# a1q123456/image_stitching

Hardware: AMD Instinct MI355X
Metric: 4K frames stitched/sec (higher is better)
Workload: dtype u8

## Files before the change

host/job.cpp:

```cpp
#include "job.hpp"
#include <algorithm>
#include <cstring>
#include <numeric>

namespace mis {

static float median_focal(const std::vector<CameraParams>& cams, const std::vector<int>& idx) {
    std::vector<double> f;
    for (int i : idx) f.push_back(cams[i].focal);
    std::sort(f.begin(), f.end());
    return f.size() % 2 == 1 ? static_cast<float>(f[f.size() / 2]) : static_cast<float>(f[f.size() / 2 - 1] + f[f.size() / 2]) * 0.5f;
}

void StitchJob::check(MisContext* c, int rc, const char* what) const {
    if (rc != MIS_OK) throw std::runtime_error(std::string(what) + " failed: " + mis_last_error(c));
}

StitchJob::StitchJob(int device, int width, int height, const std::vector<CameraParams>& cameras, const StitchConfig& cfg)
    : w_(width), h_(height), n_((int)cameras.size()), cams_(cameras), cfg_(cfg) {
    if (cfg_.features_type != "orb" || cfg_.ba_cost_func != "no" || cfg_.expos_comp_type != "no" || cfg_.seam_find_type != "no")
        throw std::runtime_error("mis::StitchJob runs the hot path (ORB, supplied cameras, no seam-scale step); use mis::Stitcher for the other options");
    if (mis_context_create(device, nullptr, &ctx_) != MIS_OK) throw std::runtime_error("mis_context_create failed: no HIP device (there is no CPU fallback)");
    check(ctx_, mis_stream_create(device, 0, &cstream_), "mis_stream_create");
    if (mis_context_create(device, cstream_, &cctx_) != MIS_OK) throw std::runtime_error("mis_context_create (compose stream) failed");
// ... 24 lines not shown
    check(ctx_, mis_context_synchronize(ctx_), "mis_context_synchronize");
    check(cctx_, mis_context_synchronize(cctx_), "mis_context_synchronize (compose)");
}

StitchJob::Compose StitchJob::prepare(const std::vector<int>& idx) {
    const int m = (int)idx.size();
    const float scale = median_focal(cams_, idx);
    std::vector<float> Ks((size_t)m * 9), Rs((size_t)m * 9);
    for (int k = 0; k < m; k++) {
        std::copy(Ks_.begin() + 9 * idx[k], Ks_.begin() + 9 * idx[k] + 9, Ks.begin() + 9 * k);
        std::copy(Rs_.begin() + 9 * idx[k], Rs_.begin() + 9 * idx[k] + 9, Rs.begin() + 9 * k);
    }
    rois_.assign(m, MisRect{});
    check(cctx_, mis_warp_roi_batch(cctx_, scale, w_, h_, m, Ks.data(), Rs.data(), rois_.data()), "mis_warp_roi_batch");
    std::vector<MisPoint> corners(m);
    std::vector<MisSize> sizes(m);
    for (int k = 0; k < m; k++) { corners[k] = {rois_[k].x, rois_[k].y}; sizes[k] = {rois_[k].width, rois_[k].height}; }
    Compose c;
    check(cctx_, mis_result_roi(corners.data(), sizes.data(), m, &c.pano), "mis_result_roi");
    check(cctx_, mis_blend_config(cfg_.blend_type, cfg_.blend_strength, c.pano.width, c.pano.height, &c.type, &c.bands, &c.sharp), "mis_blend_config");
    if (!blender_ || c.type != key_.type || c.bands != key_.bands || c.sharp != key_.sharp) {
        if (blender_) { mis_blender_destroy(blender_); blender_ = nullptr; }
        check(cctx_, mis_blender_create(cctx_, c.type, c.bands, c.sharp, &blender_), "mis_blender_create");
    }
    key_ = c;
    check(cctx_, mis_blender_prepare(blender_, corners.data(), sizes.data(), m), "mis_blender_prepare");
    return c;
}

void StitchJob::compose(const std::vector<MisImage>& frames, const std::vector<int>& idx) {
    const int m = (int)idx.size();
    const float scale = median_focal(cams_, idx);
    std::vector<MisImage> fr(m);
    std::vector<float> Ks((size_t)m * 9), Rs((size_t)m * 9);
    for (int k = 0; k < m; k++) {
        fr[k] = frames[idx[k]];
        std::copy(Ks_.begin() + 9 * idx[k], Ks_.begin() + 9 * idx[k] + 9, Ks.begin() + 9 * k);
        std::copy(Rs_.begin() + 9 * idx[k], Rs_.begin() + 9 * idx[k] + 9, Rs.begin() + 9 * k);
    }
    check(cctx_, mis_compose_frames(blender_, fr.data(), m, scale, Ks.data(), Rs.data(), rois_.data()), "mis_compose_frames");
}

void StitchJob::finalize() {
    if (pano_.data && (pano_.width != key_.pano.width || pano_.height != key_.pano.height)) { mis_image_free(cctx_, &pano_); mis_image_free(cctx_, &mask_); pano_ = MisImage{}; mask_ = MisImage{}; }
    if (!pano_.data) { pano_ = MisImage{}; mask_ = MisImage{}; pano_.mem = mask_.mem = MIS_MEM_DEVICE; }
    check(cctx_, mis_blender_blend(blender_, &pano_, &mask_), "mis_blender_blend");
}

void StitchJob::hook(void* self_) {
    StitchJob* self = static_cast<StitchJob*>(self_);
    self->hook_ran_ = true;
    try {
        const int rc = mis_match_knn_fence(self->ctx_, self->cstream_, mis_match_sequence(self->ctx_), 0);
        if (rc < 0) self->check(self->ctx_, rc, "mis_match_knn_fence");
        std::vector<int> everyone(self->n_);
        std::iota(everyone.begin(), everyone.end(), 0);
        self->compose(*self->hook_frames_, everyone);
        self->finalize();
    } catch (const std::exception& e) {
        self->hook_error_ = e.what();
    }
}

void StitchJob::prep_hook(void* self_) {
    StitchJob* self = static_cast<StitchJob*>(self_);
    self->prep_ran_ = true;
    try {
        std::vector<int> everyone(self->n_);
        std::iota(everyone.begin(), everyone.end(), 0);
        self->prepare(everyone);
    } catch (const std::exception& e) { self->prep_error_ = e.what(); }
}

JobOutput StitchJob::run(const std::vector<MisImage>& frames) {
    if ((int)frames.size() != n_) throw std::runtime_error("StitchJob::run: one frame per camera");
    JobOutput out;
    std::vector<int> everyone(n_);
    std::iota(everyone.begin(), everyone.end(), 0);
    check(cctx_, mis_context_wait(cctx_, ctx_), "mis_context_wait");
    prep_ran_ = false; prep_error_.clear();
    check(ctx_, mis_orb_on_enqueued(orb_, &StitchJob::prep_hook, this), "mis_orb_on_enqueued");
    std::vector<MisFeatures> feats(n_);
    std::memset(feats.data(), 0, sizeof(MisFeatures) * n_);
    const int rc_f = mis_orb_detect_batch(orb_, frames.data(), n_, feats.data());
    mis_orb_on_enqueued(orb_, nullptr, nullptr);
    check(ctx_, rc_f, "mis_orb_detect_batch");
    if (!prep_ran_) prep_hook(this);
    if (!prep_error_.empty()) throw std::runtime_error(prep_error_);
    for (int i = 0; i < n_; i++) { feats[i].img_idx = i; out.num_features.push_back(feats[i].n); }
    if (!pairwise_.empty()) { mis_matches_free(pairwise_.data(), (int)pairwise_.size()); pairwise_.clear(); }
    pairwise_.assign((size_t)n_ * n_, MisMatchesInfo{});
    MisMatchParams mp;
    mis_match_default_params(&mp);
    mp.match_conf = cfg_.match_conf;
    hook_frames_ = &frames; hook_ran_ = false; hook_error_.clear();
    check(ctx_, mis_match_on_enqueued(ctx_, &StitchJob::hook, this), "mis_match_on_enqueued");
    const int rc = mis_match_all_pairs(ctx_, feats.data(), n_, &mp, pairwise_.data());
    mis_match_on_enqueued(ctx_, nullptr, nullptr);
    for (auto& f : feats) mis_features_free(ctx_, &f);
    check(ctx_, rc, "mis_match_all_pairs");
    if (!hook_ran_) hook(this);
    if (!hook_error_.empty()) throw std::runtime_error(hook_error_);
    out.confidence.resize((size_t)n_ * n_);
    for (int k = 0; k < n_ * n_; k++) out.confidence[k] = pairwise_[k].confidence;
    std::vector<int> idx(n_);
    int kept = 0;
    check(ctx_, mis_leave_biggest_component(pairwise_.data(), n_, cfg_.conf_thresh, idx.data(), &kept), "mis_leave_biggest_component");
    idx.resize(kept);
    if (kept < 2) throw std::runtime_error("Need more images");
    out.indices = idx;
    out.speculation_kept = kept == n_;
    if (!out.speculation_kept) {
        prepare(idx);
        compose(frames, idx);
        finalize();
    }
    check(cctx_, mis_context_synchronize(cctx_), "mis_context_synchronize (compose)");
    out.pano = pano_; out.mask = mask_;
    out.num_bands = key_.bands; out.pano_width = key_.pano.width; out.pano_height = key_.pano.height;
    out.matches = pairwise_;
    return out;
}

}
```

image_stitching_amd/_capi.py:

```python
import ctypes as C
import os
import re

_HERE = os.path.dirname(os.path.abspath(__file__))
LIB_PATH = os.path.join(_HERE, "libmistitch.so")
HEADER_PATH = os.path.join(os.path.dirname(_HERE), "include", "mistitch.h")

MIS_OK = 0
MIS_FENCE_TIMEOUT = 1
MEM_HOST, MEM_DEVICE = 0, 1
U8, S16, F32 = 0, 1, 2
INTER_NEAREST, INTER_LINEAR = 0, 1
BORDER_CONSTANT, BORDER_REFLECT = 0, 2
BLEND_NO, BLEND_FEATHER, BLEND_MULTI_BAND = 0, 1, 2


class MisPoint(C.Structure):
    _fields_ = [("x", C.c_int), ("y", C.c_int)]


class MisSize(C.Structure):
    _fields_ = [("width", C.c_int), ("height", C.c_int)]


class MisRect(C.Structure):
    _fields_ = [("x", C.c_int), ("y", C.c_int), ("width", C.c_int), ("height", C.c_int)]


class MisLevelRect(C.Structure):
    _fields_ = [("level", C.c_int), ("x0", C.c_int), ("y0", C.c_int), ("x1", C.c_int), ("y1", C.c_int), ("offset", C.c_ulonglong)]


class MisImage(C.Structure):
    _fields_ = [("data", C.c_void_p), ("width", C.c_int), ("height", C.c_int), ("channels", C.c_int),
                ("stride", C.c_size_t), ("dtype", C.c_int), ("mem", C.c_int)]


class MisKeyPoint(C.Structure):
    _fields_ = [("x", C.c_float), ("y", C.c_float), ("size", C.c_float), ("angle", C.c_float),
                ("response", C.c_float), ("octave", C.c_int)]


class MisOrbParams(C.Structure):
    _fields_ = [("nfeatures", C.c_int), ("scale_factor", C.c_float), ("nlevels", C.c_int),
                ("edge_threshold", C.c_int), ("first_level", C.c_int), ("wta_k", C.c_int),
                ("score_type", C.c_int), ("patch_size", C.c_int), ("fast_threshold", C.c_int)]


class MisSiftParams(C.Structure):
    _fields_ = [("nfeatures", C.c_int), ("n_octave_layers", C.c_int), ("contrast_threshold", C.c_double),
                ("edge_threshold", C.c_double), ("sigma", C.c_double)]


class MisCameraParams(C.Structure):
    _fields_ = [("focal", C.c_double), ("aspect", C.c_double), ("ppx", C.c_double), ("ppy", C.c_double), ("R", C.c_double * 9),
                ("t", C.c_double * 3)]


class MisFeatures(C.Structure):
    _fields_ = [("img_idx", C.c_int), ("img_w", C.c_int), ("img_h", C.c_int), ("n", C.c_int),
                ("keypoints", C.c_void_p), ("descriptors", C.c_void_p), ("desc_cols", C.c_int),
                ("desc_dtype", C.c_int), ("owner_", C.c_void_p)]


class MisMatchParams(C.Structure):
    _fields_ = [("match_conf", C.c_float), ("num_matches_thresh1", C.c_int), ("num_matches_thresh2", C.c_int),
                ("ransac_thresh", C.c_double), ("max_iters", C.c_int), ("confidence", C.c_double)]


class MisDMatch(C.Structure):
    _fields_ = [("query_idx", C.c_int), ("train_idx", C.c_int), ("img_idx", C.c_int), ("distance", C.c_float)]


class MisMatchesInfo(C.Structure):
    _fields_ = [("src_img_idx", C.c_int), ("dst_img_idx", C.c_int), ("n_matches", C.c_int),
                ("matches", C.POINTER(MisDMatch)), ("inliers_mask", C.POINTER(C.c_uint8)), ("num_inliers", C.c_int),
                ("has_H", C.c_int), ("H", C.c_double * 9), ("confidence", C.c_double)]


_vp, _i, _f, _d = C.c_void_p, C.c_int, C.c_float, C.c_double
_P = C.POINTER

PROTOTYPES = {
    "mis_context_create": (_i, [_i, _vp, _P(_vp)]),
    "mis_stream_create": (_i, [_i, _i, _P(_vp)]),
    "mis_stream_destroy": (_i, [_vp]),
    "mis_context_destroy": (_i, [_vp]),
    "mis_context_synchronize": (_i, [_vp]),
    "mis_context_wait": (_i, [_vp, _vp]),
    "mis_last_error": (C.c_char_p, [_vp]),
    "mis_version": (C.c_char_p, []),
    "mis_image_free": (_i, [_vp, _P(MisImage)]),
    "mis_orb_default_params": (None, [_P(MisOrbParams)]),
    "mis_orb_create": (_i, [_vp, _P(MisOrbParams), _i, _i, _P(_vp)]),
    "mis_orb_destroy": (_i, [_vp]),
    "mis_orb_detect": (_i, [_vp, _P(MisImage), _P(MisFeatures)]),
    "mis_orb_detect_batch": (_i, [_vp, _P(MisImage), _i, _P(MisFeatures)]),
    "mis_orb_on_enqueued": (_i, [_vp, _vp, _vp]),
    "mis_features_download": (_i, [_vp, _P(MisFeatures), _vp, _vp]),
    "mis_features_upload": (_i, [_vp, _i, _i, _i, _vp, _vp, _i, _i, _P(MisFeatures)]),
    "mis_features_free": (_i, [_vp, _P(MisFeatures)]),
    "mis_orb_debug_level": (_i, [_vp, _i, _i, _vp, _P(_i), _P(_i)]),
    "mis_sift_default_params": (None, [_P(MisSiftParams)]),
    "mis_sift_create": (_i, [_vp, _P(MisSiftParams), _i, _i, _P(_vp)]),
    "mis_sift_destroy": (_i, [_vp]),
    "mis_sift_detect": (_i, [_vp, _P(MisImage), _P(MisFeatures)]),
    "mis_sift_detect_batch": (_i, [_vp, _P(MisImage), _i, _P(MisFeatures)]),
    "mis_sift_debug_level": (_i, [_vp, _P(MisImage), _i, _i, _i, _vp, _P(_i), _P(_i)]),
    "mis_match_default_params": (None, [_P(MisMatchParams)]),
    "mis_match_all_pairs": (_i, [_vp, _P(MisFeatures), _i, _P(MisMatchParams), _P(MisMatchesInfo)]),
    "mis_match_pairs_sharded": (_i, [_vp, _P(MisFeatures), _i, _P(MisMatchParams), _i, _i, _P(MisMatchesInfo)]),
    "mis_matches_free": (_i, [_P(MisMatchesInfo), _i]),
    "mis_match_sequence": (C.c_longlong, [_vp]),
    "mis_match_knn_fence": (_i, [_vp, _vp, C.c_longlong, _i]),
    "mis_match_on_enqueued": (_i, [_vp, _vp, _vp]),
    "mis_knn2": (_i, [_vp, _P(MisFeatures), _P(MisFeatures), _vp, _vp]),
    "mis_find_homography": (_i, [_vp, _vp, _vp, _i, _d, _i, _d, _vp, _vp, _P(_i)]),
    "mis_leave_biggest_component": (_i, [_P(MisMatchesInfo), _i, _f, _vp, _P(_i)]),
    "mis_leave_biggest_component_conf": (_i, [_vp, _i, _f, _vp, _P(_i)]),
    "mis_bundle_adjust_reproj": (_i, [_vp, _P(MisFeatures), _P(MisMatchesInfo), _i, _f, C.c_char_p, _P(MisCameraParams)]),
    "mis_wave_correct": (_i, [_vp, _i, _i]),
    "mis_warp_roi": (_i, [_f, _i, _i, _vp, _vp, _P(MisRect)]),
    "mis_warp_spherical": (_i, [_vp, _P(MisImage), _f, _vp, _vp, _i, _i, _P(MisImage), _P(MisPoint)]),
    "mis_warp_roi_batch": (_i, [_vp, _f, _i, _i, _i, _vp, _vp, _P(MisRect)]),
    "mis_warp_spherical_fused_roi": (_i, [_vp, _P(MisImage), _f, _vp, _vp, _P(MisRect), _P(MisImage), _P(MisImage), _P(MisPoint)]),
    "mis_warp_spherical_fused_batch": (_i, [_vp, _P(MisImage), _i, C.c_float, _P(C.c_float), _P(C.c_float), _P(MisRect), _P(MisImage), _P(MisImage), _P(MisPoint)]),
    "mis_warp_spherical_fused_batch_timed": (_i, [_vp, _P(MisImage), _i, C.c_float, _P(C.c_float), _P(C.c_float), _P(MisRect), _P(MisImage), _P(MisImage), _P(MisPoint), _i,
                                               _P(C.c_float)]),
    "mis_warp_spherical_fused": (_i, [_vp, _P(MisImage), _f, _vp, _vp, _P(MisImage), _P(MisImage), _P(MisPoint)]),
    "mis_resize_linear_exact": (_i, [_vp, _P(MisImage), _i, _i, C.c_double, C.c_double, _P(MisImage)]),
    "mis_rotate": (_i, [_vp, _P(MisImage), _i, _P(MisImage)]),
    "mis_seam_mask_apply": (_i, [_vp, _P(MisImage), _P(MisImage)]),
    "mis_compensator_create": (_i, [_vp, _i, _i, _i, _P(_vp)]),
    "mis_compensator_destroy": (_i, [_vp]),
    "mis_compensator_feed": (_i, [_vp, _P(MisPoint), _P(MisImage), _P(MisImage), _i]),
    "mis_compensator_gain_map": (_i, [_vp, _i, _P(C.c_float), _i, _P(_i), _P(_i)]),
    "mis_compensator_apply": (_i, [_vp, _i, _P(MisImage)]),
    "mis_seam_voronoi": (_i, [_vp, _P(MisPoint), _P(MisImage), _i]),
    "mis_seam_dp": (_i, [_vp, _P(MisPoint), _P(MisImage), _P(MisImage), _i, _i]),
    "mis_warp_spherical_fused_timed": (_i, [_vp, _P(MisImage), _f, _vp, _vp, _P(MisImage), _P(MisImage), _P(MisPoint), _i, _P(C.c_float)]),
    "mis_blend_config": (_i, [_i, _f, _i, _i, _P(_i), _P(_i), _P(_f)]),
    "mis_result_roi": (_i, [_P(MisPoint), _P(MisSize), _i, _P(MisRect)]),
    "mis_blender_create": (_i, [_vp, _i, _i, _f, _P(_vp)]),
    "mis_blender_destroy": (_i, [_vp]),
    "mis_blender_prepare": (_i, [_vp, _P(MisPoint), _P(MisSize), _i]),
    "mis_blender_num_bands": (_i, [_vp]),
    "mis_blender_feed": (_i, [_vp, _P(MisImage), _P(MisImage), MisPoint]),
    "mis_blender_feed_batch": (_i, [_vp, _P(MisImage), _P(MisImage), _P(MisPoint), _i]),
    "mis_blender_blend": (_i, [_vp, _P(MisImage), _P(MisImage)]),
    "mis_compose_frames": (_i, [_vp, _P(MisImage), _i, _f, _vp, _vp, _P(MisRect)]),
    "mis_blender_blend_columns": (_i, [_vp, _i, _i, _P(MisImage), _P(MisImage)]),
    "mis_blender_pack_rects": (_i, [_vp, _P(MisLevelRect), _i, _vp, C.c_size_t]),
    "mis_blender_add_rects": (_i, [_vp, _P(MisLevelRect), _i, _vp, C.c_size_t]),
    "mis_blender_zero_rects": (_i, [_vp, _P(MisLevelRect), _i]),
    "mis_features_pack": (_i, [_vp, _P(MisFeatures), _i, _i, _i, _vp, _vp]),
    "mis_copy_2d": (_i, [_vp, _vp, C.c_size_t, _vp, C.c_size_t, C.c_size_t, C.c_size_t]),
    "mis_blender_feed_rect": (_i, [_vp, _i, _i, MisPoint, _P(MisRect)]),
    "mis_blender_level_info": (_i, [_vp, _i, _P(_i), _P(_i), _P(_vp), _P(_vp)]),
}


def header_functions():
    txt = open(HEADER_PATH).read()
    txt = re.sub(r"/\*.*?\*/", "", txt, flags=re.S)
    return sorted(set(re.findall(r"\b(mis_[a-z0-9_]+)\s*\(", txt)))


_lib = None


def load():
    global _lib
    if _lib is not None:
        return _lib
    if not os.path.exists(LIB_PATH):
        raise ImportError("libmistitch.so is not built (%s missing): run `python -c 'import __graft_entry__ as g; g.build()'` "
                          "or `make -C image_stitching_amd/csrc`; there is no CPU fallback" % LIB_PATH)
    lib = C.CDLL(LIB_PATH)
    for name, (res, args) in PROTOTYPES.items():
        fn = getattr(lib, name)
        fn.restype = res
        fn.argtypes = args
    _lib = lib
    return lib
```

image_stitching_amd/csrc/common.h:

```cpp
#pragma once
#include <hip/hip_runtime.h>
#include <stdint.h>
#include <stdio.h>
#include <string.h>
#include <string>
#include <vector>
#include "../../include/mistitch.h"

struct MisWorkspace {
    virtual ~MisWorkspace() {}
};

struct MisContext {
    int device = 0;
    int num_cu = 256;
    MisWorkspace* match_ws = nullptr;
    std::vector<std::pair<size_t, void*>> pool;
    hipStream_t stream = nullptr;
    bool own_stream = false;
    std::string err;
    void* stage = nullptr;
    size_t stage_bytes = 0;
    hipStream_t aux[2] = {nullptr, nullptr};
    void* roi_pinned = nullptr;
    size_t roi_pinned_bytes = 0;
    void* host_stage = nullptr;
    size_t host_stage_bytes = 0;
};

int mis_set_error(MisContext* ctx, int code, const char* fmt, ...);
int mis_host_stage(MisContext* ctx, size_t bytes, void** out);
int mis_pool_alloc(MisContext* ctx, size_t bytes, void** out, size_t* got);
int mis_aux_stream(MisContext* ctx, int k, hipStream_t* out);
void mis_pool_free(MisContext* ctx, void* p, size_t bytes);
int mis_feat_block_alloc(MisContext* ctx, size_t bytes, void** out);

#define MIS_HIP(ctx, call)                                                                             \
    do {                                                                                               \
        hipError_t e_ = (call);                                                                        \
        if (e_ != hipSuccess)                                                                          \
            return mis_set_error((ctx), MIS_E_HIP, "%s failed: %s (%s:%d)", #call, hipGetErrorString(e_), \
                                 __FILE__, __LINE__);                                                  \
    } while (0)

#define MIS_CHECK(ctx, cond, code, ...)                              \
    do {                                                             \
        if (!(cond)) return mis_set_error((ctx), (code), __VA_ARGS__); \
    } while (0)

static inline size_t mis_dtype_size(int dtype) { return dtype == MIS_U8 ? 1 : (dtype == MIS_S16 ? 2 : 4); }
static inline size_t mis_align_up(size_t v, size_t a) { return (v + a - 1) / a * a; }

struct DevImage {
    void* data = nullptr;
    size_t stride = 0;
    bool owned = false;
};
int mis_dev_image_in(MisContext* ctx, const MisImage* img, DevImage* out);
int mis_dev_image_release(MisContext* ctx, DevImage* d);
int mis_dev_image_out(MisContext* ctx, MisImage* img, int width, int height, int channels, int dtype, DevImage* out);
int mis_dev_image_commit(MisContext* ctx, const MisImage* img, DevImage* d);
```

image_stitching_amd/csrc/match.hip:

```cpp
#include "common.h"
#include <thread>
#include <chrono>
#include <atomic>
#include "dev_math.h"
#include "homography.h"
#include <algorithm>
#include <vector>

namespace {

struct FeatDev {
    const uint8_t* desc;
    const MisKeyPoint* kps;
    int n, w, h;
};

struct PairDesc {
    int i, j;
    size_t knn_off12, knn_off21;
    size_t m_off;
    int cap;
};

constexpr int KNN_TILE = 256;
__global__ __launch_bounds__(256) void knn2_hamming_kernel(const FeatDev* feats, const PairDesc* pairs, int* idx2, float* dist2) {
    __shared__ uint4 tr[KNN_TILE * 2];
    const PairDesc pd = pairs[blockIdx.y >> 1];
    const bool fwd = (blockIdx.y & 1) == 0;
    const FeatDev Q = feats[fwd ? pd.i : pd.j], T = feats[fwd ? pd.j : pd.i];
    const size_t off = fwd ? pd.knn_off12 : pd.knn_off21;
    const int q0 = blockIdx.x * 256;
    if (q0 >= Q.n) return;
    const int q = q0 + threadIdx.x;
    const bool active = q < Q.n;
    uint4 a0 = make_uint4(0, 0, 0, 0), a1 = a0;
    if (active) {
        const uint4* p = reinterpret_cast<const uint4*>(Q.desc + (size_t)q * 32);
        a0 = p[0]; a1 = p[1];
    }
    int k0 = 0x7fffffff, k1 = 0x7fffffff;
    for (int t0 = 0; t0 < T.n; t0 += KNN_TILE) {
        const int nt = min(KNN_TILE, T.n - t0);
        __syncthreads();
        const uint4* src = reinterpret_cast<const uint4*>(T.desc + (size_t)t0 * 32);
        for (int k = threadIdx.x; k < nt * 2; k += 256) tr[k] = src[k];
        __syncthreads();
        if (active) {
            auto one = [&](int j) {
                const uint4 b0 = tr[2 * j], b1 = tr[2 * j + 1];
                unsigned d = 0;
                auto acc = [&](unsigned x) { asm("v_bcnt_u32_b32 %0, %1, %0" : "+v"(d) : "v"(x)); };
                acc(a0.x ^ b0.x); acc(a0.y ^ b0.y); acc(a0.z ^ b0.z); acc(a0.w ^ b0.w);
                acc(a1.x ^ b1.x); acc(a1.y ^ b1.y); acc(a1.z ^ b1.z); acc(a1.w ^ b1.w);
                const int key = (int)((d << 22) | (unsigned)(t0 + j));
                asm("v_med3_i32 %0, %1, %2, %3" : "=v"(k1) : "v"(k0), "v"(k1), "v"(key));
                k0 = min(k0, key);
            };
            int j = 0;
            for (; j + 8 <= nt; j += 8) {
#pragma unroll
                for (int u = 0; u < 8; u++) one(j + u);
            }
            for (; j < nt; j++) one(j);
        }
    }
    if (active) {
        const int d0 = k0 == 0x7fffffff ? 1 << 30 : k0 >> 22, d1 = k1 == 0x7fffffff ? 1 << 30 : k1 >> 22;
        idx2[(off + q) * 2] = k0 == 0x7fffffff ? -1 : (k0 & 0x3fffff); idx2[(off + q) * 2 + 1] = k1 == 0x7fffffff ? -1 : (k1 & 0x3fffff);
        dist2[(off + q) * 2] = (float)d0; dist2[(off + q) * 2 + 1] = (float)d1;
    }
}

typedef int v4i __attribute__((ext_vector_type(4)));
typedef int v16i __attribute__((ext_vector_type(16)));
constexpr int HM_ROWPAD = 256;
constexpr int HM_MAX_TRAINS = 8192;
constexpr int HM_NONE = 0x7f000000;

struct HmFrame { size_t train_off, query_off; };

struct HmKeys { int k0[2], k1[2]; };
struct HmJob { int pair, dir, q0, pad; };
constexpr int HM_FBIAS = 0x3F800000;
__device__ __forceinline__ void hm_update(HmKeys& K, int set, int key) {
    asm volatile("v_med3_f32 %0, %1, %2, %3" : "=v"(K.k1[set]) : "v"(K.k0[set]), "v"(K.k1[set]), "v"(key));
    asm volatile("v_min_f32 %0, %1, %2" : "=v"(K.k0[set]) : "v"(K.k0[set]), "v"(key));
}
__device__ __forceinline__ void hm_dma(const int8_t* base, unsigned voff, uint32_t lds_off) {
    asm volatile("s_mov_b32 m0, %2\n\ts_nop 0\n\tglobal_load_lds_dwordx4 %0, %1" ::"v"(voff), "s"(base), "s"(lds_off) : "memory", "m0");
}
__global__ __launch_bounds__(256) void hamming_expand4_kernel(const FeatDev* feats, const HmFrame* fr, int8_t* out) {
    const FeatDev F = feats[blockIdx.y];
    const int npad = (F.n + HM_ROWPAD - 1) / HM_ROWPAD * HM_ROWPAD;
    const int item = blockIdx.x * 256 + threadIdx.x, d = item >> 3, w = item & 7;
    if (d >= npad) return;
    const bool live = d < F.n;
    const unsigned x = live ? reinterpret_cast<const unsigned*>(F.desc)[(size_t)d * 8 + w] : 0u;
    unsigned tq[4], qq[4];
#pragma unroll
    for (int k = 0; k < 4; k++) {
        unsigned t = (x >> (8 * k)) & 255u;
        t = (t | (t << 12)) & 0x000F000Fu;
        t = (t | (t << 6)) & 0x03030303u;
        t = (t | (t << 3)) & 0x11111111u;
        tq[k] = live ? (0xEEEEEEEEu ^ (t << 3)) : 0u;
        qq[k] = live ? (0x66666666u ^ (t << 3)) : 0u;
    }
    *reinterpret_cast<uint4*>(out + fr[blockIdx.y].train_off + (size_t)d * 128 + 16 * w) = make_uint4(tq[0], tq[1], tq[2], tq[3]);
    *reinterpret_cast<uint4*>(out + fr[blockIdx.y].query_off + (size_t)d * 128 + 16 * w) = make_uint4(qq[0], qq[1], qq[2], qq[3]);
}
#define HM4_MFMA_FIRST(D, A, B, C, SA, SB) \
    asm volatile("v_mfma_scale_f32_32x32x64_f8f6f4 %0, %1, %2, %3, %4, %5 op_sel_hi:[0,0,0] cbsz:4 blgp:4" : "=&v"(D) : "v"(A), "v"(B), "v"(C), "v"(SA), "v"(SB))
#define HM4_MFMA_ACC(D, A, B, SA, SB) \
    asm volatile("v_mfma_scale_f32_32x32x64_f8f6f4 %0, %1, %2, %0, %3, %4 op_sel_hi:[0,0,0] cbsz:4 blgp:4" : "+v"(D) : "v"(A), "v"(B), "v"(SA), "v"(SB))
typedef float v16f __attribute__((ext_vector_type(16)));
__device__ __forceinline__ void hm_update_triples(HmKeys& K, int x0, int x1, int x2, int y0, int y1, int y2) {
    int t0, t1, u0, u1;
    asm volatile(
        "v_min3_f32 %4, %8, %9, %10\n\tv_med3_f32 %5, %8, %9, %10\n\tv_min3_f32 %6, %11, %12, %13\n\tv_med3_f32 %7, %11, %12, %13\n\t"
        "v_min_f32 %5, %1, %5\n\tv_min_f32 %7, %3, %7\n\t"
        "v_med3_f32 %1, %0, %4, %5\n\tv_med3_f32 %3, %2, %6, %7\n\t"
        "v_min_f32 %0, %0, %4\n\tv_min_f32 %2, %2, %6"
        : "+v"(K.k0[0]), "+v"(K.k1[0]), "+v"(K.k0[1]), "+v"(K.k1[1]), "=&v"(t0), "=&v"(t1), "=&v"(u0), "=&v"(u1)
        : "v"(x0), "v"(x1), "v"(x2), "v"(y0), "v"(y1), "v"(y2));
}
__device__ __forceinline__ void hm_update_both(HmKeys& K, int a, int b) {
    asm volatile("v_med3_f32 %1, %0, %1, %4\n\tv_min_f32 %0, %0, %4\n\tv_med3_f32 %3, %2, %3, %5\n\tv_min_f32 %2, %2, %5"
                 : "+v"(K.k0[0]), "+v"(K.k1[0]), "+v"(K.k0[1]), "+v"(K.k1[1]) : "v"(a), "v"(b));
}
template <bool UPD>
__device__ __forceinline__ void hm_tile_fp4(v16i& accA, v16i& accB, const v16i& prevA, const v16i& prevB, v16f& cb, v4i* a, const v4i (&bq)[2][4], HmKeys& K,
                                            const int8_t* lds_next, uint32_t lds_store, const int8_t* gnext, unsigned voff, const unsigned (&aoff)[4], int sa, int sb) {
    hm_dma(gnext, voff, lds_store);
#pragma unroll
    for (int s4 = 0; s4 < 4; s4++) {
#pragma unroll
        for (int half = 0; half < 2; half++) {
            const int slot = 2 * s4 + half;
            if (half == 0) { if (s4 == 0) HM4_MFMA_FIRST(accA, a[0], bq[0][0], cb, sa, sb); else HM4_MFMA_ACC(accA, a[s4], bq[0][s4], sa, sb); }
            else {
                if (s4 == 0) HM4_MFMA_FIRST(accB, a[0], bq[1][0], cb, sa, sb); else HM4_MFMA_ACC(accB, a[s4], bq[1][s4], sa, sb);
                a[s4] = *reinterpret_cast<const v4i*>(lds_next + aoff[s4]);
            }
            if (slot >= 2) {
                if (UPD) {
                    const int j = slot - 2;
                    if (j < 5) hm_update_triples(K, prevA[3 * j], prevA[3 * j + 1], prevA[3 * j + 2], prevB[3 * j], prevB[3 * j + 1], prevB[3 * j + 2]);
                    else hm_update_both(K, prevA[15], prevB[15]);
                }
                if (slot >= 4) {
#pragma unroll
                    for (int g = (slot - 4) * 4; g < (slot - 3) * 4; g++) cb[g] += 32.f;
                }
            }
            __builtin_amdgcn_sched_barrier(0);
        }
    }
    asm volatile("s_waitcnt vmcnt(0)" ::: "memory");
    __syncthreads();
}

__global__ __launch_bounds__(256) void knn2_hamming_fp4_kernel(const FeatDev* feats, const PairDesc* pairs, const HmFrame* fr, const int8_t* __restrict__ xp, int* idx2,
                                                               float* dist2, const HmJob* jobs) {
    __shared__ __attribute__((aligned(1024))) int8_t tr[2][32 * 128];
    const HmJob job = jobs[blockIdx.x];
    if (job.pair < 0) return;
    const PairDesc pd = pairs[job.pair];
    const bool fwd = job.dir == 0;
    const int qi = fwd ? pd.i : pd.j, ti = fwd ? pd.j : pd.i;
    const int nq = feats[qi].n, nt = feats[ti].n;
    const size_t off = fwd ? pd.knn_off12 : pd.knn_off21;
    const int q0 = job.q0;
    if (q0 >= nq) return;
    const int lane = threadIdx.x & 63, wave = __builtin_amdgcn_readfirstlane(threadIdx.x >> 6), r = lane & 31, h = lane >> 5;
    const int8_t* qx = xp + fr[qi].query_off;
    const int8_t* tx = xp + fr[ti].train_off;
    HmKeys K;
    K.k0[0] = K.k0[1] = K.k1[0] = K.k1[1] = HM_NONE;
    const int ntiles = (nt + 31) / 32;
    if (ntiles > 0) {
        v4i bq[2][4];
#pragma unroll
        for (int set = 0; set < 2; set++)
#pragma unroll
            for (int s4 = 0; s4 < 4; s4++)
                bq[set][s4] = *reinterpret_cast<const v4i*>(qx + (size_t)(q0 + wave * 64 + set * 32 + r) * 128 + 32 * s4 + 16 * h);
        v16f cb;
#pragma unroll
        for (int g = 0; g < 16; g++) cb[g] = (float)((1 << 20) + (g & 3) + 8 * (g >> 2) + 4 * h);
        const int sa = 127 + 4, sb = 127 + 4;
        const int R = 8 * wave + (lane >> 3);
        const unsigned voff = (unsigned)(R * 128 + 16 * ((lane & 7) ^ ((R >> 1) & 7)));
        unsigned aoff[4];
#pragma unroll
        for (int s4 = 0; s4 < 4; s4++) aoff[s4] = (unsigned)(r * 128 + 16 * ((2 * s4 + h) ^ ((r >> 1) & 7)));
        const uint32_t lds0 = (uint32_t)(uintptr_t)&tr[0][0] + (uint32_t)wave * 1024, lds1 = (uint32_t)(uintptr_t)&tr[1][0] + (uint32_t)wave * 1024;
        auto gtile = [&](int t) { return tx + (size_t)min(t, ntiles - 1) * 32 * 128; };
        hm_dma(gtile(0), voff, lds0);
        hm_dma(gtile(1), voff, lds1);
        asm volatile("s_waitcnt vmcnt(0)" ::: "memory");
        __syncthreads();
        v4i a[4];
#pragma unroll
        for (int s4 = 0; s4 < 4; s4++) a[s4] = *reinterpret_cast<const v4i*>(&tr[0][aoff[s4]]);
        __syncthreads();
        v16i A0, B0, A1, B1;
        hm_tile_fp4<false>(A0, B0, A1, B1, cb, a, bq, K, tr[1], lds0, gtile(2), voff, aoff, sa, sb);
        int t = 1;
        for (; t + 1 < ntiles; t += 2) {
            hm_tile_fp4<true>(A1, B1, A0, B0, cb, a, bq, K, tr[0], lds1, gtile(t + 2), voff, aoff, sa, sb);
            hm_tile_fp4<true>(A0, B0, A1, B1, cb, a, bq, K, tr[1], lds0, gtile(t + 3), voff, aoff, sa, sb);
        }
        const bool odd_last = t < ntiles;
        if (odd_last) hm_tile_fp4<true>(A1, B1, A0, B0, cb, a, bq, K, tr[0], lds1, gtile(t + 2), voff, aoff, sa, sb);
        asm volatile("s_nop 15\n\ts_nop 15\n\ts_nop 15\n\ts_nop 15\n\ts_nop 15" ::: "memory");
#pragma unroll
        for (int g = 0; g < 16; g++) {
            const int ka = odd_last ? A1[g] : A0[g], kb = odd_last ? B1[g] : B0[g];
            hm_update(K, 0, ((int)__int_as_float(ka) & (HM_MAX_TRAINS - 1)) < nt ? ka : HM_NONE);
            hm_update(K, 1, ((int)__int_as_float(kb) & (HM_MAX_TRAINS - 1)) < nt ? kb : HM_NONE);
        }
    }
#pragma unroll
    for (int set = 0; set < 2; set++) {
        const int o0 = __shfl_xor(K.k0[set], 32), o1 = __shfl_xor(K.k1[set], 32);
        const int b0 = min(K.k0[set], o0), b1 = min(max(K.k0[set], o0), min(K.k1[set], o1));
        const int q = q0 + wave * 64 + set * 32 + r;
        if (h == 0 && q < nq) {
            const bool v0 = b0 < HM_NONE, v1 = b1 < HM_NONE;
            const int i0 = v0 ? (int)__int_as_float(b0) : 0, i1 = v1 ? (int)__int_as_float(b1) : 0;
            idx2[(off + q) * 2] = v0 ? (i0 & (HM_MAX_TRAINS - 1)) : -1; idx2[(off + q) * 2 + 1] = v1 ? (i1 & (HM_MAX_TRAINS - 1)) : -1;
            dist2[(off + q) * 2] = (float)(v0 ? i0 >> 13 : 1 << 30); dist2[(off + q) * 2 + 1] = (float)(v1 ? i1 >> 13 : 1 << 30);
        }
    }
}

struct L2Set {
    const _Float16* h;
    const float* nrm;
    int n;
};
__global__ __launch_bounds__(256) void l2_prep_kernel(const float* desc, int n, int dim, _Float16* h, float* nrm, int* bad) {
    const int i = blockIdx.x * 4 + (threadIdx.x >> 6), lane = threadIdx.x & 63;
    if (i >= n) return;
    float s = 0;
    for (int k = lane; k < 128; k += 64) {
        float v = k < dim ? desc[(size_t)i * dim + k] : 0.f;
        if (!(v >= 0.f && v <= 255.f && v == floorf(v))) atomicOr(bad, 1);
        h[(size_t)i * 128 + k] = (_Float16)v;
        s += v * v;
    }
    for (int o = 32; o > 0; o >>= 1) s += __shfl_xor(s, o);
    if (lane == 0) nrm[i] = s;
// ... 114 lines not shown
            }
            float16v acc0 = {0, 0, 0, 0, 0, 0, 0, 0, 0, 0, 0, 0, 0, 0, 0, 0}, acc1 = acc0;
            const uint8_t* brow = sb[buf][sub] + r * L2_PITCH + 16 * hh;
#pragma unroll
            for (int s8 = 0; s8 < 8; s8++) {
                const half8 b = *reinterpret_cast<const half8*>(brow + 32 * s8);
                acc0 = __builtin_amdgcn_mfma_f32_32x32x16_f16(b, a0[s8], acc0, 0, 0, 0);
                acc1 = __builtin_amdgcn_mfma_f32_32x32x16_f16(b, a1[s8], acc1, 0, 0, 0);
            }
            l2_tile_update(acc0, tn, tbase, ta);
            l2_tile_update(acc1, tn, tbase, tb);
        }
        if (tile + L2_SUB < tile_hi) stash(buf ^ 1);
        __syncthreads();
    }
    auto finish = [&](Top2 t, int q) {
        const float od0 = __shfl_xor(t.e0, 32), od1 = __shfl_xor(t.e1, 32);
        const int oi0 = __shfl_xor(t.i0, 32), oi1 = __shfl_xor(t.i1, 32);
        top2_insert(od0, oi0, t.e0, t.i0, t.e1, t.i1);
        top2_insert(od1, oi1, t.e0, t.i0, t.e1, t.i1);
        if (hh == 0 && q < Q.n) {
            const size_t o = ((size_t)slice * Q.n + q) * 2;
            part_idx[o] = t.i0; part_idx[o + 1] = t.i1;
            part_e[o] = t.e0; part_e[o + 1] = t.e1;
        }
    };
    finish(ta, q0 + r);
    finish(tb, q0 + 32 + r);
}

__global__ __launch_bounds__(256) void l2_merge_kernel(L2Set Q, int slices, const int* __restrict__ part_idx, const float* __restrict__ part_e, int* __restrict__ idx2,
                                                      float* __restrict__ dist2) {
    const int q = blockIdx.x * 256 + threadIdx.x;
    if (q >= Q.n) return;
    float d0 = 3.0e38f, d1 = 3.0e38f;
    int i0 = 0x7fffffff, i1 = 0x7fffffff;
    for (int s = 0; s < slices; s++) {
        const size_t o = ((size_t)s * Q.n + q) * 2;
        top2_insert(part_e[o], part_idx[o], d0, i0, d1, i1);
        top2_insert(part_e[o + 1], part_idx[o + 1], d0, i0, d1, i1);
    }
    const float qn = Q.nrm[q];
    idx2[2 * (size_t)q] = i0 == 0x7fffffff ? -1 : i0; idx2[2 * (size_t)q + 1] = i1 == 0x7fffffff ? -1 : i1;
    dist2[2 * (size_t)q] = i0 == 0x7fffffff ? sqrtf(3.0e38f) : sqrtf(qn + d0);
    dist2[2 * (size_t)q + 1] = i1 == 0x7fffffff ? sqrtf(3.0e38f) : sqrtf(qn + d1);
}

static void l2_knn2_launch(hipStream_t st, int num_cu, const L2Set& Q, const L2Set& T, void* part, int* idx2, float* dist2) {
    const int qblocks = (Q.n + 128 * L2_QW - 1) / (128 * L2_QW), ntiles = (T.n + L2_TB - 1) / L2_TB;
    int slices = 1;
    while (slices < L2_MAX_SLICES && qblocks * slices < K8_WG_PER_CU * num_cu && ntiles / (2 * slices) >= 16) slices *= 2;
    const int tiles_per_slice = ((ntiles + slices - 1) / slices + L2_SUB - 1) / L2_SUB * L2_SUB;
    const int nwg = slices >= 8 ? qblocks * slices : (qblocks + 8 / slices - 1) / (8 / slices) * 8;
    int* pi = (int*)part;
    float* pe = (float*)(pi + (size_t)2 * L2_MAX_SLICES * Q.n);
    hipLaunchKernelGGL(l2_knn2_mfma_kernel, dim3(nwg), dim3(256), 0, st, Q, T, tiles_per_slice, slices, qblocks, pi, pe);
    hipLaunchKernelGGL(l2_merge_kernel, dim3((Q.n + 255) / 256), dim3(256), 0, st, Q, slices, (const int*)pi, (const float*)pe, idx2, dist2);
}

__device__ __forceinline__ int block_scan_flag(int flag, int* total) {
    __shared__ int wsum[16];
    __shared__ int wtot;
    const int lane = threadIdx.x & 63, wave = threadIdx.x >> 6;
    unsigned long long b = __ballot(flag);
    int within = __popcll(b & ((1ull << lane) - 1ull));
    if (lane == 0) wsum[wave] = __popcll(b);
    __syncthreads();
    if (threadIdx.x == 0) {
        int s = 0;
        for (int k = 0; k < (int)(blockDim.x >> 6); k++) { int v = wsum[k]; wsum[k] = s; s += v; }
        wtot = s;
    }
    __syncthreads();
    int off = wsum[wave] + within;
    *total = wtot;
    __syncthreads();
    return off;
}

__global__ __launch_bounds__(1024) void ratio_union_kernel(const FeatDev* feats, const PairDesc* pairs, const int* idx2, const float* dist2, float ratio,
                                                           MisDMatch* matches, float* src_xy, float* dst_xy, int* n_matches) {
    const PairDesc pd = pairs[blockIdx.x];
    const FeatDev F1 = feats[pd.i], F2 = feats[pd.j];
    MisDMatch* m = matches + pd.m_off;
    float* sp = src_xy + 2 * pd.m_off;
    float* dp = dst_xy + 2 * pd.m_off;
    const int* i12 = idx2 + pd.knn_off12 * 2;
    const float* d12 = dist2 + pd.knn_off12 * 2;
    const int* i21 = idx2 + pd.knn_off21 * 2;
    const float* d21 = dist2 + pd.knn_off21 * 2;
    const float hw1 = (float)F1.w * 0.5f, hh1 = (float)F1.h * 0.5f, hw2 = (float)F2.w * 0.5f, hh2 = (float)F2.h * 0.5f;
    int base = 0;
    if (F2.n >= 2)
        for (int q0 = 0; q0 < F1.n; q0 += 1024) {
            int q = q0 + threadIdx.x, ok = 0;
            if (q < F1.n) ok = d12[2 * q] < ratio * d12[2 * q + 1];
            int tot, off = block_scan_flag(ok, &tot);
            if (ok) {
                int t = i12[2 * q];
                MisDMatch mm = {q, t, 0, d12[2 * q]};
                m[base + off] = mm;
                sp[2 * (base + off)] = F1.kps[q].x - hw1; sp[2 * (base + off) + 1] = F1.kps[q].y - hh1;
                dp[2 * (base + off)] = F2.kps[t].x - hw2; dp[2 * (base + off) + 1] = F2.kps[t].y - hh2;
            }
            base += tot;
        }
    if (F1.n >= 2)
        for (int q0 = 0; q0 < F2.n; q0 += 1024) {
            int q = q0 + threadIdx.x, ok = 0, t1 = 0;
            if (q < F2.n) {
                ok = d21[2 * q] < ratio * d21[2 * q + 1];
                if (ok) {
                    t1 = i21[2 * q];
                    bool acc12 = F2.n >= 2 && d12[2 * t1] < ratio * d12[2 * t1 + 1];
                    if (acc12 && i12[2 * t1] == q) ok = 0;
                }
            }
            int tot, off = block_scan_flag(ok, &tot);
            if (ok) {
                MisDMatch mm = {t1, q, -1, d21[2 * q]};
                m[base + off] = mm;
                sp[2 * (base + off)] = F1.kps[t1].x - hw1; sp[2 * (base + off) + 1] = F1.kps[t1].y - hh1;
                dp[2 * (base + off)] = F2.kps[q].x - hw2; dp[2 * (base + off) + 1] = F2.kps[q].y - hh2;
            }
            base += tot;
        }
    if (threadIdx.x == 0) n_matches[blockIdx.x] = base;
}

struct PairOut {
    int ran_ransac;
    int passed;
    int second;
    int pad;
};

__host__ __device__ __forceinline__ double det3(const double* H) {
    return H[0] * (H[4] * H[8] - H[5] * H[7]) - H[1] * (H[3] * H[8] - H[5] * H[6]) + H[2] * (H[3] * H[7] - H[4] * H[6]);
}

__global__ void first_calls_kernel(const PairDesc* pairs, int np, const int* n_matches, const float* src_xy, const float* dst_xy, uint8_t* masks,
                                   int thresh1, HomoCall* calls, PairOut* outs) {
    int k = blockIdx.x * blockDim.x + threadIdx.x;
    if (k >= np) return;
    const PairDesc pd = pairs[k];
    const int nm = n_matches[k];
    HomoCall c;
    c.src = src_xy + 2 * pd.m_off; c.dst = dst_xy + 2 * pd.m_off; c.mask = masks + pd.m_off; c.pt_off = (long long)pd.m_off;
    c.n = nm; c.active = nm >= thresh1;
    calls[k] = c;
    outs[k].ran_ransac = c.active; outs[k].passed = 0; outs[k].second = 0;
}


__global__ __launch_bounds__(256) void pack_lists_kernel(const PairDesc* pairs, int np, const int* nm, const MisDMatch* matches, MisDMatch* host_m, int* host_nm) {
    __shared__ int red[256];
    const int k = blockIdx.x, t = threadIdx.x;
    int part = 0;
    for (int q = t; q < k; q += 256) part += nm[q];
    red[t] = part;
    __syncthreads();
    for (int o = 128; o > 0; o >>= 1) { if (t < o) red[t] += red[t + o]; __syncthreads(); }
    const int off = red[0], cnt = nm[k];
    if (t == 0) host_nm[k] = cnt;
    const uint4* s = reinterpret_cast<const uint4*>(matches + pairs[k].m_off);
    uint4* d = reinterpret_cast<uint4*>(host_m + off);
    static_assert(sizeof(MisDMatch) == 16, "one 16-byte store per match");
    for (int i = t; i < cnt; i += 256) d[i] = s[i];
}

struct CopySegs { const uint8_t* src[8]; uint8_t* dst[8]; unsigned bytes[8]; int n; };
__global__ __launch_bounds__(256) void copy_segments_kernel(CopySegs c) {
    for (int k = 0; k < c.n; k++) {
        const uint8_t* s = c.src[k];
        uint8_t* d = c.dst[k];
        const unsigned nb = c.bytes[k];
        if ((((uintptr_t)s | (uintptr_t)d) & 3) == 0) {
            const unsigned nw = nb >> 2;
            for (unsigned i = blockIdx.x * 256 + threadIdx.x; i < nw; i += gridDim.x * 256) reinterpret_cast<unsigned*>(d)[i] = reinterpret_cast<const unsigned*>(s)[i];
            for (unsigned i = (nw << 2) + blockIdx.x * 256 + threadIdx.x; i < nb; i += gridDim.x * 256) d[i] = s[i];
        } else {
            for (unsigned i = blockIdx.x * 256 + threadIdx.x; i < nb; i += gridDim.x * 256) d[i] = s[i];
        }
    }
}

__global__ void second_calls_kernel(int np, const HomoCall* calls1, const HomoResult* res1, const float* scr1, const int* fin1, int want, int thresh2,
                                    HomoCall* calls2, PairOut* outs) {
    int k = blockIdx.x * blockDim.x + threadIdx.x;
    if (k >= np) return;
    const HomoCall c1 = calls1[k];
    HomoCall c;
    c.src = nullptr; c.dst = nullptr; c.mask = nullptr; c.pt_off = c1.pt_off; c.n = 0; c.active = 0;
    if (fin1[k] == want && c1.active && res1[k].ok) {
        outs[k].passed = 1;
        const int ninl = res1[k].ninl;
        if (ninl >= thresh2) {
            c.src = scr1 + 4 * c1.pt_off; c.dst = c.src + 2 * (size_t)c1.n; c.n = ninl; c.active = 1;
            outs[k].second = 1;
        }
    }
    calls2[k] = c;
}

void invert3(const double* H, double* I) {
    double d = H[0] * (H[4] * H[8] - H[5] * H[7]) - H[1] * (H[3] * H[8] - H[5] * H[6]) + H[2] * (H[3] * H[7] - H[4] * H[6]);
    if (d != 0.) d = 1. / d;
    I[0] = (H[4] * H[8] - H[5] * H[7]) * d; I[1] = (H[2] * H[7] - H[1] * H[8]) * d; I[2] = (H[1] * H[5] - H[2] * H[4]) * d;
    I[3] = (H[5] * H[6] - H[3] * H[8]) * d; I[4] = (H[0] * H[8] - H[2] * H[6]) * d; I[5] = (H[2] * H[3] - H[0] * H[5]) * d;
    I[6] = (H[3] * H[7] - H[4] * H[6]) * d; I[7] = (H[1] * H[6] - H[0] * H[7]) * d; I[8] = (H[0] * H[4] - H[1] * H[3]) * d;
}

struct Arena {
    void* p = nullptr;
    size_t bytes = 0;
    bool host = false;
    hipError_t reserve(size_t need) {
        if (need <= bytes) return hipSuccess;
        if (p) { hipError_t e = host ? hipHostFree(p) : hipFree(p); p = nullptr; bytes = 0; if (e != hipSuccess) return e; }
        need = need + need / 4 + 4096;
        hipError_t e = host ? hipHostMalloc(&p, need, hipHostMallocDefault) : hipMalloc(&p, need);
        if (e == hipSuccess) bytes = need;
        return e;
    }
    void release() { if (p) { if (host) hipHostFree(p); else hipFree(p); } p = nullptr; bytes = 0; }
};

struct MatchWorkspace : MisWorkspace {
    Arena dev, pinned, l2;
    HomoBatch b1, b2, b3;
    hipStream_t side = nullptr, third = nullptr;
    hipEvent_t ev_phase0 = nullptr, ev_side_done = nullptr, ev_phase1 = nullptr, ev_third_done = nullptr, ev_matches = nullptr;
    hipEvent_t ev_knn = nullptr;
    hipEvent_t ev_draw1 = nullptr;
    hipEvent_t tev[8] = {nullptr};
    hipEvent_t ev_gate = nullptr;
    std::atomic<long long> seq{0}, knn_seq{0};
    hipEvent_t ev_lists = nullptr;
    void (*enqueued_cb)(void*) = nullptr;
    void* enqueued_user = nullptr;
    MatchWorkspace() { pinned.host = true; }
    ~MatchWorkspace() override {
        dev.release(); pinned.release(); l2.release();
        homo_batch_release(&b1); homo_batch_release(&b2); homo_batch_release(&b3);
        if (ev_phase1) hipEventDestroy(ev_phase1);
        if (ev_third_done) hipEventDestroy(ev_third_done);
        if (ev_matches) hipEventDestroy(ev_matches);
        if (ev_lists) hipEventDestroy(ev_lists);
        if (ev_phase0) hipEventDestroy(ev_phase0);
        if (ev_side_done) hipEventDestroy(ev_side_done);
        if (ev_knn) hipEventDestroy(ev_knn);
        if (ev_draw1) hipEventDestroy(ev_draw1);
    }
};

MatchWorkspace* workspace(MisContext* ctx) {
    if (!ctx->match_ws) ctx->match_ws = new MatchWorkspace();
    return static_cast<MatchWorkspace*>(ctx->match_ws);
}

struct Carver {
    size_t off = 0;
    size_t take(size_t bytes) { size_t o = off; off += mis_align_up(bytes ? bytes : 1, 256); return o; }
};

void init_info(MisMatchesInfo* m) {
    memset(m, 0, sizeof(*m));
    m->src_img_idx = -1; m->dst_img_idx = -1;
}

int match_impl(MisContext* ctx, const MisFeatures* feats, int n, const MisMatchParams* p, int rank, int world, MisMatchesInfo* out) {
    MIS_CHECK(ctx, feats && p && out && n >= 1, MIS_E_INVALID, "null argument");
    MIS_CHECK(ctx, world >= 1 && rank >= 0 && rank < world, MIS_E_INVALID, "bad rank / world size");
    MIS_HIP(ctx, hipSetDevice(ctx->device));
    const auto t_begin = std::chrono::steady_clock::now();
    struct SeqGuard {
        MatchWorkspace* ws; long long seq;
        ~SeqGuard() { if (ws->knn_seq.load() < seq) ws->knn_seq.store(seq); }
    } seq_guard{workspace(ctx), 0};
    seq_guard.seq = ++seq_guard.ws->seq;
    for (int i = 0; i < n * n; i++) init_info(&out[i]);
    std::vector<PairDesc> pairs;
    std::vector<FeatDev> fd(n);
    size_t knn_total = 0, m_total = 0;
    bool use_l2 = false, use_bin = false;
    for (int i = 0; i < n; i++) {
        const bool bin_i = feats[i].desc_dtype == MIS_U8 && feats[i].desc_cols == 32;
        const bool l2_i = feats[i].desc_dtype == MIS_F32 && feats[i].desc_cols >= 1 && feats[i].desc_cols <= 128;
        MIS_CHECK(ctx, feats[i].n == 0 || bin_i || l2_i, MIS_E_UNSUPPORTED,
                  "all-pairs matching supports 32-byte binary descriptors (Hamming) or f32 descriptors of <= 128 columns (L2)");
        MIS_CHECK(ctx, feats[i].n < (1 << 22), MIS_E_UNSUPPORTED, "more than 4 M keypoints in one image");
        if (feats[i].n > 0) { if (l2_i) use_l2 = true; else use_bin = true; }
        fd[i] = FeatDev{(const uint8_t*)feats[i].descriptors, feats[i].keypoints, feats[i].n, feats[i].img_w, feats[i].img_h};
    }
    int pair_index = 0;
    for (int i = 0; i < n; i++)
        for (int j = i + 1; j < n; j++) {
            if (feats[i].n <= 0 || feats[j].n <= 0) continue;
            if ((pair_index++ % world) != rank) continue;
            PairDesc pd;
            pd.i = i; pd.j = j;
            pd.knn_off12 = knn_total; knn_total += feats[i].n;
            pd.knn_off21 = knn_total; knn_total += feats[j].n;
            pd.m_off = m_total; pd.cap = feats[i].n + feats[j].n; m_total += pd.cap;
            pairs.push_back(pd);
        }
    MIS_CHECK(ctx, !(use_l2 && use_bin), MIS_E_INVALID, "binary and float descriptors cannot be mixed in one matcher call");
    for (int i = 0, cols = 0; use_l2 && i < n; i++)
        if (feats[i].n > 0) {
            MIS_CHECK(ctx, cols == 0 || feats[i].desc_cols == cols, MIS_E_INVALID, "float descriptors of different widths in one matcher call");
            cols = feats[i].desc_cols;
        }
    const int np = (int)pairs.size();
    if (np == 0) return MIS_OK;
    int maxq = 0;
    for (int i = 0; i < n; i++) maxq = std::max(maxq, feats[i].n);
    std::vector<HmJob> hm_jobs;
    if (!use_l2 && maxq <= HM_MAX_TRAINS) {
        std::vector<HmJob> lists[8];
        for (int t = 0; t < n; t++)
            for (int k = 0; k < np; k++) {
                const int dir = pairs[k].j == t ? 0 : (pairs[k].i == t ? 1 : -1);
                if (dir < 0) continue;
                const int nqf = feats[dir == 0 ? pairs[k].i : pairs[k].j].n;
                for (int q0 = 0; q0 < nqf; q0 += 256) lists[t & 7].push_back(HmJob{k, dir, q0, 0});
            }
        size_t longest = 0;
        for (auto& l : lists) longest = std::max(longest, l.size());
        hm_jobs.assign(longest * 8, HmJob{-1, 0, 0, 0});
        for (int c = 0; c < 8; c++)
            for (size_t sl = 0; sl < lists[c].size(); sl++) hm_jobs[sl * 8 + c] = lists[c][sl];
    }
    MatchWorkspace* ws = workspace(ctx);
    hipStream_t st = ctx->stream;
    MIS_HIP(ctx, hipStreamSynchronize(st));
    Carver dc;
    const size_t o_feats = dc.take(sizeof(FeatDev) * n), o_pairs = dc.take(sizeof(PairDesc) * np), o_idx = dc.take(sizeof(int) * 2 * knn_total),
                 o_dist = dc.take(sizeof(int) * 2 * knn_total), o_matches = dc.take(sizeof(MisDMatch) * m_total), o_src = dc.take(sizeof(float) * 2 * m_total),
                 o_dst = dc.take(sizeof(float) * 2 * m_total), o_nm = dc.take(sizeof(int) * np), o_mask = dc.take(m_total), o_out = dc.take(sizeof(PairOut) * np);
    MIS_HIP(ctx, ws->dev.reserve(dc.off));
    uint8_t* D = (uint8_t*)ws->dev.p;
    FeatDev* d_feats = (FeatDev*)(D + o_feats); PairDesc* d_pairs = (PairDesc*)(D + o_pairs);
    int* d_idx = (int*)(D + o_idx); float* d_dist = (float*)(D + o_dist);
    MisDMatch* d_matches = (MisDMatch*)(D + o_matches); float* d_src = (float*)(D + o_src); float* d_dst = (float*)(D + o_dst);
    int* d_nm = (int*)(D + o_nm); uint8_t* d_mask = D + o_mask; PairOut* d_out = (PairOut*)(D + o_out);
    int rc;
    if ((rc = homo_batch_reserve(ctx, &ws->b1, np, (long long)m_total, p->max_iters)) != MIS_OK) return rc;
    if ((rc = homo_batch_reserve(ctx, &ws->b2, np, (long long)m_total, p->max_iters)) != MIS_OK) return rc;
    if ((rc = homo_batch_reserve(ctx, &ws->b3, np, (long long)m_total, p->max_iters)) != MIS_OK) return rc;
    Carver hc;
    const size_t h_in = hc.take(sizeof(FeatDev) * n + sizeof(PairDesc) * np + sizeof(HmFrame) * n + 1024), h_nm = hc.take(sizeof(int) * np), h_out = hc.take(sizeof(PairOut) * np),
                 h_r1 = hc.take(sizeof(HomoResult) * np), h_r2 = hc.take(sizeof(HomoResult) * np), h_r3 = hc.take(sizeof(HomoResult) * np), h_fin = hc.take(sizeof(int) * np), h_m = hc.take(sizeof(MisDMatch) * m_total), h_mask = hc.take(m_total), h_bad = hc.take(256), h_jobs = hc.take(sizeof(HmJob) * std::max<size_t>(hm_jobs.size(), 1));
    MIS_HIP(ctx, ws->pinned.reserve(hc.off));
    uint8_t* Hh = (uint8_t*)ws->pinned.p;
    memcpy(Hh + h_in, fd.data(), sizeof(FeatDev) * n);
    PairDesc* h_pairs = (PairDesc*)(Hh + h_in + mis_align_up(sizeof(FeatDev) * n, 256));
    memcpy(h_pairs, pairs.data(), sizeof(PairDesc) * np);
    MIS_HIP(ctx, hipMemcpyAsync(d_feats, Hh + h_in, sizeof(FeatDev) * n, hipMemcpyHostToDevice, st));
    MIS_HIP(ctx, hipMemcpyAsync(d_pairs, h_pairs, sizeof(PairDesc) * np, hipMemcpyHostToDevice, st));
    volatile int& l2_bad = *reinterpret_cast<volatile int*>(Hh + h_bad);
    l2_bad = 0;
    if (!use_l2 && maxq > HM_MAX_TRAINS) {
        hipLaunchKernelGGL(knn2_hamming_kernel, dim3((maxq + 255) / 256, 2 * np), dim3(256), 0, st, (const FeatDev*)d_feats, (const PairDesc*)d_pairs, d_idx, d_dist);
    } else if (!use_l2 && !hm_jobs.empty()) {
        std::vector<HmFrame> hf(n);
        Carver lc;
        const size_t o_fr = lc.take(sizeof(HmFrame) * n), o_jobs = lc.take(sizeof(HmJob) * hm_jobs.size());
        for (int i = 0; i < n; i++) {
            const size_t rows = (size_t)(std::max(feats[i].n, 1) + HM_ROWPAD - 1) / HM_ROWPAD * HM_ROWPAD;
            hf[i].train_off = lc.take(rows * 128); hf[i].query_off = lc.take(rows * 128);
        }
        MIS_HIP(ctx, ws->l2.reserve(lc.off));
        uint8_t* L = (uint8_t*)ws->l2.p;
        HmFrame* h_fr = (HmFrame*)(Hh + h_in + mis_align_up(sizeof(FeatDev) * n, 256) + mis_align_up(sizeof(PairDesc) * np, 256));
        memcpy(h_fr, hf.data(), sizeof(HmFrame) * n);
        MIS_HIP(ctx, hipMemcpyAsync(L + o_fr, h_fr, sizeof(HmFrame) * n, hipMemcpyHostToDevice, st));
        const int maxpad = (maxq + HM_ROWPAD - 1) / HM_ROWPAD * HM_ROWPAD;
        hipLaunchKernelGGL(hamming_expand4_kernel, dim3(maxpad * 8 / 256, n), dim3(256), 0, st, (const FeatDev*)d_feats, (const HmFrame*)(L + o_fr), (int8_t*)L);
        memcpy(Hh + h_jobs, hm_jobs.data(), sizeof(HmJob) * hm_jobs.size());
        MIS_HIP(ctx, hipMemcpyAsync(L + o_jobs, Hh + h_jobs, sizeof(HmJob) * hm_jobs.size(), hipMemcpyHostToDevice, st));
        hipLaunchKernelGGL(knn2_hamming_fp4_kernel, dim3((unsigned)hm_jobs.size()), dim3(256), 0, st, (const FeatDev*)d_feats, (const PairDesc*)d_pairs,
                           (const HmFrame*)(L + o_fr), (const int8_t*)L, d_idx, d_dist, (const HmJob*)(L + o_jobs));
    } else if (!use_l2) {
    } else {
        std::vector<size_t> hoff(n), noff(n);
        Carver lc;
        for (int i = 0; i < n; i++) { hoff[i] = lc.take((size_t)std::max(feats[i].n, 1) * 256); noff[i] = lc.take((size_t)std::max(feats[i].n, 1) * 4); }
        const size_t o_bad = lc.take(4);
        const size_t o_part = lc.take((size_t)16 * L2_MAX_SLICES * std::max(maxq, 1));
        MIS_HIP(ctx, ws->l2.reserve(lc.off));
        uint8_t* L = (uint8_t*)ws->l2.p;
        MIS_HIP(ctx, hipMemsetAsync(L + o_bad, 0, 4, st));
        for (int i = 0; i < n; i++)
            if (feats[i].n > 0)
                hipLaunchKernelGGL(l2_prep_kernel, dim3((feats[i].n + 3) / 4), dim3(256), 0, st, (const float*)feats[i].descriptors, feats[i].n,
                                   feats[i].desc_cols, (_Float16*)(L + hoff[i]), (float*)(L + noff[i]), (int*)(L + o_bad));
        for (const PairDesc& pd : pairs) {
            L2Set A{(const _Float16*)(L + hoff[pd.i]), (const float*)(L + noff[pd.i]), feats[pd.i].n}, B{(const _Float16*)(L + hoff[pd.j]), (const float*)(L + noff[pd.j]), feats[pd.j].n};
            l2_knn2_launch(st, ctx->num_cu, A, B, L + o_part, d_idx + 2 * pd.knn_off12, d_dist + 2 * pd.knn_off12);
            l2_knn2_launch(st, ctx->num_cu, B, A, L + o_part, d_idx + 2 * pd.knn_off21, d_dist + 2 * pd.knn_off21);
        }
        MIS_HIP(ctx, hipMemcpyAsync(Hh + h_bad, L + o_bad, 4, hipMemcpyDeviceToHost, st));
    }
    if (!ws->ev_knn) MIS_HIP(ctx, hipEventCreateWithFlags(&ws->ev_knn, hipEventDisableTiming));
    MIS_HIP(ctx, hipEventRecord(ws->ev_knn, st));
    ws->ev_gate = ws->ev_knn;
    hipLaunchKernelGGL(ratio_union_kernel, dim3(np), dim3(1024), 0, st, (const FeatDev*)d_feats, (const PairDesc*)d_pairs, (const int*)d_idx,
                       (const float*)d_dist, 1.f - p->match_conf, d_matches, d_src, d_dst, d_nm);
    hipLaunchKernelGGL(first_calls_kernel, dim3((np + 127) / 128), dim3(128), 0, st, (const PairDesc*)d_pairs, np, (const int*)d_nm, (const float*)d_src,
                       (const float*)d_dst, d_mask, p->num_matches_thresh1, ws->b1.calls, d_out);
    if (!ws->side) {
        if ((rc = mis_aux_stream(ctx, 0, &ws->side)) != MIS_OK) return rc;
        MIS_HIP(ctx, hipEventCreateWithFlags(&ws->ev_phase0, hipEventDisableTiming));
        MIS_HIP(ctx, hipEventCreateWithFlags(&ws->ev_side_done, hipEventDisableTiming));
    }
    const double rt = p->ransac_thresh, cf = p->confidence;
    static const bool trace_ev = getenv("MIS_MATCH_TRACE") != nullptr;
    auto mark = [&](int i, hipStream_t s_) {
        if (!trace_ev) return;
        if (!ws->tev[i]) hipEventCreate(&ws->tev[i]);
        hipEventRecord(ws->tev[i], s_);
    };
    mark(0, st);
    auto enqueue_chains = [&]() -> int {
        if (!ws->third) {
            if ((rc = mis_aux_stream(ctx, 1, &ws->third)) != MIS_OK) return rc;
            MIS_HIP(ctx, hipEventCreateWithFlags(&ws->ev_phase1, hipEventDisableTiming));
            MIS_HIP(ctx, hipEventCreateWithFlags(&ws->ev_third_done, hipEventDisableTiming));
            MIS_HIP(ctx, hipEventCreateWithFlags(&ws->ev_matches, hipEventDisableTiming));
            MIS_HIP(ctx, hipEventCreateWithFlags(&ws->ev_lists, hipEventDisableTiming));
        }
        MIS_HIP(ctx, hipEventRecord(ws->ev_matches, st));
        MIS_HIP(ctx, hipStreamWaitEvent(ws->third, ws->ev_matches, 0));
        hipLaunchKernelGGL(pack_lists_kernel, dim3(np), dim3(256), 0, ws->third, (const PairDesc*)d_pairs, np, (const int*)d_nm, (const MisDMatch*)d_matches,
                           (MisDMatch*)(Hh + h_m), (int*)(Hh + h_nm));
        MIS_HIP(ctx, hipEventRecord(ws->ev_lists, ws->third));
        if ((rc = homo_batch_run(ctx, &ws->b1, rt, p->max_iters, cf, HOMO_PHASE0_REPLAY, st)) != MIS_OK) return rc;
        if ((rc = homo_batch_run(ctx, &ws->b1, rt, p->max_iters, cf, HOMO_TAIL0_MASK, st)) != MIS_OK) return rc;
        MIS_HIP(ctx, hipEventRecord(ws->ev_phase0, st));
        mark(1, st);
        MIS_HIP(ctx, hipStreamWaitEvent(ws->side, ws->ev_phase0, 0));
        hipLaunchKernelGGL(second_calls_kernel, dim3((np + 127) / 128), dim3(128), 0, ws->side, np, (const HomoCall*)ws->b1.calls, (const HomoResult*)ws->b1.results,
                           (const float*)ws->b1.scr, (const int*)ws->b1.fin, 0, p->num_matches_thresh2, ws->b2.calls, d_out);
        if (!ws->ev_draw1) MIS_HIP(ctx, hipEventCreateWithFlags(&ws->ev_draw1, hipEventDisableTiming));
        {
            HomoSync sy;
            sy.rec = ws->ev_draw1; sy.rec_pos = 2; ws->ev_gate = ws->ev_draw1;
            if ((rc = homo_batch_run(ctx, &ws->b2, rt, p->max_iters, cf, HOMO_BOTH_PHASES, ws->side, &sy)) != MIS_OK) return rc;
        }
        MIS_HIP(ctx, hipEventRecord(ws->ev_side_done, ws->side));
        mark(4, ws->side);
        MIS_HIP(ctx, hipStreamWaitEvent(ws->third, ws->ev_phase0, 0));
        if ((rc = homo_batch_run(ctx, &ws->b1, rt, p->max_iters, cf, HOMO_TAIL0_REFINE, ws->third)) != MIS_OK) return rc;
        mark(6, ws->third);
        {
            HomoSync sy;
            if (trace_ev) {
                if (!ws->tev[7]) hipEventCreate(&ws->tev[7]);
                sy.rec = ws->tev[7]; sy.rec_pos = 0;
            }
            if ((rc = homo_batch_run(ctx, &ws->b1, rt, p->max_iters, cf, HOMO_PHASE1_REPLAY, st, &sy)) != MIS_OK) return rc;
        }
        if ((rc = homo_batch_run(ctx, &ws->b1, rt, p->max_iters, cf, HOMO_TAIL1_MASK, st)) != MIS_OK) return rc;
        MIS_HIP(ctx, hipEventRecord(ws->ev_phase1, st));
        mark(2, st);
        if ((rc = homo_batch_run(ctx, &ws->b1, rt, p->max_iters, cf, HOMO_TAIL1_REFINE, st)) != MIS_OK) return rc;
        mark(3, st);
        MIS_HIP(ctx, hipStreamWaitEvent(ws->third, ws->ev_phase1, 0));
        hipLaunchKernelGGL(second_calls_kernel, dim3((np + 127) / 128), dim3(128), 0, ws->third, np, (const HomoCall*)ws->b1.calls, (const HomoResult*)ws->b1.results,
                           (const float*)ws->b1.scr, (const int*)ws->b1.fin, 1, p->num_matches_thresh2, ws->b3.calls, d_out);
        if ((rc = homo_batch_run(ctx, &ws->b3, rt, p->max_iters, cf, HOMO_BOTH_PHASES, ws->third)) != MIS_OK) return rc;
        MIS_HIP(ctx, hipEventRecord(ws->ev_third_done, ws->third));
        mark(5, ws->third);
        MIS_HIP(ctx, hipStreamWaitEvent(st, ws->ev_third_done, 0));
        MIS_HIP(ctx, hipStreamWaitEvent(st, ws->ev_side_done, 0));
        return MIS_OK;
    };
    if ((rc = enqueue_chains()) != MIS_OK) {
        if (ws->side) hipStreamSynchronize(ws->side);
        if (ws->third) hipStreamSynchronize(ws->third);
        hipStreamSynchronize(st);
        return rc;
    }
    MIS_HIP(ctx, hipGetLastError());
    int* nm = (int*)(Hh + h_nm);
    PairOut* po = (PairOut*)(Hh + h_out);
    HomoResult* r1 = (HomoResult*)(Hh + h_r1);
    HomoResult* r2 = (HomoResult*)(Hh + h_r2);
    HomoResult* r3 = (HomoResult*)(Hh + h_r3);
    int* fin = (int*)(Hh + h_fin);
    MisDMatch* hm = (MisDMatch*)(Hh + h_m);
    uint8_t* hmask = Hh + h_mask;
    {
        CopySegs cs;
        const void* srcs[6] = {d_out, ws->b1.results, ws->b2.results, ws->b3.results, ws->b1.fin, d_mask};
        void* dsts[6] = {po, r1, r2, r3, fin, hmask};
        const size_t sizes[6] = {sizeof(PairOut) * np, sizeof(HomoResult) * np, sizeof(HomoResult) * np, sizeof(HomoResult) * np, sizeof(int) * np, m_total};
        cs.n = 6;
        for (int k = 0; k < 6; k++) { cs.src[k] = (const uint8_t*)srcs[k]; cs.dst[k] = (uint8_t*)dsts[k]; cs.bytes[k] = (unsigned)sizes[k]; }
        for (int k = 6; k < 8; k++) { cs.src[k] = nullptr; cs.dst[k] = nullptr; cs.bytes[k] = 0; }
        hipLaunchKernelGGL(copy_segments_kernel, dim3(64), dim3(256), 0, st, cs);
    }
    ws->knn_seq.store(seq_guard.seq);
    if (ws->enqueued_cb) {
        void (*cb)(void*) = ws->enqueued_cb;
        void* user = ws->enqueued_user;
        ws->enqueued_cb = nullptr; ws->enqueued_user = nullptr;
        cb(user);
        MIS_HIP(ctx, hipSetDevice(ctx->device));
    }
    const bool trace = getenv("MIS_MATCH_TRACE") != nullptr;
    const auto tq = std::chrono::steady_clock::now();
    auto drop_lists = [&]() {
        for (int k = 0; k < np; k++) {
            const PairDesc& pd = pairs[k];
            MisMatchesInfo* e[2] = {&out[pd.i * n + pd.j], &out[pd.j * n + pd.i]};
            for (MisMatchesInfo* m : e) { free(m->matches); free(m->inliers_mask); init_info(m); }
        }
    };
    MIS_HIP(ctx, hipEventSynchronize(ws->ev_lists));
    {
        size_t packed_off = 0;
        for (int k = 0; k < np; k++) {
            const PairDesc& pd = pairs[k];
            MisMatchesInfo* a = &out[pd.i * n + pd.j];
            MisMatchesInfo* b = &out[pd.j * n + pd.i];
            a->src_img_idx = pd.i; a->dst_img_idx = pd.j;
            a->n_matches = nm[k];
            a->matches = (MisDMatch*)malloc(sizeof(MisDMatch) * (size_t)(nm[k] + 1));
            memcpy(a->matches, hm + packed_off, sizeof(MisDMatch) * (size_t)nm[k]);
            packed_off += (size_t)nm[k];
            b->matches = (MisDMatch*)malloc(sizeof(MisDMatch) * (size_t)(nm[k] + 1));
            for (int q = 0; q < nm[k]; q++) {
                b->matches[q] = a->matches[q];
                b->matches[q].query_idx = a->matches[q].train_idx;
                b->matches[q].train_idx = a->matches[q].query_idx;
            }
        }
    }
    {
        const hipError_t e = hipStreamSynchronize(st);
        if (e != hipSuccess) {
            drop_lists();
            return mis_set_error(ctx, MIS_E_HIP, "hipStreamSynchronize failed: %s (%s:%d)", hipGetErrorString(e), __FILE__, __LINE__);
        }
    }
    const auto ts = std::chrono::steady_clock::now();
    if (l2_bad) {
        drop_lists();
        return mis_set_error(ctx, MIS_E_UNSUPPORTED, "L2 matching needs integer-valued descriptors in 0..255 (SIFT style)");
    }
    for (int k = 0; k < np; k++) {
        const PairDesc& pd = pairs[k];
        MisMatchesInfo* a = &out[pd.i * n + pd.j];
        MisMatchesInfo* b = &out[pd.j * n + pd.i];
        MisDMatch* bm = b->matches;
        if (po[k].ran_ransac) {
            a->inliers_mask = (uint8_t*)malloc((size_t)nm[k] + 1);
            memcpy(a->inliers_mask, hmask + pd.m_off, (size_t)nm[k]);
        }
        const bool det_ok = !(fabs(det3(r1[k].H)) < DBL_EPSILON);
        const bool passed = po[k].passed && det_ok, second = po[k].second && det_ok;
        const HomoResult& hr = second ? (fin[k] == 0 ? r2[k] : r3[k]) : r1[k];
        a->has_H = po[k].ran_ransac ? hr.ok : 0;
        if (a->has_H) memcpy(a->H, hr.H, sizeof(a->H));
        a->num_inliers = passed ? r1[k].ninl : 0;
        if (passed) {
            double c = a->num_inliers / (8 + 0.3 * nm[k]);
            a->confidence = c > 3. ? 0. : c;
        }
        *b = *a;
        b->src_img_idx = pd.j; b->dst_img_idx = pd.i;
        b->matches = bm;
        if (a->inliers_mask) {
            b->inliers_mask = (uint8_t*)malloc((size_t)nm[k] + 1);
            memcpy(b->inliers_mask, a->inliers_mask, (size_t)nm[k]);
        }
        if (a->has_H) invert3(a->H, b->H);
    }
    if (trace) {
        const auto te = std::chrono::steady_clock::now();
        auto us = [](auto a, auto b) { return (double)std::chrono::duration_cast<std::chrono::microseconds>(b - a).count(); };
        fprintf(stderr, "match: enqueue %.0f us, device wait %.0f us, host assembly %.0f us\n", us(t_begin, tq), us(tq, ts), us(ts, te));
        if (ws->tev[0] && ws->tev[1] && ws->tev[3] && ws->tev[4] && ws->tev[5] && ws->tev[6]) {
            float e1 = 0, e3 = 0, e4 = 0, e5 = 0, e6 = 0;
            hipEventElapsedTime(&e1, ws->tev[0], ws->tev[1]); hipEventElapsedTime(&e3, ws->tev[0], ws->tev[3]); hipEventElapsedTime(&e4, ws->tev[0], ws->tev[4]);
            hipEventElapsedTime(&e5, ws->tev[0], ws->tev[5]); hipEventElapsedTime(&e6, ws->tev[0], ws->tev[6]);
            float e2 = 0, e7 = 0;
            if (ws->tev[2]) hipEventElapsedTime(&e2, ws->tev[0], ws->tev[2]);
            if (ws->tev[7]) { hipEventElapsedTime(&e7, ws->tev[0], ws->tev[7]); fprintf(stderr, "match chains: main chain's second draw done %.2f\n", e7); }
            fprintf(stderr, "match chains, ms after the 2-NN pass was enqueued-behind (device events): first phase done %.2f | tails of its finishers done %.2f | main chain: second RANSAC phase done %.2f, done %.2f | side chain done %.2f | third chain done %.2f\n", e1, e6, e2, e3, e4, e5);
        }
    }
    return MIS_OK;
}

}

extern "C" int mis_match_on_enqueued(MisContext* ctx, void (*fn)(void*), void* user) {
    if (!ctx) return MIS_E_INVALID;
    MatchWorkspace* ws = workspace(ctx);
    ws->enqueued_cb = fn; ws->enqueued_user = user;
    return MIS_OK;
}

extern "C" long long mis_match_sequence(MisContext* ctx) {
    if (!ctx) return -1;
    return workspace(ctx)->seq.load();
}

extern "C" int mis_match_knn_fence(MisContext* ctx, void* stream, long long target_seq, int timeout_ms) {
    if (!ctx) return MIS_E_INVALID;
    MatchWorkspace* ws = (MatchWorkspace*)ctx->match_ws;
    MIS_CHECK(ctx, ws, MIS_E_STATE, "mis_match_sequence must have been called on this context first");
    const auto t0 = std::chrono::steady_clock::now();
    while (ws->knn_seq.load() < target_seq) {
        if (std::chrono::duration_cast<std::chrono::milliseconds>(std::chrono::steady_clock::now() - t0).count() >= timeout_ms) return MIS_FENCE_TIMEOUT;
        std::this_thread::yield();
    }
    if (stream && ws->ev_gate && hipStreamWaitEvent((hipStream_t)stream, ws->ev_gate, 0) != hipSuccess) return mis_set_error(ctx, MIS_E_HIP, "hipStreamWaitEvent failed");
    return MIS_OK;
}

extern "C" int mis_debug_ransac_states(MisContext* ctx, int which, int* out, int cap) {
    if (!ctx || !ctx->match_ws || !out) return -1;
    MatchWorkspace* ws = (MatchWorkspace*)ctx->match_ws;
    return homo_batch_debug_states(ctx, which ? &ws->b2 : &ws->b1, out, cap);
}

extern "C" void mis_match_default_params(MisMatchParams* p) {
    if (p) *p = MisMatchParams{0.32f, 6, 6, 3.0, 2000, 0.995};
}

extern "C" int mis_match_all_pairs(MisContext* ctx, const MisFeatures* feats, int n, const MisMatchParams* p, MisMatchesInfo* out) {
    if (!ctx) return MIS_E_INVALID;
    return match_impl(ctx, feats, n, p, 0, 1, out);
}

extern "C" int mis_match_pairs_sharded(MisContext* ctx, const MisFeatures* feats, int n, const MisMatchParams* p, int rank, int world,
                                       MisMatchesInfo* out) {
    if (!ctx) return MIS_E_INVALID;
    return match_impl(ctx, feats, n, p, rank, world, out);
}

extern "C" int mis_matches_free(MisMatchesInfo* m, int count) {
    if (!m) return MIS_E_INVALID;
    for (int i = 0; i < count; i++) {
        free(m[i].matches); free(m[i].inliers_mask);
        m[i].matches = nullptr; m[i].inliers_mask = nullptr;
    }
    return MIS_OK;
}

extern "C" int mis_knn2(MisContext* ctx, const MisFeatures* q, const MisFeatures* t, int* idx2, float* dist2) {
    if (!ctx) return MIS_E_INVALID;
    MIS_CHECK(ctx, q && t && idx2 && dist2, MIS_E_INVALID, "null argument");
    const bool binary = q->desc_dtype == MIS_U8 && q->desc_cols == 32 && t->desc_dtype == MIS_U8 && t->desc_cols == 32;
    const bool l2 = q->desc_dtype == MIS_F32 && t->desc_dtype == MIS_F32 && q->desc_cols == t->desc_cols && q->desc_cols >= 1 && q->desc_cols <= 128;
    MIS_CHECK(ctx, binary || l2, MIS_E_UNSUPPORTED, "mis_knn2 supports 32-byte binary descriptors (Hamming) and f32 descriptors of <= 128 columns (L2)");
    if (q->n <= 0) return MIS_OK;
    MIS_HIP(ctx, hipSetDevice(ctx->device));
    MatchWorkspace* ws = workspace(ctx);
    hipStream_t st = ctx->stream;
    MIS_HIP(ctx, hipStreamSynchronize(st));
    const size_t nq = (size_t)q->n, nt = (size_t)std::max(t->n, 0);
    Carver dc;
    const size_t o_feats = dc.take(2 * sizeof(FeatDev)), o_pairs = dc.take(sizeof(PairDesc)), o_idx = dc.take(sizeof(int) * 2 * nq), o_dist = dc.take(sizeof(float) * 2 * nq);
    const size_t o_qh = dc.take(nq * 256), o_th = dc.take(nt * 256), o_qn = dc.take(nq * 4), o_tn = dc.take(nt * 4), o_bad = dc.take(4);
    const size_t o_part = dc.take((size_t)16 * L2_MAX_SLICES * nq);
    MIS_HIP(ctx, ws->dev.reserve(dc.off));
    uint8_t* D = (uint8_t*)ws->dev.p;
    int bad = 0;
    if (binary) {
        FeatDev fd[2] = {{(const uint8_t*)q->descriptors, q->keypoints, q->n, q->img_w, q->img_h},
                         {(const uint8_t*)t->descriptors, t->keypoints, t->n, t->img_w, t->img_h}};
        PairDesc pd;
        pd.i = 0; pd.j = 1; pd.knn_off12 = 0; pd.knn_off21 = q->n; pd.m_off = 0; pd.cap = q->n + t->n;
        MIS_HIP(ctx, hipMemcpyAsync(D + o_feats, fd, sizeof(fd), hipMemcpyHostToDevice, st));
        MIS_HIP(ctx, hipMemcpyAsync(D + o_pairs, &pd, sizeof(pd), hipMemcpyHostToDevice, st));
        MIS_HIP(ctx, hipStreamSynchronize(st));
        hipLaunchKernelGGL(knn2_hamming_kernel, dim3((q->n + 255) / 256, 1), dim3(256), 0, st, (const FeatDev*)(D + o_feats), (const PairDesc*)(D + o_pairs),
                           (int*)(D + o_idx), (float*)(D + o_dist));
    } else {
        MIS_HIP(ctx, hipMemsetAsync(D + o_bad, 0, 4, st));
        hipLaunchKernelGGL(l2_prep_kernel, dim3((q->n + 3) / 4), dim3(256), 0, st, (const float*)q->descriptors, q->n, q->desc_cols, (_Float16*)(D + o_qh),
                           (float*)(D + o_qn), (int*)(D + o_bad));
        if (t->n > 0)
            hipLaunchKernelGGL(l2_prep_kernel, dim3((t->n + 3) / 4), dim3(256), 0, st, (const float*)t->descriptors, t->n, t->desc_cols, (_Float16*)(D + o_th),
                               (float*)(D + o_tn), (int*)(D + o_bad));
        L2Set Q{(const _Float16*)(D + o_qh), (const float*)(D + o_qn), q->n}, T{(const _Float16*)(D + o_th), (const float*)(D + o_tn), std::max(t->n, 0)};
        l2_knn2_launch(st, ctx->num_cu, Q, T, D + o_part, (int*)(D + o_idx), (float*)(D + o_dist));
        MIS_HIP(ctx, hipMemcpyAsync(&bad, D + o_bad, 4, hipMemcpyDeviceToHost, st));
    }
    MIS_HIP(ctx, hipGetLastError());
    MIS_HIP(ctx, hipMemcpyAsync(idx2, D + o_idx, sizeof(int) * 2 * nq, hipMemcpyDeviceToHost, st));
    MIS_HIP(ctx, hipMemcpyAsync(dist2, D + o_dist, sizeof(float) * 2 * nq, hipMemcpyDeviceToHost, st));
    MIS_HIP(ctx, hipStreamSynchronize(st));
    MIS_CHECK(ctx, !bad, MIS_E_UNSUPPORTED, "L2 matching needs integer-valued descriptors in 0..255 (SIFT style): exactness of the fp16 MFMA path");
    return MIS_OK;
}

extern "C" int mis_find_homography(MisContext* ctx, const float* src, const float* dst, int n, double thresh, int max_iters, double confidence,
                                   double H[9], uint8_t* mask, int* ok) {
    if (!ctx) return MIS_E_INVALID;
    MIS_CHECK(ctx, src && dst && H && ok && n >= 0, MIS_E_INVALID, "null argument");
    MIS_HIP(ctx, hipSetDevice(ctx->device));
    MatchWorkspace* ws = workspace(ctx);
    hipStream_t st = ctx->stream;
    MIS_HIP(ctx, hipStreamSynchronize(st));
    const size_t nn = (size_t)std::max(n, 1);
    Carver dc;
    const size_t o_src = dc.take(sizeof(float) * 2 * nn), o_dst = dc.take(sizeof(float) * 2 * nn), o_mask = dc.take(nn);
    MIS_HIP(ctx, ws->dev.reserve(dc.off));
    uint8_t* D = (uint8_t*)ws->dev.p;
    int rc;
    if ((rc = homo_batch_reserve(ctx, &ws->b1, 1, (long long)nn, max_iters)) != MIS_OK) return rc;
    if (n) {
        MIS_HIP(ctx, hipMemcpyAsync(D + o_src, src, sizeof(float) * 2 * n, hipMemcpyHostToDevice, st));
        MIS_HIP(ctx, hipMemcpyAsync(D + o_dst, dst, sizeof(float) * 2 * n, hipMemcpyHostToDevice, st));
    }
    HomoCall c;
    c.src = (const float*)(D + o_src); c.dst = (const float*)(D + o_dst); c.mask = D + o_mask; c.pt_off = 0; c.n = n; c.active = 1;
    MIS_HIP(ctx, hipMemcpyAsync(ws->b1.calls, &c, sizeof(c), hipMemcpyHostToDevice, st));
    MIS_HIP(ctx, hipStreamSynchronize(st));
    if ((rc = homo_batch_run(ctx, &ws->b1, thresh, max_iters, confidence)) != MIS_OK) return rc;
    HomoResult r;
    MIS_HIP(ctx, hipMemcpyAsync(&r, ws->b1.results, sizeof(r), hipMemcpyDeviceToHost, st));
    if (mask && n) MIS_HIP(ctx, hipMemcpyAsync(mask, D + o_mask, n, hipMemcpyDeviceToHost, st));
    MIS_HIP(ctx, hipStreamSynchronize(st));
    *ok = r.ok;
    if (r.ok) memcpy(H, r.H, sizeof(r.H)); else memset(H, 0, sizeof(r.H));
    return MIS_OK;
}

static int biggest_component(const double* conf, int n, float conf_threshold, int* indices, int* n_indices) {
    std::vector<int> parent(n), rank_(n, 0), size(n, 1);
    for (int i = 0; i < n; i++) parent[i] = i;
    auto find = [&](int elem) {
        int set = elem;
        while (set != parent[set]) set = parent[set];
        while (elem != parent[elem]) { int next = parent[elem]; parent[elem] = set; elem = next; }
        return set;
    };
    for (int i = 0; i < n; i++)
        for (int j = 0; j < n; j++) {
            if (conf[(size_t)i * n + j] < conf_threshold) continue;
            int c1 = find(i), c2 = find(j);
            if (c1 == c2) continue;
            if (rank_[c1] < rank_[c2]) { parent[c1] = c2; size[c2] += size[c1]; }
            else if (rank_[c2] < rank_[c1]) { parent[c2] = c1; size[c1] += size[c2]; }
            else { parent[c1] = c2; rank_[c2]++; size[c2] += size[c1]; }
        }
    int max_comp = (int)(std::max_element(size.begin(), size.end()) - size.begin());
    int k = 0;
    for (int i = 0; i < n; i++) if (find(i) == max_comp) indices[k++] = i;
    *n_indices = k;
    return MIS_OK;
}
// ... 13 lines not shown
```

image_stitching_amd/csrc/orb.hip:

```cpp
#include "common.h"
#include "dev_math.h"
#include <algorithm>
#include <cmath>
#include <mutex>
#include <unordered_map>

#define ORB_MAX_LEVELS 16
#define ORB_BORDER 32

namespace {

struct LevelDesc {
    int w, h;
    int pp;
    int sp;
    size_t pad_off;
    size_t map_off;
    float scale;
    int nfeat;
    int n2;
    int tiles_x, tiles_y, tile_off;
    int cap1, cand_off;
    int cap2, fin_off;
    int tab_off;
// ... 808 lines not shown
                    m01 += in ? v * (vp - vm) : 0;
                }
            } else {
                for (int v = 1; v <= hp; ++v) {
                    if (abs(u) <= umax[v]) {
                        const int vp = ctr[u + v * DD_PITCH], vm = ctr[u - v * DD_PITCH];
                        m10 += u * (vp + vm);
                        m01 += v * (vp - vm);
                    }
                }
            }
        }
#pragma unroll
        for (int o = 32; o > 0; o >>= 1) { m01 += __shfl_xor(m01, o); m10 += __shfl_xor(m10, o); }
        kp_angle = mis_fast_atan2((float)m01, (float)m10);
        if (lane == 0) kps[i].angle = kp_angle;
    }
    float ang = kp_angle * (float)(3.14159265358979323846 / 180.f);
    float sa, ca;
    mis_sincosf(ang, &sa, &ca);
    const int b = lane & 31, h = lane >> 5;
    const int8_t* pat = pattern + b * 32 + h * 16;
    const unsigned* P32 = reinterpret_cast<const unsigned*>(P);
    auto blurred = [&](int ix, int iy) {
        const int a = c0 + (iy - 3) * DD_PITCH + (ix - 3);
        const bool inside = (unsigned)(cx + ix) < (unsigned)d.w && (unsigned)(cy + iy) < (unsigned)d.h;
        const unsigned* q = P32 + (a >> 2);
        const unsigned sh = (unsigned)(a & 3) << 3;
        const int kq[7] = {18, 34, 48, 56, 48, 34, 18};
        unsigned acc = 0, centre = 0;
#pragma unroll
        for (int j = 0; j < 7; j++) {
            const unsigned d0 = q[j * (DD_PITCH / 4)], d1 = q[j * (DD_PITCH / 4) + 1], d2 = q[j * (DD_PITCH / 4) + 2];
            const unsigned lo = __builtin_amdgcn_alignbit(d1, d0, sh), hi = __builtin_amdgcn_alignbit(d2, d1, sh);
            const unsigned hs = __builtin_amdgcn_udot4(lo, 0x38302212u, __builtin_amdgcn_udot4(hi, 0x00122230u, 0u, false), false);
            acc += (unsigned)kq[j] * hs;
            if (j == 3) centre = lo >> 24;
        }
        return inside ? (int)((acc + (1u << 15)) >> 16) : (int)centre;
    };
    int val = 0;
#ifndef DD_UNROLL
#define DD_UNROLL 1
#endif
#pragma unroll DD_UNROLL
    for (int bit = 0; bit < 4; bit++) {
        float x0 = (float)pat[4 * bit], y0 = (float)pat[4 * bit + 1], x1 = (float)pat[4 * bit + 2], y1 = (float)pat[4 * bit + 3];
        int ix0 = mis_round_f(x0 * ca - y0 * sa), iy0 = mis_round_f(x0 * sa + y0 * ca);
        int ix1 = mis_round_f(x1 * ca - y1 * sa), iy1 = mis_round_f(x1 * sa + y1 * ca);
        const int t0 = blurred(ix0, iy0), t1 = blurred(ix1, iy1);
        val |= (t0 < t1) << (bit + 4 * h);
    }
    val |= __shfl_xor(val, 32);
    if (h == 0) desc[(size_t)i * 32 + b] = (uint8_t)val;
}

constexpr int ORB_GATHER_MAX = 96;
struct GatherPtrs { const int* p[ORB_GATHER_MAX]; };
__global__ void gather_ints_kernel(GatherPtrs g, int n, int* __restrict__ out) {
    const int i = blockIdx.x * blockDim.x + threadIdx.x;
    if (i < n) out[i] = *g.p[i];
}

}

struct MisOrb {
    MisContext* ctx = nullptr;
    void (*enqueued_cb)(void*) = nullptr;
    void* enqueued_user = nullptr;
    MisOrbParams p;
    int max_w = 0, max_h = 0;
    int cur_w = 0, cur_h = 0;
    Levels L;
    Work w;
    size_t ws_stride = 0;
    int ws_frames = 0;
    int umax_host[64] = {0};
    int8_t pattern_host[1024] = {0};
    void* mem = nullptr;
    size_t pad_bytes = 0, map_bytes = 0;
    int cand_total = 0, fin_total = 0, tab_total = 0, surv_total = 0, out_cap = 0;
    std::vector<int> tab_host;
    int* host_counts = nullptr;
    bool direct_describe = false;
};

namespace {

void linear_exact_coeffs(int dlen, int slen, int* ofs, int* m1) {
    double inv = (double)dlen / (double)slen, scale = 1.0 / inv;
    for (int i = 0; i < dlen; i++) {
        double v = ((double)i + 0.5) * scale - 0.5;
        int iv = (int)floor(v);
        if (iv < 0) { ofs[i] = 0; m1[i] = 0; }
        else if (iv >= slen - 1) { ofs[i] = slen - 1; m1[i] = 0; }
        else { ofs[i] = iv; m1[i] = (int)lrint((v - (double)iv) * 256.0); }
    }
}

constexpr int ORB_MAX_LEVEL_FEATURES = 2048 - 128;

inline float level_scale(const MisOrbParams& p, int l) { return (float)pow((double)p.scale_factor, (double)l); }
inline int level_dim(int len, float sc) { return (int)lrint((double)((float)len / sc)); }

void level_budgets(const MisOrbParams& p, int* nfeat) {
    float factor = (float)(1.0 / (double)p.scale_factor);
    float nd = (float)p.nfeatures * (1 - factor) / (1 - (float)pow((double)factor, (double)p.nlevels));
    int sum = 0;
    for (int l = 0; l < p.nlevels - 1; l++) { nfeat[l] = (int)lrintf(nd); sum += nfeat[l]; nd *= factor; }
    nfeat[p.nlevels - 1] = std::max(p.nfeatures - sum, 0);
}

int check_level_sizes(MisContext* ctx, const MisOrbParams& p, int w, int h) {
    for (int l = 0; l < p.nlevels; l++) {
        const float sc = level_scale(p, l);
        MIS_CHECK(ctx, level_dim(w, sc) >= 1 && level_dim(h, sc) >= 1, MIS_E_UNSUPPORTED,
                  "ORB level %d of a %dx%d frame is empty (scale_factor %g, nlevels %d)", l, w, h, (double)p.scale_factor, p.nlevels);
    }
    return MIS_OK;
}

void plan_levels(MisOrb* o, int w, int h) {
    Levels& L = o->L;
    const MisOrbParams& p = o->p;
    L.n = p.nlevels; L.fast_t = p.fast_threshold; L.patch = p.patch_size; L.half_patch = p.patch_size / 2; L.edge = p.edge_threshold;
    size_t pad_off = 0, map_off = 0;
    int cand_off = 0, fin_off = 0, tab_off = 0, surv_off = 0;
    int nfeat[ORB_MAX_LEVELS];
    level_budgets(p, nfeat);
    for (int l = 0; l < L.n; l++) {
        LevelDesc& d = L.d[l];
        float sc = level_scale(p, l);
        d.scale = sc;
        d.w = level_dim(w, sc);
        d.h = level_dim(h, sc);
        d.pp = (int)mis_align_up((size_t)d.w + 2 * ORB_BORDER, 64);
        d.sp = (int)mis_align_up((size_t)d.w, 64);
        d.pad_off = pad_off; pad_off += (size_t)d.pp * (d.h + 2 * ORB_BORDER);
        d.map_off = map_off; map_off += (size_t)d.sp * d.h;
        d.nfeat = nfeat[l];
        d.n2 = p.score_type == 0 ? 2 * d.nfeat : d.nfeat;
        d.tiles_x = (d.w + FT_COLS - 1) / FT_COLS; d.tiles_y = (d.h + FT_ROWS - 1) / FT_ROWS;
        d.tile_off = surv_off; surv_off += d.tiles_x * d.tiles_y;
        d.cap1 = 4 * d.n2 + 4096;
        d.cap2 = std::min(d.nfeat + 128, 2048);
        d.cand_off = cand_off; cand_off += d.cap1;
        d.fin_off = fin_off; fin_off += d.cap2;
        d.tab_off = tab_off; tab_off += (2 * ((d.w + 3) & ~3) + 2 * d.h + 3) & ~3;
    }
    o->pad_bytes = pad_off; o->map_bytes = map_off; o->cand_total = cand_off; o->fin_total = fin_off; o->tab_total = tab_off; o->surv_total = surv_off;
    o->tab_host.assign(tab_off, 0);
    for (int l = 1; l < L.n; l++) {
        int* t = o->tab_host.data() + L.d[l].tab_off;
        const int dw4 = (L.d[l].w + 3) & ~3;
        linear_exact_coeffs(L.d[l].w, L.d[l - 1].w, t, t + dw4);
        linear_exact_coeffs(L.d[l].h, L.d[l - 1].h, t + 2 * dw4, t + 2 * dw4 + L.d[l].h);
    }
}

int upload_tables(MisOrb* o) {
    MisContext* ctx = o->ctx;
    if (o->tab_total)
        MIS_HIP(ctx, hipMemcpyAsync(o->w.tab, o->tab_host.data(), sizeof(int) * o->tab_total, hipMemcpyHostToDevice, ctx->stream));
    MIS_HIP(ctx, hipStreamSynchronize(ctx->stream));
    return MIS_OK;
}
// ... 156 lines not shown
    }
    if (old) MIS_HIP(ctx, hipFree(old));
    return orb_init_workspace(o);
}

}

int mis_feat_block_alloc(MisContext* ctx, size_t bytes, void** out) {
    size_t got = 0;
    const int rc = mis_pool_alloc(ctx, bytes, out, &got);
    if (rc != MIS_OK) return rc;
    std::lock_guard<std::mutex> lock(g_feat_mutex);
    g_feat_sizes[*out] = got;
    return MIS_OK;
}


extern "C" void mis_orb_default_params(MisOrbParams* p) {
    if (p) *p = MisOrbParams{4000, 1.2f, 8, 1, 0, 2, 0, 40, 20};
}

extern "C" int mis_orb_create(MisContext* ctx, const MisOrbParams* p, int max_w, int max_h, MisOrb** out) {
    if (!ctx || !out) return MIS_E_INVALID;
    MIS_CHECK(ctx, p, MIS_E_INVALID, "null params");
    MIS_CHECK(ctx, p->nlevels >= 1 && p->nlevels <= ORB_MAX_LEVELS && p->first_level == 0 && p->wta_k == 2 && p->patch_size >= 2 &&
                       p->patch_size <= 40 && p->nfeatures >= 1 && p->scale_factor > 1.f && (p->score_type == 0 || p->score_type == 1) &&
                       p->edge_threshold >= 0 && p->fast_threshold >= 1 && p->fast_threshold < 255,
              MIS_E_UNSUPPORTED, "unsupported ORB parameters (need first_level 0, wta_k 2, patch <= 40, nlevels <= 16)");
    MIS_CHECK(ctx, p->patch_size != 31, MIS_E_UNSUPPORTED, "ORB patch_size 31 (OpenCV's fixed bit_pattern_31_) is not supported");
    {
        int nfeat[ORB_MAX_LEVELS];
        level_budgets(*p, nfeat);
        for (int l = 0; l < p->nlevels; l++)
            MIS_CHECK(ctx, nfeat[l] <= ORB_MAX_LEVEL_FEATURES, MIS_E_UNSUPPORTED,
                      "ORB nfeatures %d gives level %d a budget of %d keypoints (at most %d per level)", p->nfeatures, l, nfeat[l], ORB_MAX_LEVEL_FEATURES);
    }
    MIS_CHECK(ctx, max_w >= 64 && max_h >= 64 && max_w <= 32767 && max_h <= 32767, MIS_E_INVALID, "bad maximum size");
    if (int rc = check_level_sizes(ctx, *p, max_w, max_h)) return rc;
    MIS_HIP(ctx, hipSetDevice(ctx->device));
    MisOrb* o = new MisOrb();
    o->ctx = ctx; o->p = *p; o->max_w = max_w; o->max_h = max_h;
    plan_levels(o, max_w, max_h);
    o->out_cap = o->fin_total;
    int umax[64] = {0};
    {
        int hp = p->patch_size / 2, v, v0;
        int vmax = (int)floor((double)((float)hp * sqrtf(2.f) / 2 + 1));
        int vmin = (int)ceil((double)((float)hp * sqrtf(2.f) / 2));
        for (v = 0; v <= vmax; ++v) umax[v] = (int)lrint(sqrt((double)hp * hp - (double)v * v));
        for (v = hp, v0 = 0; v >= vmin; --v) {
            while (umax[v0] == umax[v0 + 1]) ++v0;
            umax[v] = v0;
            ++v0;
        }
    }
    int8_t pat[1024];
    {
        uint64_t state = 0x34985739u;
        auto next = [&]() { state = (uint64_t)(uint32_t)state * 4164903690u + (uint32_t)(state >> 32); return (uint32_t)state; };
        int hp = p->patch_size / 2;
        for (int i = 0; i < 1024; i++) pat[i] = (int8_t)(int)(next() % (uint32_t)(2 * hp + 1) + (uint32_t)(-hp));
    }
    {
        int max_sq = 0;
        for (int i = 0; i < 512; i++) max_sq = std::max(max_sq, (int)pat[2 * i] * pat[2 * i] + (int)pat[2 * i + 1] * pat[2 * i + 1]);
        const int reach = (int)floor(sqrt((double)max_sq) + 0.5);
        o->direct_describe = reach <= DD_R && 3 + ORB_BORDER >= DD_P;
    }
    int rc0 = orb_alloc_workspace(o, 1);
    if (rc0 != MIS_OK) { delete o; return rc0; }
    memcpy(o->umax_host, umax, sizeof(umax));
    memcpy(o->pattern_host, pat, sizeof(pat));
    o->cur_w = max_w; o->cur_h = max_h;
    int rc = orb_init_workspace(o);
    if (rc != MIS_OK) { hipFree(o->mem); delete o; return rc; }
    *out = o;
    return MIS_OK;
}

extern "C" int mis_orb_destroy(MisOrb* o) {
    if (!o) return MIS_OK;
    hipSetDevice(o->ctx->device);
    hipStreamSynchronize(o->ctx->stream);
    if (o->mem) hipFree(o->mem);
    if (o->host_counts) hipHostFree(o->host_counts);
    delete o;
    return MIS_OK;
}


extern "C" int mis_orb_detect_batch(MisOrb* o, const MisImage* imgs, int n, MisFeatures* out) {
    if (!o) return MIS_E_INVALID;
    MisContext* ctx = o->ctx;
    MIS_CHECK(ctx, imgs && out && n >= 1, MIS_E_INVALID, "null argument");
    MIS_HIP(ctx, hipSetDevice(ctx->device));
    int rc;
    for (int i = 0; i < n; i++) {
        if ((rc = check_image(o, &imgs[i])) != MIS_OK) return rc;
        MIS_CHECK(ctx, imgs[i].width == imgs[0].width && imgs[i].height == imgs[0].height, MIS_E_INVALID, "batch frames must share one size");
    }
    if ((rc = replan_if_needed(o, imgs[0].width, imgs[0].height)) != MIS_OK) return rc;
    if ((rc = orb_ensure_frames(o, n)) != MIS_OK) return rc;
    std::vector<DevImage> dimg(n);
    for (int i = 0; i < n; i++) memset(&out[i], 0, sizeof(MisFeatures));
    auto fail = [&](int code) {
        hipStreamSynchronize(ctx->stream);
        for (int i = 0; i < n; i++) {
            if (out[i].keypoints || out[i].descriptors) mis_features_free(ctx, &out[i]);
            if (dimg[i].data) mis_dev_image_release(ctx, &dimg[i]);
        }
        return code;
    };
    for (int i = 0; i < n; i++) {
        out[i].img_idx = i; out[i].img_w = imgs[i].width; out[i].img_h = imgs[i].height;
        if ((rc = alloc_features(ctx, o->out_cap, 32, MIS_U8, &out[i])) != MIS_OK) return fail(rc);
        if ((rc = mis_dev_image_in(ctx, &imgs[i], &dimg[i])) != MIS_OK) return fail(rc);
    }
    const bool trace = getenv("MIS_ORB_TRACE") != nullptr;
    const auto t_enq0 = std::chrono::steady_clock::now();
    for (int g0 = 0; g0 < n; g0 += o->ws_frames) {
        const int ng = std::min(o->ws_frames, n - g0);
        if ((rc = enqueue_detect_group(o, &dimg[g0], imgs[0].width, imgs[0].height, &out[g0], ng)) != MIS_OK) return fail(rc);
    }
    if (trace) fprintf(stderr, "orb batch: %d frames enqueued in %.0f us\n", n, (double)std::chrono::duration_cast<std::chrono::microseconds>(std::chrono::steady_clock::now() - t_enq0).count());
    if (o->enqueued_cb) {
        void (*cb)(void*) = o->enqueued_cb;
        void* user = o->enqueued_user;
        o->enqueued_cb = nullptr; o->enqueued_user = nullptr;
        cb(user);
        MIS_HIP(ctx, hipSetDevice(ctx->device));
    }
    std::vector<int> counts(n);
    const int nl = o->ws_frames;
    std::vector<int> ws_flags(nl, 0);
    if (!o->host_counts) MIS_HIP(ctx, hipHostMalloc((void**)&o->host_counts, sizeof(int) * ORB_GATHER_MAX, hipHostMallocMapped));
    for (int i0 = 0; i0 < n + nl; i0 += ORB_GATHER_MAX) {
        const int m = std::min(ORB_GATHER_MAX, n + nl - i0);
        GatherPtrs gp;
        for (int k = 0; k < m; k++)
            gp.p[k] = i0 + k < n ? feat_count(&out[i0 + k], o->out_cap) : (const int*)((const char*)o->w.flags + (size_t)(i0 + k - n) * o->ws_stride);
        int* dev_view = nullptr;
        MIS_HIP(ctx, hipHostGetDevicePointer((void**)&dev_view, o->host_counts, 0));
        hipLaunchKernelGGL(gather_ints_kernel, dim3(1), dim3(ORB_GATHER_MAX), 0, ctx->stream, gp, m, dev_view);
        MIS_HIP(ctx, hipStreamSynchronize(ctx->stream));
        for (int k = 0; k < m; k++) (i0 + k < n ? counts[i0 + k] : ws_flags[i0 + k - n]) = o->host_counts[k];
    }
    int flags = 0;
    for (int k = 0; k < nl; k++) flags |= ws_flags[k];
    if (flags) hipMemset2DAsync(o->w.flags, o->ws_stride, 0, sizeof(int), (size_t)nl, ctx->stream);
    for (int i = 0; i < n; i++) { out[i].n = counts[i]; mis_dev_image_release(ctx, &dimg[i]); }
    if (flags) {
        return mis_set_error(ctx, MIS_E_OVERFLOW, "ORB candidate buffers overflowed (flags %d): too many tied scores", flags);
    }
    return MIS_OK;
}

extern "C" int mis_orb_detect(MisOrb* o, const MisImage* bgr, MisFeatures* out) { return mis_orb_detect_batch(o, bgr, 1, out); }

extern "C" int mis_orb_on_enqueued(MisOrb* o, void (*fn)(void*), void* user) {
    if (!o) return MIS_E_INVALID;
    o->enqueued_cb = fn; o->enqueued_user = user;
    return MIS_OK;
}

extern "C" int mis_features_download(MisContext* ctx, const MisFeatures* f, MisKeyPoint* kps, void* desc) {
    if (!ctx || !f) return MIS_E_INVALID;
    MIS_HIP(ctx, hipSetDevice(ctx->device));
    if (f->n > 0) {
        if (kps) MIS_HIP(ctx, hipMemcpyAsync(kps, f->keypoints, sizeof(MisKeyPoint) * (size_t)f->n, hipMemcpyDeviceToHost, ctx->stream));
        if (desc) MIS_HIP(ctx, hipMemcpyAsync(desc, f->descriptors, (size_t)f->n * f->desc_cols * mis_dtype_size(f->desc_dtype), hipMemcpyDeviceToHost, ctx->stream));
    }
    MIS_HIP(ctx, hipStreamSynchronize(ctx->stream));
    return MIS_OK;
}

extern "C" int mis_features_upload(MisContext* ctx, int img_w, int img_h, int n, const MisKeyPoint* kps, const void* desc, int desc_cols,
                                   int desc_dtype, MisFeatures* out) {
    if (!ctx || !out) return MIS_E_INVALID;
    MIS_CHECK(ctx, n >= 0 && (n == 0 || (kps && desc)) && desc_cols > 0 && (desc_dtype == MIS_U8 || desc_dtype == MIS_F32), MIS_E_INVALID,
              "bad feature arrays");
    MIS_HIP(ctx, hipSetDevice(ctx->device));
    memset(out, 0, sizeof(*out));
    out->img_w = img_w; out->img_h = img_h;
    int rc = alloc_features(ctx, std::max(n, 1), desc_cols, desc_dtype, out);
    if (rc != MIS_OK) return rc;
    if (n) {
        MIS_HIP(ctx, hipMemcpyAsync(out->keypoints, kps, sizeof(MisKeyPoint) * (size_t)n, hipMemcpyHostToDevice, ctx->stream));
        MIS_HIP(ctx, hipMemcpyAsync(out->descriptors, desc, (size_t)n * desc_cols * mis_dtype_size(desc_dtype), hipMemcpyHostToDevice, ctx->stream));
        MIS_HIP(ctx, hipStreamSynchronize(ctx->stream));
    }
    out->n = n;
    return MIS_OK;
}

extern "C" int mis_features_free(MisContext* ctx, MisFeatures* f) {
    if (!ctx || !f) return MIS_E_INVALID;
    if (f->owner_) {
        size_t bytes = 0;
        {
            std::lock_guard<std::mutex> lock(g_feat_mutex);
            auto it = g_feat_sizes.find(f->owner_);
            if (it != g_feat_sizes.end()) { bytes = it->second; g_feat_sizes.erase(it); }
        }
        if (bytes) mis_pool_free(ctx, f->owner_, bytes);
        else {
            MIS_HIP(ctx, hipSetDevice(ctx->device));
            MIS_HIP(ctx, hipStreamSynchronize(ctx->stream));
            MIS_HIP(ctx, hipFree(f->owner_));
        }
    }
    f->owner_ = nullptr; f->keypoints = nullptr; f->descriptors = nullptr; f->n = 0;
    return MIS_OK;
}

extern "C" int mis_orb_debug_level(MisOrb* o, int level, int which, uint8_t* host_out, int* width, int* height) {
    if (!o) return MIS_E_INVALID;
    MisContext* ctx = o->ctx;
    MIS_CHECK(ctx, level >= 0 && level < o->L.n && which >= 0 && which <= 2, MIS_E_INVALID, "bad level / selector");
    const LevelDesc& d = o->L.d[level];
    int w = which == 2 ? d.w + 2 * ORB_BORDER : d.w, h = which == 2 ? d.h + 2 * ORB_BORDER : d.h;
    if (width) *width = w;
    if (height) *height = h;
    if (!host_out) return MIS_OK;
    MIS_HIP(ctx, hipSetDevice(ctx->device));
    const uint8_t* src;
    size_t pitch;
    if (which == 0) { src = o->w.pad + d.pad_off + (size_t)ORB_BORDER * d.pp + ORB_BORDER; pitch = d.pp; }
    else if (which == 1) {
        MIS_HIP(ctx, hipMemsetAsync(o->w.nms + d.map_off, 0, (size_t)d.sp * d.h, ctx->stream));
        hipLaunchKernelGGL(nms_raster_kernel, dim3(256), dim3(64), 0, ctx->stream, d, o->w.tile_cnt, o->w.surv_xy, o->w.surv_sc, o->w.nms);
        src = o->w.nms + d.map_off; pitch = d.sp;
    }
    else {
        if (o->direct_describe) {
            const int pw0 = o->L.d[0].w + 2 * ORB_BORDER, ph0 = o->L.d[0].h + 2 * ORB_BORDER;
            hipLaunchKernelGGL(blur_kernel, dim3((pw0 + 63) / 64, (ph0 + 31) / 32, o->L.n), dim3(256), 0, ctx->stream, o->L, o->w.pad, o->w.blur);
// ... 17 lines not shown
```

image_stitching_amd/distributed.py:

```python
import ctypes as C
import os
import time

import numpy as np
import torch

from . import _capi as capi
from . import stitching as st


def frame_block(n, rank, world):
    base, rem = divmod(n, world)
    lo = rank * base + min(rank, rem)
    return list(range(lo, lo + base + (1 if rank < rem else 0)))


class Comm:

    def __init__(self, rank=0, world=1, group=None, always_collective=False):
        self.rank, self.world, self.group = rank, world, group
        self._stage = False
        self._solo = world == 1 and not always_collective
        if not self._solo:
            import torch.distributed as dist
# ... 15 lines not shown
        if not self._solo:
            import torch.distributed as dist
            h = self._h(t)
            dist.all_reduce(h, op=dist.ReduceOp.SUM, group=self.group)
            if h is not t:
                t.copy_(h)
        return t

    def all_to_all_bytes(self, send, recv_sizes):
        if self._solo:
            return [send[0]]
        import torch.distributed as dist
        dev = send[0].device
        hs = [self._h(t).contiguous() for t in send]
        hdev = hs[0].device
        recv = [torch.empty(int(n), dtype=torch.uint8, device=hdev) for n in recv_sizes]
        if self._stage:
            ops = []
            for k in range(self.world):
                if k == self.rank:
                    recv[k].copy_(hs[k])
                    continue
                if hs[k].numel():
                    ops.append(dist.P2POp(dist.isend, hs[k], k, group=self.group))
                if recv[k].numel():
                    ops.append(dist.P2POp(dist.irecv, recv[k], k, group=self.group))
            if ops:
                for w in dist.batch_isend_irecv(ops):
                    w.wait()
        else:
            inp, out = torch.cat(hs), torch.empty(int(sum(recv_sizes)), dtype=torch.uint8, device=hdev)
            dist.all_to_all_single(out, inp, [int(n) for n in recv_sizes], [int(t.numel()) for t in hs], group=self.group)
            o = 0
            for k, n in enumerate(recv_sizes):
                recv[k] = out[o:o + int(n)]
                o += int(n)
        return [r.to(dev) for r in recv]

    def all_gather_objects(self, obj):
        if self._solo:
            return [obj]
        import torch.distributed as dist
        out = [None] * self.world
        dist.all_gather_object(out, obj, group=self.group)
        return out

    def gather_to_root(self, t):
        if self._solo:
            return [t]
        import torch.distributed as dist
        h = self._h(t)
        bufs = [torch.empty_like(h) for _ in range(self.world)] if self.rank == 0 else None
        dist.gather(h, bufs, dst=0, group=self.group)
        return [b.to(t.device) for b in bufs] if bufs is not None else None


class _DevArray:

    def __init__(self, ptr, shape, typestr):
        self.__cuda_array_interface__ = {"shape": tuple(shape), "typestr": typestr, "data": (int(ptr), False), "version": 2}


def dev_tensor(ptr, shape, typestr, device):
    return torch.as_tensor(_DevArray(ptr, shape, typestr), device=device)


class HipEngine:

    def __init__(self, ctx, frame_size, config=None):
        self.ctx = ctx
        self.cfg = config or st.StitchConfig.hot_path()
        self.frame_size = frame_size
        self.finder = st.SiftFeatureFinder(ctx, frame_size) if self.cfg.features_type == "sift" else st.OrbFeatureFinder(ctx, frame_size)
        self.matcher = st.BestOf2NearestMatcher(ctx, self.cfg.match_conf)
        self.blender = None
        self._keep = []
        h = C.c_void_p()
        ctx.check(ctx.lib.mis_stream_create(ctx.device.index, 0, C.byref(h)))
        self._compose_stream_handle = h
        self.compose_stream = torch.cuda.ExternalStream(h.value, device=ctx.device)
        self.cctx = st.Context(ctx.device.index, stream=h.value)
        self.exchange_device = ctx.device
        self.speculative_compose = True

    def detect(self, frames):
        return self.finder.detect_batch(frames)

    def feature_counts(self, feats):
        return torch.tensor([len(f) for f in feats], dtype=torch.int32, device=self.ctx.device)

    def pack_features(self, feats, cap):
        m = len(feats)
        dev = self.ctx.device
        rb = self._row_bytes(feats)
        kps = torch.empty((m, cap * 24), dtype=torch.uint8, device=dev)
        desc = torch.empty((m, cap * rb), dtype=torch.uint8, device=dev)
        if m:
            arr = (capi.MisFeatures * m)()
            for k, f in enumerate(feats):
                C.memmove(C.byref(arr[k]), C.byref(f.raw), C.sizeof(capi.MisFeatures))
            self.ctx.check(self.ctx.lib.mis_features_pack(self.ctx.h, arr, m, int(cap), int(rb), C.c_void_p(kps.data_ptr()), C.c_void_p(desc.data_ptr())))
        return kps, desc

    def _row_bytes(self, feats=None):
        return 512 if self.cfg.features_type == "sift" else 32

    def unpack_features(self, kps_all, desc_all, counts_all):
        self._keep = [kps_all, desc_all, counts_all]
        counts = counts_all.cpu().tolist()
        w, h = self.frame_size
        sift = self.cfg.features_type == "sift"
        out = []
        for i, n in enumerate(counts):
            raw = capi.MisFeatures()
            raw.img_idx, raw.img_w, raw.img_h, raw.n = i, w, h, int(n)
            raw.keypoints = kps_all[i].data_ptr()
            raw.descriptors = desc_all[i].data_ptr()
            raw.desc_cols, raw.desc_dtype, raw.owner_ = (128, capi.F32, None) if sift else (32, capi.U8, None)
            out.append(st.ImageFeatures(self.ctx, raw))
        return out

    def match(self, feats, rank, world):
        return self.matcher(feats, rank, world)

    def confidence_tensor(self, pm, n, on_device=True):
        t = torch.from_numpy(pm.confidences()).view(n, n)
        return t.to(self.ctx.device) if on_device else t

    def refine_cameras(self, feats, pm, indices, cams):
        return st.refine_cameras(self.ctx, feats, pm, indices, cams, self.cfg)

    def match_entries(self, pm, conf_thresh):
        out = []
        n = pm.n
        for i in range(n):
            for j in range(i + 1, n):
                raw = pm._mis[i * n + j]
                if raw.src_img_idx < 0:
                    continue
                m = pm[i * n + j]
                strong = m.confidence > conf_thresh
                out.append((i, j, m.matches if strong else m.matches[:0], m.inliers_mask if strong else m.inliers_mask[:0], m.num_inliers, m.H is not None,
                            m.H, m.confidence))
        return out

    def matches_from_entries(self, per_rank, n):
        return st.PairwiseMatches.from_entries(self.ctx, n, [e for entries in per_rank for e in entries])

    def seam_local(self, frames, cams, scale):
        return [st.seam_scale_warp(self.cctx, self.cfg, self.frame_size, f, c, scale) for f, c in zip(frames, cams)]

    def seam_pack(self, item, cap):
        _, iw, mw = item
        buf = torch.zeros(cap * 4, dtype=torch.uint8, device=self.ctx.device)
        n = mw.numel()
        buf[:3 * n] = iw.reshape(-1)
        buf[3 * cap:3 * cap + n] = mw.reshape(-1)
        return buf

    def seam_unpack(self, buf, w, h, cap):
        return buf[:3 * w * h].view(h, w, 3), buf[3 * cap:3 * cap + w * h].view(h, w)

    def seam_global(self, corners, images, masks):
        self._seam = st.seam_solve(self.cctx, self.cfg, corners, images, masks)

    def warp_feed_seam_many(self, frames, cams, rois, ks):
        if not frames:
            return
        warped = self.warper.warp_fused_batch(frames, cams, rois)
# ... 96 lines not shown

    def pack_rects(self, rects, nbytes):
        buf = torch.empty(max(int(nbytes), 16), dtype=torch.uint8, device=self.ctx.device)
        if rects:
            self.cctx.check(self.cctx.lib.mis_blender_pack_rects(self.blender.h, self._rect_array(rects), len(rects), C.c_void_p(buf.data_ptr()), buf.numel()))
        return buf[:int(nbytes)]

    def add_rects(self, rects, buf):
        if rects:
            self.cctx.check(self.cctx.lib.mis_blender_add_rects(self.blender.h, self._rect_array(rects), len(rects), C.c_void_p(buf.data_ptr()), buf.numel()))

    def zero_rects(self, rects):
        if rects:
            self.cctx.check(self.cctx.lib.mis_blender_zero_rects(self.blender.h, self._rect_array(rects), len(rects)))

    def finalize_columns(self, x0, x1):
        w, h = self.blender._size
        x1 = min(x1, w)
        dst = st._empty_image(self.cctx, h, x1 - x0, 3, torch.int16)
        msk = st._empty_image(self.cctx, h, x1 - x0, 1, torch.uint8)
        d, m = st.as_image(dst), st.as_image(msk)
        self.cctx.check(self.cctx.lib.mis_blender_blend_columns(self.blender.h, int(x0), int(x1), C.byref(d), C.byref(m)))
        return dst, msk

    def strip_to_bytes(self, img, msk, cap_w):
        h, w = msk.shape
        out = torch.zeros(h * cap_w * 7, dtype=torch.uint8, device=self.ctx.device)
        lib, cx = self.cctx.lib, self.cctx
        cx.check(lib.mis_copy_2d(cx.h, C.c_void_p(out.data_ptr()), cap_w * 6, C.c_void_p(img.data_ptr()), img.stride(0) * 2, w * 6, h))
        cx.check(lib.mis_copy_2d(cx.h, C.c_void_p(out.data_ptr() + h * cap_w * 6), cap_w, C.c_void_p(msk.data_ptr()), msk.stride(0), w, h))
        return out

    def assemble(self, strips, bounds, cap_w, size):
        w, h = size
        pano = st._empty_image(self.cctx, h, w, 3, torch.int16)
        mask = st._empty_image(self.cctx, h, w, 1, torch.uint8)
        lib, cx = self.cctx.lib, self.cctx
        for k, (x0, x1) in enumerate(bounds):
            x1 = min(x1, w)
            if x1 <= x0:
                continue
            base = strips[k].data_ptr()
            cx.check(lib.mis_copy_2d(cx.h, C.c_void_p(pano.data_ptr() + x0 * 6), pano.stride(0) * 2, C.c_void_p(base), cap_w * 6, (x1 - x0) * 6, h))
            cx.check(lib.mis_copy_2d(cx.h, C.c_void_p(mask.data_ptr() + x0), mask.stride(0), C.c_void_p(base + h * cap_w * 6), cap_w, x1 - x0, h))
        return pano, mask

    def sync(self):
        torch.cuda.synchronize(self.ctx.device)


class StitchJob:

    def __init__(self, ctx, frame_size, cameras, rank=0, world_size=1, group=None, engine=None, config=None, force_collectives=False, always_collective=False):
        self.cfg = config or st.StitchConfig.hot_path()
        st.check_seam_config(self.cfg)
        self.engine = engine or HipEngine(ctx, frame_size, self.cfg)
        self.cams = cameras
        self.cams0 = cameras
        self.n = len(cameras)
        self.rank, self.world = rank, world_size
        self.comm = Comm(rank, world_size, group, always_collective)
        self.my_frames = frame_block(self.n, rank, world_size)
        self.frame_size = frame_size
        self.scale = st.Stitcher.warped_image_scale(cameras)
        self.force_collectives = force_collectives
        self.seam_needed = self.cfg.expos_comp_type != "no" or self.cfg.seam_find_type != "no"
        counts = {len(frame_block(self.n, r, world_size)) for r in range(world_size)}
        if len(counts) != 1:
            raise ValueError("the frame count must divide evenly over the ranks")

    def stage_features(self, frames):
        return self.engine.detect([frames[i] for i in self.my_frames])

    def stage_gather(self, local_feats):
        if self.world == 1 and not self.force_collectives:
            return local_feats
        counts_all = self.comm.all_gather(self.engine.feature_counts(local_feats)).flatten(0, 1)
        cap = max(int(counts_all.max()), 1)
        kps, desc = self.engine.pack_features(local_feats, cap)
        kps_all = self.comm.all_gather(kps).flatten(0, 1)
        desc_all = self.comm.all_gather(desc).flatten(0, 1)
        return self.engine.unpack_features(kps_all, desc_all, counts_all)

    def stage_match(self, feats):
        pm = self.engine.match(feats, self.rank, self.world)
        if self.world == 1 and not self.force_collectives and isinstance(self.engine, HipEngine):
            return pm, self.engine.confidence_tensor(pm, self.n, on_device=False)
        conf = self.engine.confidence_tensor(pm, self.n)
        conf = self.comm.all_reduce_sum(conf)
        return pm, conf

    def stage_prune(self, conf):
        return [int(i) for i in st.leaveBiggestComponentConf(conf.cpu().numpy().reshape(self.n, self.n), self.cfg.conf_thresh)]

    def stage_compose_prepare(self, indices):
        eng = self.engine
        self.scale = st.Stitcher.warped_image_scale([self.cams[i] for i in indices])
        g = st.compose_geometry(self.cfg, self.frame_size, self.scale)
        self._geom = g
        ccams = {i: st.scaled_camera(self.cams[i], g.aspect) for i in indices} if g.aspect != 1.0 else {i: self.cams[i] for i in indices}
        if g.size != tuple(self.frame_size) and not hasattr(eng, "resize_frame"):
            raise NotImplementedError("this engine does not resize frames (compose_megapix > 0 needs resize_frame)")
        if hasattr(eng, "warp_rois"):
            rois = dict(zip(indices, eng.warp_rois(g.warp_scale, [ccams[i] for i in indices], g.size)))
        else:
            rois = {i: eng.warp_roi(g.warp_scale, ccams[i], g.size) for i in indices}
        corners = [(rois[i][0], rois[i][1]) for i in indices]
        sizes = [(rois[i][2], rois[i][3]) for i in indices]
        btype, bands = eng.begin_compose(g.warp_scale, corners, sizes)
        self._compose_indices, self._compose_rois, self._compose_cams = indices, rois, ccams
        return btype, bands

    def stage_compose(self, frames, indices, prepared=None):
        eng = self.engine
        btype, bands = prepared if prepared is not None else self.stage_compose_prepare(indices)
        rois, ccams, g = self._compose_rois, self._compose_cams, self._geom
        mine = [i for i in self.my_frames if i in rois]
        cframes = {i: eng.resize_frame(frames[i], g.compose_scale) for i in mine} if g.size != tuple(self.frame_size) else frames
        if self.seam_needed:
            marks = getattr(self, "marks", None)
            if marks is not None:
                marks.append(("compose: sized", time.perf_counter()))
            self.stage_seam(frames, indices)
            if marks is not None:
                marks.append(("compose: seams solved", time.perf_counter()))
            if hasattr(eng, "warp_feed_seam_many"):
                eng.warp_feed_seam_many([cframes[i] for i in mine], [ccams[i] for i in mine], [rois[i] for i in mine], [indices.index(i) for i in mine])
            else:
                for i in mine:
                    eng.warp_feed_seam(cframes[i], ccams[i], rois[i], indices.index(i))
            return btype, bands
        if hasattr(eng, "warp_feed_many"):
            eng.warp_feed_many([cframes[i] for i in mine], [ccams[i] for i in mine], [rois[i] for i in mine])
        else:
            for i in mine:
                eng.warp_feed(cframes[i], ccams[i], rois[i])
        return btype, bands

    def stage_seam(self, frames, indices):
        eng = self.engine
        mine = [i for i in self.my_frames if i in indices]
        local = eng.seam_local([frames[i] for i in mine], [self.cams[i] for i in mine], self.scale)
        if getattr(self, "marks", None) is not None:
            self.marks.append(("compose: seam-scale warps enqueued", time.perf_counter()))
        if self.world == 1 and not self.force_collectives:
            items = local
        else:
            per = len(self.my_frames)
            meta = torch.zeros((per, 5), dtype=torch.int32)
            for k, (i, it) in enumerate(zip(mine, local)):
                meta[k] = torch.tensor([i, it[0][0], it[0][1], it[2].shape[1], it[2].shape[0]], dtype=torch.int32)
            meta[len(mine):, 0] = -1
            dev = torch.device(getattr(eng, "exchange_device", None) or (local[0][1].device if local else "cpu"))
            meta_all = self.comm.all_gather(meta.to(dev)).flatten(0, 1).cpu()
            cap = max(int((meta_all[:, 3] * meta_all[:, 4]).max()), 1)
            bufs = [eng.seam_pack(it, cap) for it in local] + [torch.zeros(cap * 4, dtype=torch.uint8, device=dev) for _ in range(per - len(mine))]
            all_bufs = self.comm.all_gather(torch.stack(bufs)).flatten(0, 1)
            by_index = {}
            for row, buf in zip(meta_all.tolist(), all_bufs):
                if row[0] >= 0:
                    iw, mw = eng.seam_unpack(buf, row[3], row[4], cap)
                    by_index[row[0]] = ((row[1], row[2]), iw, mw)
            items = [by_index[i] for i in indices]
        eng.seam_global([it[0] for it in items], [it[1] for it in items], [it[2] for it in items])

    def rank_region(self, r, indices, rois, bands, w0, h0):
        mine = [i for i in frame_block(self.n, r, self.world) if i in rois]
        if not mine:
# ... 35 lines not shown
            if x1 <= x0 or y1 <= y0:
                continue
            m = (x1 - x0) * (y1 - y0)
            rects.append((l, x0, y0, x1, y1, off))
            off += (m * 6 + 15) // 16 * 16 + (m * 4 + 15) // 16 * 16
        return rects, off

    def stage_reduce_finalize(self):
        eng = self.engine
        sizes = eng.level_sizes()
        bands = len(sizes) - 1
        w0, h0 = sizes[0]
        indices, rois = self._compose_indices, self._compose_rois
        world = self.world
        bounds = self.strip_bounds(w0, bands, world)
        needs = [self.need_ranges(bnd, sizes) for bnd in bounds]
        regions = [self.rank_region(r, indices, rois, bands, w0, h0) for r in range(world)]
        plan = [[self.exchange_rects(regions[r], needs[k], sizes) for k in range(world)] for r in range(world)]
        me = self.rank
        send = [eng.pack_rects(*plan[me][k]) for k in range(world)]
        recv = self.comm.all_to_all_bytes(send, [plan[r][me][1] for r in range(world)])
        full_h = [(l, lo, 0, hi, sizes[l][1], 0) for l, (lo, hi) in enumerate(needs[me]) if hi > lo]
        eng.zero_rects(full_h)
        for r in range(world):
            eng.add_rects(plan[r][me][0], recv[r])
        pw, ph = eng.pano_size
        x0, x1 = bounds[me][0], min(bounds[me][1], pw)
        cap_w = max(min(b1, pw) - b0 for b0, b1 in bounds)
        if x1 > x0:
            img, msk = eng.finalize_columns(x0, x1)
            mine = eng.strip_to_bytes(img, msk, cap_w)
        else:
            mine = torch.zeros(ph * cap_w * 7, dtype=torch.uint8, device=send[0].device)
        strips = self.comm.all_gather(mine)
        if self.rank != 0:
            return None, None
        return eng.assemble(strips, bounds, cap_w, (pw, ph))

    def stage_finalize(self):
        if self.rank == 0:
            return self.engine.finalize()
        return None, None

    def stage_exchange_finalize(self):
        if self.world == 1 and not self.force_collectives:
            return self.stage_finalize()
        side = getattr(self.engine, "compose_stream", None)
        if side is None:
            return self.stage_reduce_finalize()
        with torch.cuda.stream(side):
            return self.stage_reduce_finalize()

    def _compose_on_side_stream(self, frames, indices, prepared=None):
        eng = self.engine
        if getattr(eng, "compose_stream", None) is None:
            return self.stage_compose(frames, indices, prepared)
        with torch.cuda.stream(eng.compose_stream):
            return self.stage_compose(frames, indices, prepared)

    def run(self, frames):
        marks = self.marks = [("start", time.perf_counter())] if os.environ.get("MIS_JOB_TRACE") else None

        def mark(name):
            if marks is not None:
                marks.append((name, time.perf_counter()))
        refine = self.cfg.ba_cost_func != "no"
        solo_rank = self.world == 1 and not self.force_collectives
        spec = getattr(self.engine, "speculative_compose", False) and not refine and (not self.seam_needed or solo_rank)
        prepared = None
        side = getattr(self.engine, "compose_stream", None)
        if side is not None:
            side.wait_stream(torch.cuda.current_stream(self.engine.ctx.device))
        if spec:
            finder = getattr(self.engine, "finder", None)
            box0 = {}

            def prep():
                try:
                    with torch.cuda.stream(self.engine.compose_stream):
                        box0["p"] = self.stage_compose_prepare(list(range(self.n)))
                except BaseException as e:
                    box0["e"] = e
            hooked = hasattr(finder, "on_enqueued") and len(self.my_frames) > 0
            if hooked:
                finder.on_enqueued(prep)
            else:
                prep()
            try:
                local = self.stage_features(frames)
            finally:
                if hooked:
                    finder.on_enqueued(None)
            if "p" not in box0 and "e" not in box0:
                prep()
            if "e" in box0:
                raise box0["e"]
            prepared = box0["p"]
            feats = self.stage_gather(local)
        else:
            feats = self.stage_gather(self.stage_features(frames))
        mark("features")
        if spec:
            import threading
            everyone = list(range(self.n))
            box = {}

            fence = self.engine.match_fence_target() if hasattr(self.engine, "match_fence_target") else None

            solo = self.world == 1 and not self.force_collectives

            def work():
                try:
                    if fence is not None:
                        self.engine.compose_after_knn(fence)
                    mark("compose: fence passed")
                    box["r"] = self._compose_on_side_stream(frames, everyone, prepared)
                    mark("compose: enqueued")
                    if solo:
                        with torch.cuda.stream(self.engine.compose_stream):
                            box["f"] = self.stage_finalize()
                    mark("compose: finalise enqueued")
                except BaseException as e:
                    box["e"] = e
            if hasattr(self.engine, "on_match_enqueued"):
                self.engine.on_match_enqueued(work)
                try:
                    pm, conf = self.stage_match(feats)
                finally:
                    self.engine.on_match_enqueued(None)
                mark("match returned")
                if not box:
                    work()
                indices = self.stage_prune(conf)
                mark("pruned")
            else:
                th = threading.Thread(target=work)
                th.start()
                try:
                    pm, conf = self.stage_match(feats)
                    indices = self.stage_prune(conf)
                finally:
                    th.join()
            if "e" in box:
                raise box["e"]
            if indices == everyone and "f" in box:
                (btype, bands), (pano, mask) = box["r"], box["f"]
            else:
                btype, bands = box["r"] if indices == everyone else self._compose_on_side_stream(frames, indices)
                with torch.cuda.stream(self.engine.compose_stream):
                    pano, mask = self.stage_exchange_finalize()
            box.clear()
        else:
            pm, conf = self.stage_match(feats)
            indices = self.stage_prune(conf)
            if refine:
                if self.cfg.ba_cost_func != "reproj":
                    raise ValueError("ba_cost_func must be 'no' or 'reproj'")
                if self.world > 1 or self.force_collectives:
                    pm = self.engine.matches_from_entries(self.comm.all_gather_objects(self.engine.match_entries(pm, self.cfg.conf_thresh)), self.n)
                refined = self.engine.refine_cameras(feats, pm, indices, self.cams0)
                self.cams = list(self.cams0)
                for i, c in zip(indices, refined):
                    self.cams[i] = c
                self.scale = st.Stitcher.warped_image_scale([self.cams[i] for i in indices])
            btype, bands = self._compose_on_side_stream(frames, indices)
            pano, mask = self.stage_exchange_finalize()
        self.engine.sync()
        mark("synchronised")
        return {"pano": pano, "mask": mask, "indices": indices, "confidence": conf, "matches": pm, "features": feats,
                "pano_size": self.engine.pano_size, "num_bands": bands}

    def breakdown(self, frames, reps=3):
        out = {}

        def timed(name, fn):
            self.engine.sync()
            t0 = time.perf_counter()
            r = fn()
            self.engine.sync()
            out[name] = out.get(name, 0.0) + (time.perf_counter() - t0) * 1e3 / reps
            return r
        for _ in range(reps):
            lf = timed("features (detect+describe)", lambda: self.stage_features(frames))
            feats = timed("feature all-gather", lambda: self.stage_gather(lf))
            pm, conf = timed("match + RANSAC", lambda: self.stage_match(feats))
            idx = timed("prune (host)", lambda: self.stage_prune(conf))
            side = getattr(self.engine, "compose_stream", None)

            def on_side(fn):
                if side is None:
                    return fn()
                with torch.cuda.stream(side):
                    return fn()
            timed("warp + blend feed", lambda: on_side(lambda: self.stage_compose(frames, idx)))
            timed("blend exchange + finalise", lambda: on_side(self.stage_exchange_finalize))
        return out
```

image_stitching_amd/stitching.py:

```python
import ctypes as C
import math
from dataclasses import dataclass, field

import numpy as np

from . import _capi as capi

try:
    import torch
except Exception:
    torch = None


class MisError(RuntimeError):
    def __init__(self, code, text):
        super().__init__("libmistitch error %d: %s" % (code, text))
        self.code = code


KP_DTYPE = np.dtype([("x", "f4"), ("y", "f4"), ("size", "f4"), ("angle", "f4"), ("response", "f4"), ("octave", "i4")])
DMATCH_DTYPE = np.dtype([("query_idx", "i4"), ("train_idx", "i4"), ("img_idx", "i4"), ("distance", "f4")])

_TORCH_DT = {}
if torch is not None:
# ... 440 lines not shown
        n = self.raw.n
        kps = np.zeros(n, KP_DTYPE)
        dt = np.uint8 if self.raw.desc_dtype == capi.U8 else np.float32
        desc = np.zeros((n, self.raw.desc_cols), dt)
        if n:
            self.ctx.check(self.ctx.lib.mis_features_download(self.ctx.h, C.byref(self.raw), kps.ctypes.data_as(C.c_void_p),
                                                              desc.ctypes.data_as(C.c_void_p)))
        return kps, desc

    @staticmethod
    def upload(ctx, img_size, kps, desc, img_idx=0):
        kps = np.ascontiguousarray(kps, KP_DTYPE)
        desc = np.ascontiguousarray(desc)
        raw = capi.MisFeatures()
        ctx.check(ctx.lib.mis_features_upload(ctx.h, int(img_size[0]), int(img_size[1]), len(kps),
                                              kps.ctypes.data_as(C.c_void_p), desc.ctypes.data_as(C.c_void_p), desc.shape[1],
                                              _NP_DT[desc.dtype], C.byref(raw)))
        raw.img_idx = img_idx
        return ImageFeatures(ctx, raw)

    def close(self):
        if self.raw is not None and self.ctx.h:
            self.ctx.lib.mis_features_free(self.ctx.h, C.byref(self.raw))
        self.raw = None

    def __del__(self):
        try:
            self.close()
        except Exception:
            pass


def orb_params(**kw):
    p = capi.MisOrbParams()
    capi.load().mis_orb_default_params(C.byref(p))
    for k, v in kw.items():
        setattr(p, k, v)
    return p


class OrbFeatureFinder:

    def __init__(self, ctx, max_size, params=None):
        self.ctx = ctx
        self.params = params or orb_params()
        h = C.c_void_p()
        ctx.check(ctx.lib.mis_orb_create(ctx.h, C.byref(self.params), int(max_size[0]), int(max_size[1]), C.byref(h)))
        self.h = h

    def detect(self, img):
        raw = capi.MisFeatures()
        i = as_image(img)
        self.ctx.check(self.ctx.lib.mis_orb_detect(self.h, C.byref(i), C.byref(raw)))
        return ImageFeatures(self.ctx, raw)

    def on_enqueued(self, fn):
        if fn is None:
            self._enqueued_fn = None
            self.ctx.lib.mis_orb_on_enqueued(self.h, None, None)
            return
        self._enqueued_fn = fn
        if getattr(self, "_enqueued_cb", None) is None:
            self._enqueued_cb = C.CFUNCTYPE(None, C.c_void_p)(self._run_enqueued)
        self.ctx.check(self.ctx.lib.mis_orb_on_enqueued(self.h, C.cast(self._enqueued_cb, C.c_void_p), None))

    def _run_enqueued(self, _user):
        fn, self._enqueued_fn = getattr(self, "_enqueued_fn", None), None
        if fn is not None:
            fn()

    def detect_batch(self, imgs):
        n = len(imgs)
        arr = (capi.MisImage * n)(*[as_image(i) for i in imgs])
        raws = (capi.MisFeatures * n)()
        self.ctx.check(self.ctx.lib.mis_orb_detect_batch(self.h, arr, n, raws))
        out = []
        for k in range(n):
            r = capi.MisFeatures()
            C.memmove(C.byref(r), C.byref(raws[k]), C.sizeof(capi.MisFeatures))
            r.img_idx = k
            out.append(ImageFeatures(self.ctx, r))
        return out

    def debug_level(self, level, which):
        w, h = C.c_int(), C.c_int()
        self.ctx.check(self.ctx.lib.mis_orb_debug_level(self.h, level, which, None, C.byref(w), C.byref(h)))
        out = np.zeros((h.value, w.value), np.uint8)
        self.ctx.check(self.ctx.lib.mis_orb_debug_level(self.h, level, which, out.ctypes.data_as(C.c_void_p), C.byref(w), C.byref(h)))
        return out

    def close(self):
        if getattr(self, "h", None) and self.ctx.h:
            self.ctx.lib.mis_orb_destroy(self.h)
        self.h = None

    def __del__(self):
        try:
            self.close()
        except Exception:
            pass


class SiftFeatureFinder:

    def __init__(self, ctx, max_size, params=None):
        self.ctx = ctx
        p = capi.MisSiftParams()
        ctx.lib.mis_sift_default_params(C.byref(p))
        for k, v in (params or {}).items():
            setattr(p, k, v)
        self.params = p
        h = C.c_void_p()
        ctx.check(ctx.lib.mis_sift_create(ctx.h, C.byref(p), int(max_size[0]), int(max_size[1]), C.byref(h)))
        self.h = h

    def detect(self, img):
        raw = capi.MisFeatures()
        i = as_image(img)
        self.ctx.check(self.ctx.lib.mis_sift_detect(self.h, C.byref(i), C.byref(raw)))
        return ImageFeatures(self.ctx, raw)

    def detect_batch(self, imgs):
        n = len(imgs)
        if n == 0:
            return []
        arr = (capi.MisImage * n)(*[as_image(im) for im in imgs])
        raws = (capi.MisFeatures * n)()
        self.ctx.check(self.ctx.lib.mis_sift_detect_batch(self.h, arr, n, raws))
        out = []
        for k in range(n):
            raw = capi.MisFeatures()
            C.memmove(C.byref(raw), C.byref(raws[k]), C.sizeof(capi.MisFeatures))
            out.append(ImageFeatures(self.ctx, raw))
        return out

    def debug_level(self, img, octave, layer, dog=False):
        i = as_image(img)
        w, h = C.c_int(), C.c_int()
        self.ctx.check(self.ctx.lib.mis_sift_debug_level(self.h, C.byref(i), octave, layer, int(dog), None, C.byref(w), C.byref(h)))
        out = np.zeros((h.value, w.value), np.float32)
        self.ctx.check(self.ctx.lib.mis_sift_debug_level(self.h, C.byref(i), octave, layer, int(dog), out.ctypes.data_as(C.c_void_p), C.byref(w), C.byref(h)))
        return out

    def close(self):
        if getattr(self, "h", None) and self.ctx.h:
            self.ctx.lib.mis_sift_destroy(self.h)
        self.h = None

    def __del__(self):
        try:
            self.close()
        except Exception:
            pass


def computeImageFeatures(finder, img, img_idx=0):
    f = finder.detect(img)
    f.img_idx = img_idx
    return f


@dataclass
class MatchesInfo:
    src_img_idx: int = -1
    dst_img_idx: int = -1
    matches: np.ndarray = field(default_factory=lambda: np.zeros(0, DMATCH_DTYPE))
# ... 20 lines not shown

    def __init__(self, ctx, mis, n):
        self._ctx, self._mis, self.n = ctx, mis, n
        self._cache = {}

    @classmethod
    def from_entries(cls, ctx, n, entries):
        mis = (capi.MisMatchesInfo * (n * n))()
        keep = []
        for k in range(n * n):
            mis[k].src_img_idx = mis[k].dst_img_idx = -1
        for i, j, matches, mask, num_inliers, has_H, H, conf in entries:
            mm = np.ascontiguousarray(matches, DMATCH_DTYPE)
            mk = np.ascontiguousarray(mask, np.uint8)
            sw = mm.copy()
            sw["query_idx"], sw["train_idx"] = mm["train_idx"], mm["query_idx"]
            Hd = np.asarray(H, np.float64).reshape(3, 3) if has_H else None
            for (a, b, arr, Hm) in ((i, j, mm, Hd), (j, i, sw, np.linalg.inv(Hd) if has_H else None)):
                e = mis[a * n + b]
                e.src_img_idx, e.dst_img_idx, e.n_matches = a, b, len(arr)
                e.matches = C.cast(arr.ctypes.data, C.POINTER(capi.MisDMatch)) if len(arr) else None
                e.inliers_mask = C.cast(mk.ctypes.data, C.POINTER(C.c_uint8)) if len(mk) else None
                e.num_inliers, e.has_H, e.confidence = int(num_inliers), 1 if has_H else 0, float(conf)
                if has_H:
                    for q, v in enumerate(Hm.reshape(9)):
                        e.H[q] = v
            keep += [mm, mk, sw]
        obj = cls(ctx, mis, n)
        obj._keep, obj._borrowed = keep, True
        return obj

    def __len__(self):
        return self.n * self.n

    def __getitem__(self, i):
        if isinstance(i, slice):
            return [self[k] for k in range(*i.indices(len(self)))]
        if i < 0:
            i += len(self)
        if i not in self._cache:
            self._cache[i] = _unpack_mi(self._mis[i])
        return self._cache[i]

    def __iter__(self):
        return (self[i] for i in range(len(self)))

    def confidences(self):
        return np.array([self._mis[i].confidence for i in range(len(self))], np.float64)

    def __del__(self):
        try:
            if self._mis is not None and self._ctx.h and not getattr(self, "_borrowed", False):
                self._ctx.lib.mis_matches_free(self._mis, self.n * self.n)
            self._mis = None
        except Exception:
            pass


def match_params(**kw):
    p = capi.MisMatchParams()
    capi.load().mis_match_default_params(C.byref(p))
    for k, v in kw.items():
        setattr(p, k, v)
    return p


class BestOf2NearestMatcher:

    def __init__(self, ctx, match_conf=0.32, num_matches_thresh1=6, num_matches_thresh2=6):
        self.ctx = ctx
        self.params = match_params(match_conf=match_conf, num_matches_thresh1=num_matches_thresh1,
                                   num_matches_thresh2=num_matches_thresh2)

    def __call__(self, features, rank=0, world_size=1):
        n = len(features)
        arr = (capi.MisFeatures * n)()
        for k, f in enumerate(features):
            C.memmove(C.byref(arr[k]), C.byref(f.raw), C.sizeof(capi.MisFeatures))
        mis = (capi.MisMatchesInfo * (n * n))()
        if world_size == 1:
            rc = self.ctx.lib.mis_match_all_pairs(self.ctx.h, arr, n, C.byref(self.params), mis)
        else:
            rc = self.ctx.lib.mis_match_pairs_sharded(self.ctx.h, arr, n, C.byref(self.params), rank, world_size, mis)
        self.ctx.check(rc)
        return PairwiseMatches(self.ctx, mis, n)

    def collectGarbage(self):
        pass


def leaveBiggestComponent(pairwise_matches, n, conf_threshold):
    lib = capi.load()
    mis = (capi.MisMatchesInfo * (n * n))()
    for i, m in enumerate(pairwise_matches):
        mis[i].confidence = m.confidence
    idx = np.zeros(n, np.int32)
    k = C.c_int()
    rc = lib.mis_leave_biggest_component(mis, n, float(conf_threshold), idx.ctypes.data_as(C.c_void_p), C.byref(k))
    if rc != capi.MIS_OK:
        raise MisError(rc, "mis_leave_biggest_component")
    return idx[: k.value].copy()


def leaveBiggestComponentConf(confidence, conf_threshold):
    conf = np.ascontiguousarray(confidence, np.float64)
    n = conf.shape[0]
    idx = np.zeros(n, np.int32)
    k = C.c_int()
    rc = capi.load().mis_leave_biggest_component_conf(conf.ctypes.data_as(C.c_void_p), n, float(conf_threshold), idx.ctypes.data_as(C.c_void_p), C.byref(k))
    if rc != capi.MIS_OK:
        raise MisError(rc, "mis_leave_biggest_component_conf")
    return idx[: k.value].copy()


WAVE_CORRECT_HORIZ, WAVE_CORRECT_VERT = 0, 1


def refine_cameras(ctx, features, pairwise_matches, indices, cameras, cfg):
    n, k = pairwise_matches.n, len(indices)
    sub = (capi.MisMatchesInfo * (k * k))()
    for a, i in enumerate(indices):
        for b, j in enumerate(indices):
            C.memmove(C.byref(sub[a * k + b]), C.byref(pairwise_matches._mis[i * n + j]), C.sizeof(capi.MisMatchesInfo))
            sub[a * k + b].src_img_idx, sub[a * k + b].dst_img_idx = a, b
    view = PairwiseMatches.__new__(PairwiseMatches)
    view._ctx, view._mis, view.n, view._cache = ctx, sub, k, {}
    view._owner = pairwise_matches
    start = [dict(focal=float(cameras[i]["K"][0, 0]), aspect=float(cameras[i]["K"][1, 1] / cameras[i]["K"][0, 0]), ppx=float(cameras[i]["K"][0, 2]),
                  ppy=float(cameras[i]["K"][1, 2]), R=cameras[i]["R"]) for i in indices]
    try:
        refined = bundle_adjust_reproj(ctx, [features[i] for i in indices], view, start, cfg.conf_thresh, cfg.ba_refine_mask)
    finally:
        view._mis = None
    if cfg.wave_correct != "no":
        Rs = wave_correct([c["R"] for c in refined], WAVE_CORRECT_VERT if cfg.wave_correct == "vert" else WAVE_CORRECT_HORIZ)
        for c, R in zip(refined, Rs):
            c["R"] = R
    out = []
    for i, c in zip(indices, refined):
        d = dict(cameras[i])
        d["K"] = np.array([[c["focal"], 0, c["ppx"]], [0, c["focal"] * c["aspect"], c["ppy"]], [0, 0, 1]], np.float64)
        d["R"] = c["R"]
        d["f"] = c["focal"]
        out.append(d)
    return out


def bundle_adjust_reproj(ctx, features, pairwise_matches, cameras, conf_thresh=0.95, refine_mask="xxxxx"):
    n = len(features)
    if not isinstance(pairwise_matches, PairwiseMatches):
        raise TypeError("pairwise_matches must be the PairwiseMatches object a BestOf2NearestMatcher call returned")
    arr = (capi.MisFeatures * n)()
    for k, f in enumerate(features):
        C.memmove(C.byref(arr[k]), C.byref(f.raw), C.sizeof(capi.MisFeatures))
    cams = (capi.MisCameraParams * n)()
    for k, c in enumerate(cameras):
        cams[k].focal, cams[k].aspect, cams[k].ppx, cams[k].ppy = float(c["focal"]), float(c.get("aspect", 1.0)), float(c["ppx"]), float(c["ppy"])
        R = np.asarray(c["R"], np.float64).reshape(9)
        t = np.asarray(c.get("t", np.zeros(3)), np.float64).reshape(3)
        for i in range(9):
            cams[k].R[i] = R[i]
        for i in range(3):
            cams[k].t[i] = t[i]
    ctx.check(ctx.lib.mis_bundle_adjust_reproj(ctx.h, arr, pairwise_matches._mis, n, float(conf_thresh), refine_mask.encode(), cams))
    return [dict(focal=cams[k].focal, aspect=cams[k].aspect, ppx=cams[k].ppx, ppy=cams[k].ppy, R=np.array(list(cams[k].R)).reshape(3, 3),
                 t=np.array(list(cams[k].t))) for k in range(n)]
# ... 195 lines not shown
```

include/mistitch.h:

```cpp
#ifndef MISTITCH_H
#define MISTITCH_H

#include <stddef.h>
#include <stdint.h>

#ifdef __cplusplus
extern "C" {
#endif

#define MIS_OK 0
#define MIS_E_INVALID (-1)
#define MIS_E_HIP (-2)
#define MIS_E_NOMEM (-3)
#define MIS_E_OVERFLOW (-4)
#define MIS_E_STATE (-5)
#define MIS_E_UNSUPPORTED (-6)
#define MIS_FENCE_TIMEOUT 1

enum { MIS_MEM_HOST = 0, MIS_MEM_DEVICE = 1 };
enum { MIS_U8 = 0, MIS_S16 = 1, MIS_F32 = 2 };
enum { MIS_INTER_NEAREST = 0, MIS_INTER_LINEAR = 1 };
enum { MIS_BORDER_CONSTANT = 0, MIS_BORDER_REFLECT = 2 };
enum { MIS_BLEND_NO = 0, MIS_BLEND_FEATHER = 1, MIS_BLEND_MULTI_BAND = 2 };

typedef struct MisContext MisContext;
typedef struct MisOrb MisOrb;
typedef struct MisBlender MisBlender;

typedef struct { int x, y; } MisPoint;
typedef struct { int width, height; } MisSize;
typedef struct { int x, y, width, height; } MisRect;

typedef struct {
    void* data;
    int width, height, channels;
    size_t stride;
    int dtype;
    int mem;
} MisImage;

int mis_context_create(int device, void* stream, MisContext** out);
int mis_stream_create(int device, int priority, void** stream);
int mis_stream_destroy(void* stream);
int mis_context_destroy(MisContext* ctx);
int mis_context_synchronize(MisContext* ctx);
int mis_context_wait(MisContext* ctx, MisContext* other);
const char* mis_last_error(const MisContext* ctx);
const char* mis_version(void);
int mis_image_free(MisContext* ctx, MisImage* img);

typedef struct {
    float x, y, size, angle, response;
    int octave;
} MisKeyPoint;

typedef struct {
    int nfeatures;
    float scale_factor;
    int nlevels, edge_threshold, first_level, wta_k, score_type, patch_size, fast_threshold;
} MisOrbParams;

typedef struct {
    int img_idx;
    int img_w, img_h;
    int n;
    MisKeyPoint* keypoints;
    void* descriptors;
    int desc_cols, desc_dtype;
    void* owner_;
} MisFeatures;

void mis_orb_default_params(MisOrbParams* p);
int mis_orb_create(MisContext* ctx, const MisOrbParams* p, int max_width, int max_height, MisOrb** out);
int mis_orb_destroy(MisOrb* orb);
int mis_orb_detect(MisOrb* orb, const MisImage* bgr, MisFeatures* out);
int mis_orb_detect_batch(MisOrb* orb, const MisImage* bgr, int n_images, MisFeatures* out);
int mis_orb_on_enqueued(MisOrb* orb, void (*fn)(void*), void* user);
int mis_features_download(MisContext* ctx, const MisFeatures* f, MisKeyPoint* kps_host, void* desc_host);
int mis_features_upload(MisContext* ctx, int img_w, int img_h, int n, const MisKeyPoint* kps_host,
                        const void* desc_host, int desc_cols, int desc_dtype, MisFeatures* out);
int mis_features_free(MisContext* ctx, MisFeatures* f);
int mis_features_pack(MisContext* ctx, const MisFeatures* feats, int m, int cap, int row_bytes, void* kps_dst, void* desc_dst);
int mis_copy_2d(MisContext* ctx, void* dst, size_t dst_pitch, const void* src, size_t src_pitch, size_t width_bytes, size_t height);
int mis_orb_debug_level(MisOrb* orb, int level, int which, uint8_t* host_out, int* width, int* height);

typedef struct {
    float match_conf;
    int num_matches_thresh1, num_matches_thresh2;
    double ransac_thresh;
    int max_iters;
    double confidence;
} MisMatchParams;

typedef struct { int query_idx, train_idx, img_idx; float distance; } MisDMatch;

typedef struct {
    int src_img_idx, dst_img_idx;
    int n_matches;
    MisDMatch* matches;
    uint8_t* inliers_mask;
    int num_inliers;
    int has_H;
    double H[9];
    double confidence;
} MisMatchesInfo;

void mis_match_default_params(MisMatchParams* p);
int mis_match_all_pairs(MisContext* ctx, const MisFeatures* feats, int n, const MisMatchParams* p, MisMatchesInfo* out);
int mis_match_pairs_sharded(MisContext* ctx, const MisFeatures* feats, int n, const MisMatchParams* p, int rank,
                            int world_size, MisMatchesInfo* out);
int mis_matches_free(MisMatchesInfo* m, int count);
long long mis_match_sequence(MisContext* ctx);
int mis_match_knn_fence(MisContext* ctx, void* stream, long long target_seq, int timeout_ms);
int mis_match_on_enqueued(MisContext* ctx, void (*fn)(void*), void* user);
int mis_knn2(MisContext* ctx, const MisFeatures* query, const MisFeatures* train, int* idx2_host, float* dist2_host);
int mis_find_homography(MisContext* ctx, const float* src_xy, const float* dst_xy, int n, double thresh, int max_iters,
                        double confidence, double H[9], uint8_t* mask, int* ok);
int mis_leave_biggest_component(const MisMatchesInfo* pairwise, int n, float conf_threshold, int* indices, int* n_indices);
int mis_leave_biggest_component_conf(const double* confidence, int n, float conf_threshold, int* indices, int* n_indices);

typedef struct {
    double focal, aspect, ppx, ppy;
    double R[9];
    double t[3];
} MisCameraParams;
int mis_bundle_adjust_reproj(MisContext* ctx, const MisFeatures* features, const MisMatchesInfo* pairwise, int n, float conf_thresh,
                             const char* refine_mask, MisCameraParams* cameras);
int mis_wave_correct(double* rmats, int n, int kind);

int mis_warp_roi(float scale, int src_width, int src_height, const float K[9], const float R[9], MisRect* roi);
int mis_warp_roi_batch(MisContext* ctx, float scale, int src_width, int src_height, int n, const float* Ks, const float* Rs, MisRect* rois);
int mis_warp_spherical(MisContext* ctx, const MisImage* src, float scale, const float K[9], const float R[9], int interp,
                       int border, MisImage* dst, MisPoint* tl);
int mis_warp_spherical_fused(MisContext* ctx, const MisImage* src_bgr, float scale, const float K[9], const float R[9],
                             MisImage* dst_s16x3, MisImage* dst_mask, MisPoint* tl);
int mis_warp_spherical_fused_roi(MisContext* ctx, const MisImage* src_bgr, float scale, const float K[9], const float R[9],
                                 const MisRect* roi, MisImage* dst_s16x3, MisImage* dst_mask, MisPoint* tl);
int mis_warp_spherical_fused_batch(MisContext* ctx, const MisImage* srcs_u8x3, int n, float scale, const float* Ks, const float* Rs, const MisRect* rois,
                                   MisImage* dsts_s16x3, MisImage* dmasks_u8, MisPoint* tls);
int mis_warp_spherical_fused_batch_timed(MisContext* ctx, const MisImage* srcs_u8x3, int n, float scale, const float* Ks, const float* Rs,
                                         const MisRect* rois, MisImage* dsts_s16x3, MisImage* dmasks_u8, MisPoint* tls, int repeats, float* avg_us);
int mis_warp_spherical_fused_timed(MisContext* ctx, const MisImage* src_bgr, float scale, const float K[9], const float R[9],
                                   MisImage* dst_s16x3, MisImage* dst_mask, MisPoint* tl, int repeats, float* avg_us);

typedef struct {
    int nfeatures, n_octave_layers;
    double contrast_threshold, edge_threshold, sigma;
} MisSiftParams;
typedef struct MisSift MisSift;
void mis_sift_default_params(MisSiftParams* p);
int mis_sift_create(MisContext* ctx, const MisSiftParams* params , int max_width, int max_height, MisSift** out);
int mis_sift_destroy(MisSift* sift);
int mis_sift_detect(MisSift* sift, const MisImage* bgr, MisFeatures* out);
int mis_sift_detect_batch(MisSift* sift, const MisImage* bgr, int n_images, MisFeatures* out);
int mis_sift_debug_level(MisSift* sift, const MisImage* bgr, int octave, int layer, int dog, float* host_out, int* width, int* height);

int mis_resize_linear_exact(MisContext* ctx, const MisImage* src, int dst_w, int dst_h, double fx, double fy, MisImage* dst);
int mis_rotate(MisContext* ctx, const MisImage* src, int rotate_code, MisImage* dst);
int mis_seam_mask_apply(MisContext* ctx, const MisImage* seam_mask_warped, MisImage* mask_warped);

typedef struct MisCompensator MisCompensator;
int mis_compensator_create(MisContext* ctx, int block_width, int block_height, int nr_gain_filtering_iterations, MisCompensator** out);
int mis_compensator_destroy(MisCompensator* c);
int mis_compensator_feed(MisCompensator* c, const MisPoint* corners, const MisImage* images, const MisImage* masks, int n);
int mis_compensator_gain_map(const MisCompensator* c, int index, float* map_host, int capacity, int* blocks_x, int* blocks_y);
int mis_compensator_apply(MisCompensator* c, int index, MisImage* image);
int mis_seam_voronoi(MisContext* ctx, const MisPoint* corners, MisImage* masks, int n);
#define MIS_SEAM_DP_COLOR 0
int mis_seam_dp(MisContext* ctx, const MisPoint* corners, const MisImage* images, MisImage* masks, int n, int cost_func);

int mis_blend_config(int blend_type, float blend_strength, int pano_width, int pano_height, int* type_out, int* num_bands,
                     float* sharpness);
int mis_result_roi(const MisPoint* corners, const MisSize* sizes, int n, MisRect* roi);
int mis_blender_create(MisContext* ctx, int type, int num_bands, float sharpness, MisBlender** out);
int mis_blender_destroy(MisBlender* b);
int mis_blender_prepare(MisBlender* b, const MisPoint* corners, const MisSize* sizes, int n);
int mis_blender_num_bands(const MisBlender* b);
int mis_blender_feed(MisBlender* b, const MisImage* img_s16x3, const MisImage* mask_u8, MisPoint tl);
int mis_blender_feed_batch(MisBlender* b, const MisImage* imgs_s16x3, const MisImage* masks_u8, const MisPoint* tls, int n);
int mis_blender_blend(MisBlender* b, MisImage* dst_s16x3, MisImage* dst_mask);
int mis_blender_blend_columns(MisBlender* b, int x0, int x1, MisImage* dst_s16x3, MisImage* dst_mask);
typedef struct { int level, x0, y0, x1, y1; unsigned long long offset; } MisLevelRect;
int mis_blender_pack_rects(MisBlender* b, const MisLevelRect* rects, int n, void* dev_buf, size_t bytes);
int mis_blender_add_rects(MisBlender* b, const MisLevelRect* rects, int n, const void* dev_buf, size_t bytes);
int mis_blender_zero_rects(MisBlender* b, const MisLevelRect* rects, int n);
int mis_compose_frames(MisBlender* b, const MisImage* frames, int n, float scale, const float* Ks, const float* Rs, const MisRect* rois);
int mis_blender_feed_rect(const MisBlender* b, int width, int height, MisPoint tl, MisRect* tile);
int mis_blender_level_info(const MisBlender* b, int level, int* width, int* height, void** lap_dev, void** weight_dev);

#ifdef __cplusplus
}
// ... 3 lines not shown
```

Before: 3373.

## Enqueue matching on pending ORB counts without host sync between detect and match

ORB detection is split into enqueue and wait phases. The matcher now runs with device-side keypoint counts, sized by the capacity upper bound, so its kernels are launched before the host learns the real counts. The host sync after detection is replaced by an event wait, which lets detect and match enqueue overlap with host work. In exchange, buffers are sized to capacity rather than actual counts, and the error and cleanup paths become more complex.

```diff
diff --git a/host/job.cpp b/host/job.cpp
--- a/host/job.cpp
+++ b/host/job.cpp
@@ -130,23 +130,24 @@
     check(ctx_, mis_orb_on_enqueued(orb_, &StitchJob::prep_hook, this), "mis_orb_on_enqueued");
     std::vector<MisFeatures> feats(n_);
     std::memset(feats.data(), 0, sizeof(MisFeatures) * n_);
-    const int rc_f = mis_orb_detect_batch(orb_, frames.data(), n_, feats.data());
+    const int rc_f = mis_orb_detect_batch_enqueue(orb_, frames.data(), n_, feats.data());
     mis_orb_on_enqueued(orb_, nullptr, nullptr);
-    check(ctx_, rc_f, "mis_orb_detect_batch");
+    check(ctx_, rc_f, "mis_orb_detect_batch_enqueue");
     if (!prep_ran_) prep_hook(this);
-    if (!prep_error_.empty()) throw std::runtime_error(prep_error_);
-    for (int i = 0; i < n_; i++) { feats[i].img_idx = i; out.num_features.push_back(feats[i].n); }
     if (!pairwise_.empty()) { mis_matches_free(pairwise_.data(), (int)pairwise_.size()); pairwise_.clear(); }
     pairwise_.assign((size_t)n_ * n_, MisMatchesInfo{});
     MisMatchParams mp;
     mis_match_default_params(&mp);
     mp.match_conf = cfg_.match_conf;
     hook_frames_ = &frames; hook_ran_ = false; hook_error_.clear();
-    check(ctx_, mis_match_on_enqueued(ctx_, &StitchJob::hook, this), "mis_match_on_enqueued");
-    const int rc = mis_match_all_pairs(ctx_, feats.data(), n_, &mp, pairwise_.data());
+    int rc = prep_error_.empty() ? mis_match_on_enqueued(ctx_, &StitchJob::hook, this) : MIS_OK;
+    if (rc == MIS_OK && prep_error_.empty()) rc = mis_match_all_pairs_pending(ctx_, orb_, feats.data(), n_, &mp, pairwise_.data());
+    else mis_orb_detect_batch_wait(orb_, feats.data(), n_);
     mis_match_on_enqueued(ctx_, nullptr, nullptr);
+    for (int i = 0; i < n_; i++) { feats[i].img_idx = i; out.num_features.push_back(feats[i].n); }
     for (auto& f : feats) mis_features_free(ctx_, &f);
-    check(ctx_, rc, "mis_match_all_pairs");
+    if (!prep_error_.empty()) throw std::runtime_error(prep_error_);
+    check(ctx_, rc, "mis_match_all_pairs_pending");
     if (!hook_ran_) hook(this);
     if (!hook_error_.empty()) throw std::runtime_error(hook_error_);
     out.confidence.resize((size_t)n_ * n_);
diff --git a/image_stitching_amd/_capi.py b/image_stitching_amd/_capi.py
--- a/image_stitching_amd/_capi.py
+++ b/image_stitching_amd/_capi.py
@@ -96,6 +96,8 @@
     "mis_orb_destroy": (_i, [_vp]),
     "mis_orb_detect": (_i, [_vp, _P(MisImage), _P(MisFeatures)]),
     "mis_orb_detect_batch": (_i, [_vp, _P(MisImage), _i, _P(MisFeatures)]),
+    "mis_orb_detect_batch_enqueue": (_i, [_vp, _P(MisImage), _i, _P(MisFeatures)]),
+    "mis_orb_detect_batch_wait": (_i, [_vp, _P(MisFeatures), _i]),
     "mis_orb_on_enqueued": (_i, [_vp, _vp, _vp]),
     "mis_features_download": (_i, [_vp, _P(MisFeatures), _vp, _vp]),
     "mis_features_upload": (_i, [_vp, _i, _i, _i, _vp, _vp, _i, _i, _P(MisFeatures)]),
@@ -109,6 +111,7 @@
     "mis_sift_debug_level": (_i, [_vp, _P(MisImage), _i, _i, _i, _vp, _P(_i), _P(_i)]),
     "mis_match_default_params": (None, [_P(MisMatchParams)]),
     "mis_match_all_pairs": (_i, [_vp, _P(MisFeatures), _i, _P(MisMatchParams), _P(MisMatchesInfo)]),
+    "mis_match_all_pairs_pending": (_i, [_vp, _vp, _P(MisFeatures), _i, _P(MisMatchParams), _P(MisMatchesInfo)]),
     "mis_match_pairs_sharded": (_i, [_vp, _P(MisFeatures), _i, _P(MisMatchParams), _i, _i, _P(MisMatchesInfo)]),
     "mis_matches_free": (_i, [_P(MisMatchesInfo), _i]),
     "mis_match_sequence": (C.c_longlong, [_vp]),
diff --git a/image_stitching_amd/csrc/common.h b/image_stitching_amd/csrc/common.h
--- a/image_stitching_amd/csrc/common.h
+++ b/image_stitching_amd/csrc/common.h
@@ -34,6 +34,7 @@
 int mis_aux_stream(MisContext* ctx, int k, hipStream_t* out);
 void mis_pool_free(MisContext* ctx, void* p, size_t bytes);
 int mis_feat_block_alloc(MisContext* ctx, size_t bytes, void** out);
+int mis_orb_pending_counts(MisContext* ctx, MisOrb* o, const MisFeatures* feats, int n, const int** counts, int* cap);
 
 #define MIS_HIP(ctx, call)                                                                             \
     do {                                                                                               \
diff --git a/image_stitching_amd/csrc/match.hip b/image_stitching_amd/csrc/match.hip
--- a/image_stitching_amd/csrc/match.hip
+++ b/image_stitching_amd/csrc/match.hip
@@ -12,8 +12,10 @@
 struct FeatDev {
     const uint8_t* desc;
     const MisKeyPoint* kps;
+    const int* cnt;
     int n, w, h;
 };
+__device__ __forceinline__ int feat_n(const FeatDev& F) { return F.cnt ? min(max(*F.cnt, 0), F.n) : F.n; }
 
 struct PairDesc {
     int i, j;
@@ -29,18 +31,19 @@
     const bool fwd = (blockIdx.y & 1) == 0;
     const FeatDev Q = feats[fwd ? pd.i : pd.j], T = feats[fwd ? pd.j : pd.i];
     const size_t off = fwd ? pd.knn_off12 : pd.knn_off21;
+    const int nq = feat_n(Q), ntr = feat_n(T);
     const int q0 = blockIdx.x * 256;
-    if (q0 >= Q.n) return;
+    if (q0 >= nq) return;
     const int q = q0 + threadIdx.x;
-    const bool active = q < Q.n;
+    const bool active = q < nq;
     uint4 a0 = make_uint4(0, 0, 0, 0), a1 = a0;
     if (active) {
         const uint4* p = reinterpret_cast<const uint4*>(Q.desc + (size_t)q * 32);
         a0 = p[0]; a1 = p[1];
     }
     int k0 = 0x7fffffff, k1 = 0x7fffffff;
-    for (int t0 = 0; t0 < T.n; t0 += KNN_TILE) {
-        const int nt = min(KNN_TILE, T.n - t0);
+    for (int t0 = 0; t0 < ntr; t0 += KNN_TILE) {
+        const int nt = min(KNN_TILE, ntr - t0);
         __syncthreads();
         const uint4* src = reinterpret_cast<const uint4*>(T.desc + (size_t)t0 * 32);
         for (int k = threadIdx.x; k < nt * 2; k += 256) tr[k] = src[k];
@@ -91,10 +94,11 @@
 }
 __global__ __launch_bounds__(256) void hamming_expand4_kernel(const FeatDev* feats, const HmFrame* fr, int8_t* out) {
     const FeatDev F = feats[blockIdx.y];
-    const int npad = (F.n + HM_ROWPAD - 1) / HM_ROWPAD * HM_ROWPAD;
+    const int nf = feat_n(F);
+    const int npad = (nf + HM_ROWPAD - 1) / HM_ROWPAD * HM_ROWPAD;
     const int item = blockIdx.x * 256 + threadIdx.x, d = item >> 3, w = item & 7;
     if (d >= npad) return;
-    const bool live = d < F.n;
+    const bool live = d < nf;
     const unsigned x = live ? reinterpret_cast<const unsigned*>(F.desc)[(size_t)d * 8 + w] : 0u;
     unsigned tq[4], qq[4];
 #pragma unroll
@@ -168,7 +172,7 @@
     const PairDesc pd = pairs[job.pair];
     const bool fwd = job.dir == 0;
     const int qi = fwd ? pd.i : pd.j, ti = fwd ? pd.j : pd.i;
-    const int nq = feats[qi].n, nt = feats[ti].n;
+    const int nq = __builtin_amdgcn_readfirstlane(feat_n(feats[qi])), nt = __builtin_amdgcn_readfirstlane(feat_n(feats[ti]));
     const size_t off = fwd ? pd.knn_off12 : pd.knn_off21;
     const int q0 = job.q0;
     if (q0 >= nq) return;
@@ -449,6 +453,7 @@
                                                            MisDMatch* matches, float* src_xy, float* dst_xy, int* n_matches) {
     const PairDesc pd = pairs[blockIdx.x];
     const FeatDev F1 = feats[pd.i], F2 = feats[pd.j];
+    const int n1 = feat_n(F1), n2 = feat_n(F2);
     MisDMatch* m = matches + pd.m_off;
     float* sp = src_xy + 2 * pd.m_off;
     float* dp = dst_xy + 2 * pd.m_off;
@@ -458,10 +463,10 @@
     const float* d21 = dist2 + pd.knn_off21 * 2;
     const float hw1 = (float)F1.w * 0.5f, hh1 = (float)F1.h * 0.5f, hw2 = (float)F2.w * 0.5f, hh2 = (float)F2.h * 0.5f;
     int base = 0;
-    if (F2.n >= 2)
-        for (int q0 = 0; q0 < F1.n; q0 += 1024) {
+    if (n2 >= 2)
+        for (int q0 = 0; q0 < n1; q0 += 1024) {
             int q = q0 + threadIdx.x, ok = 0;
-            if (q < F1.n) ok = d12[2 * q] < ratio * d12[2 * q + 1];
+            if (q < n1) ok = d12[2 * q] < ratio * d12[2 * q + 1];
             int tot, off = block_scan_flag(ok, &tot);
             if (ok) {
                 int t = i12[2 * q];
@@ -472,14 +477,14 @@
             }
             base += tot;
         }
-    if (F1.n >= 2)
-        for (int q0 = 0; q0 < F2.n; q0 += 1024) {
+    if (n1 >= 2)
+        for (int q0 = 0; q0 < n2; q0 += 1024) {
             int q = q0 + threadIdx.x, ok = 0, t1 = 0;
-            if (q < F2.n) {
+            if (q < n2) {
                 ok = d21[2 * q] < ratio * d21[2 * q + 1];
                 if (ok) {
                     t1 = i21[2 * q];
-                    bool acc12 = F2.n >= 2 && d12[2 * t1] < ratio * d12[2 * t1 + 1];
+                    bool acc12 = n2 >= 2 && d12[2 * t1] < ratio * d12[2 * t1 + 1];
                     if (acc12 && i12[2 * t1] == q) ok = 0;
                 }
             }
@@ -604,6 +609,7 @@
     hipEvent_t ev_gate = nullptr;
     std::atomic<long long> seq{0}, knn_seq{0};
     hipEvent_t ev_lists = nullptr;
+    hipEvent_t ev_done = nullptr;
     void (*enqueued_cb)(void*) = nullptr;
     void* enqueued_user = nullptr;
     MatchWorkspace() { pinned.host = true; }
@@ -618,6 +624,7 @@
         if (ev_side_done) hipEventDestroy(ev_side_done);
         if (ev_knn) hipEventDestroy(ev_knn);
         if (ev_draw1) hipEventDestroy(ev_draw1);
+        if (ev_done) hipEventDestroy(ev_done);
     }
 };
 
@@ -636,10 +643,23 @@
     m->src_img_idx = -1; m->dst_img_idx = -1;
 }
 
-int match_impl(MisContext* ctx, const MisFeatures* feats, int n, const MisMatchParams* p, int rank, int world, MisMatchesInfo* out) {
+int match_impl(MisContext* ctx, const MisFeatures* feats, int n, const MisMatchParams* p, int rank, int world, MisMatchesInfo* out,
+               MisOrb* orb = nullptr, MisFeatures* pending = nullptr) {
+    struct BatchWait {
+        MisOrb* orb; MisFeatures* f; int n; bool done = false;
+        int wait() { done = true; return mis_orb_detect_batch_wait(orb, f, n); }
+        ~BatchWait() { if (orb && !done) mis_orb_detect_batch_wait(orb, f, n); }
+    } batch{orb, pending, n};
     MIS_CHECK(ctx, feats && p && out && n >= 1, MIS_E_INVALID, "null argument");
     MIS_CHECK(ctx, world >= 1 && rank >= 0 && rank < world, MIS_E_INVALID, "bad rank / world size");
     MIS_HIP(ctx, hipSetDevice(ctx->device));
+    std::vector<const int*> dev_counts;
+    int pend_cap = 0;
+    if (orb) {
+        dev_counts.resize(n);
+        if (int rc = mis_orb_pending_counts(ctx, orb, feats, n, dev_counts.data(), &pend_cap)) return rc;
+    }
+    auto nf = [&](int i) { return orb ? pend_cap : feats[i].n; };
     const auto t_begin = std::chrono::steady_clock::now();
     struct SeqGuard {
         MatchWorkspace* ws; long long seq;
@@ -654,34 +674,34 @@
     for (int i = 0; i < n; i++) {
         const bool bin_i = feats[i].desc_dtype == MIS_U8 && feats[i].desc_cols == 32;
         const bool l2_i = feats[i].desc_dtype == MIS_F32 && feats[i].desc_cols >= 1 && feats[i].desc_cols <= 128;
-        MIS_CHECK(ctx, feats[i].n == 0 || bin_i || l2_i, MIS_E_UNSUPPORTED,
+        MIS_CHECK(ctx, nf(i) == 0 || bin_i || l2_i, MIS_E_UNSUPPORTED,
                   "all-pairs matching supports 32-byte binary descriptors (Hamming) or f32 descriptors of <= 128 columns (L2)");
-        MIS_CHECK(ctx, feats[i].n < (1 << 22), MIS_E_UNSUPPORTED, "more than 4 M keypoints in one image");
-        if (feats[i].n > 0) { if (l2_i) use_l2 = true; else use_bin = true; }
-        fd[i] = FeatDev{(const uint8_t*)feats[i].descriptors, feats[i].keypoints, feats[i].n, feats[i].img_w, feats[i].img_h};
+        MIS_CHECK(ctx, nf(i) < (1 << 22), MIS_E_UNSUPPORTED, "more than 4 M keypoints in one image");
+        if (nf(i) > 0) { if (l2_i) use_l2 = true; else use_bin = true; }
+        fd[i] = FeatDev{(const uint8_t*)feats[i].descriptors, feats[i].keypoints, orb ? dev_counts[i] : nullptr, nf(i), feats[i].img_w, feats[i].img_h};
     }
     int pair_index = 0;
     for (int i = 0; i < n; i++)
         for (int j = i + 1; j < n; j++) {
-            if (feats[i].n <= 0 || feats[j].n <= 0) continue;
+            if (nf(i) <= 0 || nf(j) <= 0) continue;
             if ((pair_index++ % world) != rank) continue;
             PairDesc pd;
             pd.i = i; pd.j = j;
-            pd.knn_off12 = knn_total; knn_total += feats[i].n;
-            pd.knn_off21 = knn_total; knn_total += feats[j].n;
-            pd.m_off = m_total; pd.cap = feats[i].n + feats[j].n; m_total += pd.cap;
+            pd.knn_off12 = knn_total; knn_total += nf(i);
+            pd.knn_off21 = knn_total; knn_total += nf(j);
+            pd.m_off = m_total; pd.cap = nf(i) + nf(j); m_total += pd.cap;
             pairs.push_back(pd);
         }
     MIS_CHECK(ctx, !(use_l2 && use_bin), MIS_E_INVALID, "binary and float descriptors cannot be mixed in one matcher call");
     for (int i = 0, cols = 0; use_l2 && i < n; i++)
-        if (feats[i].n > 0) {
+        if (nf(i) > 0) {
             MIS_CHECK(ctx, cols == 0 || feats[i].desc_cols == cols, MIS_E_INVALID, "float descriptors of different widths in one matcher call");
             cols = feats[i].desc_cols;
         }
     const int np = (int)pairs.size();
-    if (np == 0) return MIS_OK;
+    if (np == 0) return orb ? batch.wait() : MIS_OK;
     int maxq = 0;
-    for (int i = 0; i < n; i++) maxq = std::max(maxq, feats[i].n);
+    for (int i = 0; i < n; i++) maxq = std::max(maxq, nf(i));
     std::vector<HmJob> hm_jobs;
     if (!use_l2 && maxq <= HM_MAX_TRAINS) {
         std::vector<HmJob> lists[8];
@@ -689,7 +709,7 @@
             for (int k = 0; k < np; k++) {
                 const int dir = pairs[k].j == t ? 0 : (pairs[k].i == t ? 1 : -1);
                 if (dir < 0) continue;
-                const int nqf = feats[dir == 0 ? pairs[k].i : pairs[k].j].n;
+                const int nqf = nf(dir == 0 ? pairs[k].i : pairs[k].j);
                 for (int q0 = 0; q0 < nqf; q0 += 256) lists[t & 7].push_back(HmJob{k, dir, q0, 0});
             }
         size_t longest = 0;
@@ -700,7 +720,8 @@
     }
     MatchWorkspace* ws = workspace(ctx);
     hipStream_t st = ctx->stream;
-    MIS_HIP(ctx, hipStreamSynchronize(st));
+    if (orb) { if (ws->ev_done) MIS_HIP(ctx, hipEventSynchronize(ws->ev_done)); }
+    else MIS_HIP(ctx, hipStreamSynchronize(st));
     Carver dc;
     const size_t o_feats = dc.take(sizeof(FeatDev) * n), o_pairs = dc.take(sizeof(PairDesc) * np), o_idx = dc.take(sizeof(int) * 2 * knn_total),
                  o_dist = dc.take(sizeof(int) * 2 * knn_total), o_matches = dc.take(sizeof(MisDMatch) * m_total), o_src = dc.take(sizeof(float) * 2 * m_total),
@@ -734,7 +755,7 @@
         Carver lc;
         const size_t o_fr = lc.take(sizeof(HmFrame) * n), o_jobs = lc.take(sizeof(HmJob) * hm_jobs.size());
         for (int i = 0; i < n; i++) {
-            const size_t rows = (size_t)(std::max(feats[i].n, 1) + HM_ROWPAD - 1) / HM_ROWPAD * HM_ROWPAD;
+            const size_t rows = (size_t)(std::max(nf(i), 1) + HM_ROWPAD - 1) / HM_ROWPAD * HM_ROWPAD;
             hf[i].train_off = lc.take(rows * 128); hf[i].query_off = lc.take(rows * 128);
         }
         MIS_HIP(ctx, ws->l2.reserve(lc.off));
@@ -868,6 +889,8 @@
         for (int k = 6; k < 8; k++) { cs.src[k] = nullptr; cs.dst[k] = nullptr; cs.bytes[k] = 0; }
         hipLaunchKernelGGL(copy_segments_kernel, dim3(64), dim3(256), 0, st, cs);
     }
+    if (!ws->ev_done) MIS_HIP(ctx, hipEventCreateWithFlags(&ws->ev_done, hipEventDisableTiming));
+    MIS_HIP(ctx, hipEventRecord(ws->ev_done, st));
     ws->knn_seq.store(seq_guard.seq);
     if (ws->enqueued_cb) {
         void (*cb)(void*) = ws->enqueued_cb;
@@ -878,6 +901,15 @@
     }
     const bool trace = getenv("MIS_MATCH_TRACE") != nullptr;
     const auto tq = std::chrono::steady_clock::now();
+    if (orb) {
+        const int rc_b = batch.wait();
+        if (rc_b != MIS_OK) {
+            hipStreamSynchronize(st);
+            return rc_b;
+        }
+    }
+    const auto tw = std::chrono::steady_clock::now();
+    auto skipped = [&](const PairDesc& pd) { return orb && (feats[pd.i].n <= 0 || feats[pd.j].n <= 0); };
     auto drop_lists = [&]() {
         for (int k = 0; k < np; k++) {
             const PairDesc& pd = pairs[k];
@@ -890,6 +922,7 @@
         size_t packed_off = 0;
         for (int k = 0; k < np; k++) {
             const PairDesc& pd = pairs[k];
+            if (skipped(pd)) continue;
             MisMatchesInfo* a = &out[pd.i * n + pd.j];
             MisMatchesInfo* b = &out[pd.j * n + pd.i];
             a->src_img_idx = pd.i; a->dst_img_idx = pd.j;
@@ -919,6 +952,7 @@
     }
     for (int k = 0; k < np; k++) {
         const PairDesc& pd = pairs[k];
+        if (skipped(pd)) continue;
         MisMatchesInfo* a = &out[pd.i * n + pd.j];
         MisMatchesInfo* b = &out[pd.j * n + pd.i];
         MisDMatch* bm = b->matches;
@@ -948,7 +982,8 @@
     if (trace) {
         const auto te = std::chrono::steady_clock::now();
         auto us = [](auto a, auto b) { return (double)std::chrono::duration_cast<std::chrono::microseconds>(b - a).count(); };
-        fprintf(stderr, "match: enqueue %.0f us, device wait %.0f us, host assembly %.0f us\n", us(t_begin, tq), us(tq, ts), us(ts, te));
+        fprintf(stderr, "match: enqueue %.0f us, feature batch wait %.0f us, device wait %.0f us, host assembly %.0f us\n", us(t_begin, tq), us(tq, tw), us(tw, ts),
+                us(ts, te));
         if (ws->tev[0] && ws->tev[1] && ws->tev[3] && ws->tev[4] && ws->tev[5] && ws->tev[6]) {
             float e1 = 0, e3 = 0, e4 = 0, e5 = 0, e6 = 0;
             hipEventElapsedTime(&e1, ws->tev[0], ws->tev[1]); hipEventElapsedTime(&e3, ws->tev[0], ws->tev[3]); hipEventElapsedTime(&e4, ws->tev[0], ws->tev[4]);
@@ -1002,6 +1037,11 @@
 extern "C" int mis_match_all_pairs(MisContext* ctx, const MisFeatures* feats, int n, const MisMatchParams* p, MisMatchesInfo* out) {
     if (!ctx) return MIS_E_INVALID;
     return match_impl(ctx, feats, n, p, 0, 1, out);
+}
+
+extern "C" int mis_match_all_pairs_pending(MisContext* ctx, MisOrb* orb, MisFeatures* feats, int n, const MisMatchParams* p, MisMatchesInfo* out) {
+    if (!ctx || !orb) return MIS_E_INVALID;
+    return match_impl(ctx, feats, n, p, 0, 1, out, orb, feats);
 }
 
 extern "C" int mis_match_pairs_sharded(MisContext* ctx, const MisFeatures* feats, int n, const MisMatchParams* p, int rank, int world,
@@ -1039,8 +1079,8 @@
     uint8_t* D = (uint8_t*)ws->dev.p;
     int bad = 0;
     if (binary) {
-        FeatDev fd[2] = {{(const uint8_t*)q->descriptors, q->keypoints, q->n, q->img_w, q->img_h},
-                         {(const uint8_t*)t->descriptors, t->keypoints, t->n, t->img_w, t->img_h}};
+        FeatDev fd[2] = {{(const uint8_t*)q->descriptors, q->keypoints, nullptr, q->n, q->img_w, q->img_h},
+                         {(const uint8_t*)t->descriptors, t->keypoints, nullptr, t->n, t->img_w, t->img_h}};
         PairDesc pd;
         pd.i = 0; pd.j = 1; pd.knn_off12 = 0; pd.knn_off21 = q->n; pd.m_off = 0; pd.cap = q->n + t->n;
         MIS_HIP(ctx, hipMemcpyAsync(D + o_feats, fd, sizeof(fd), hipMemcpyHostToDevice, st));
diff --git a/image_stitching_amd/csrc/orb.hip b/image_stitching_amd/csrc/orb.hip
--- a/image_stitching_amd/csrc/orb.hip
+++ b/image_stitching_amd/csrc/orb.hip
@@ -914,6 +914,10 @@
     int cand_total = 0, fin_total = 0, tab_total = 0, surv_total = 0, out_cap = 0;
     std::vector<int> tab_host;
     int* host_counts = nullptr;
+    int host_counts_cap = 0;
+    hipEvent_t ev_counts = nullptr;
+    int pend_n = 0;
+    std::vector<DevImage> pend_img;
     bool direct_describe = false;
 };
 
@@ -1236,17 +1240,20 @@
     if (!o) return MIS_OK;
     hipSetDevice(o->ctx->device);
     hipStreamSynchronize(o->ctx->stream);
+    for (DevImage& d : o->pend_img) if (d.data) mis_dev_image_release(o->ctx, &d);
     if (o->mem) hipFree(o->mem);
     if (o->host_counts) hipHostFree(o->host_counts);
+    if (o->ev_counts) hipEventDestroy(o->ev_counts);
     delete o;
     return MIS_OK;
 }
 
 
-extern "C" int mis_orb_detect_batch(MisOrb* o, const MisImage* imgs, int n, MisFeatures* out) {
+extern "C" int mis_orb_detect_batch_enqueue(MisOrb* o, const MisImage* imgs, int n, MisFeatures* out) {
     if (!o) return MIS_E_INVALID;
     MisContext* ctx = o->ctx;
     MIS_CHECK(ctx, imgs && out && n >= 1, MIS_E_INVALID, "null argument");
+    MIS_CHECK(ctx, o->pend_n == 0, MIS_E_STATE, "a batch of this finder is still pending (mis_orb_detect_batch_wait)");
     MIS_HIP(ctx, hipSetDevice(ctx->device));
     int rc;
     for (int i = 0; i < n; i++) {
@@ -1255,6 +1262,13 @@
     }
     if ((rc = replan_if_needed(o, imgs[0].width, imgs[0].height)) != MIS_OK) return rc;
     if ((rc = orb_ensure_frames(o, n)) != MIS_OK) return rc;
+    const int nl = o->ws_frames;
+    if (o->host_counts_cap < n + nl) {
+        if (o->host_counts) { MIS_HIP(ctx, hipHostFree(o->host_counts)); o->host_counts = nullptr; o->host_counts_cap = 0; }
+        MIS_HIP(ctx, hipHostMalloc((void**)&o->host_counts, sizeof(int) * (size_t)(n + nl), hipHostMallocMapped));
+        o->host_counts_cap = n + nl;
+    }
+    if (!o->ev_counts) MIS_HIP(ctx, hipEventCreateWithFlags(&o->ev_counts, hipEventDisableTiming));
     std::vector<DevImage> dimg(n);
     for (int i = 0; i < n; i++) memset(&out[i], 0, sizeof(MisFeatures));
     auto fail = [&](int code) {
@@ -1276,7 +1290,19 @@
         const int ng = std::min(o->ws_frames, n - g0);
         if ((rc = enqueue_detect_group(o, &dimg[g0], imgs[0].width, imgs[0].height, &out[g0], ng)) != MIS_OK) return fail(rc);
     }
+    int* dev_view = nullptr;
+    if (hipHostGetDevicePointer((void**)&dev_view, o->host_counts, 0) != hipSuccess) return fail(mis_set_error(ctx, MIS_E_HIP, "hipHostGetDevicePointer failed"));
+    for (int i0 = 0; i0 < n + nl; i0 += ORB_GATHER_MAX) {
+        const int m = std::min(ORB_GATHER_MAX, n + nl - i0);
+        GatherPtrs gp;
+        for (int k = 0; k < m; k++)
+            gp.p[k] = i0 + k < n ? feat_count(&out[i0 + k], o->out_cap) : (const int*)((const char*)o->w.flags + (size_t)(i0 + k - n) * o->ws_stride);
+        hipLaunchKernelGGL(gather_ints_kernel, dim3(1), dim3(ORB_GATHER_MAX), 0, ctx->stream, gp, m, dev_view + i0);
+    }
+    if (hipEventRecord(o->ev_counts, ctx->stream) != hipSuccess) return fail(mis_set_error(ctx, MIS_E_HIP, "hipEventRecord failed"));
     if (trace) fprintf(stderr, "orb batch: %d frames enqueued in %.0f us\n", n, (double)std::chrono::duration_cast<std::chrono::microseconds>(std::chrono::steady_clock::now() - t_enq0).count());
+    o->pend_img = std::move(dimg);
+    o->pend_n = n;
     if (o->enqueued_cb) {
         void (*cb)(void*) = o->enqueued_cb;
         void* user = o->enqueued_user;
@@ -1284,28 +1310,40 @@
         cb(user);
         MIS_HIP(ctx, hipSetDevice(ctx->device));
     }
-    std::vector<int> counts(n);
+    return MIS_OK;
+}
+
+extern "C" int mis_orb_detect_batch_wait(MisOrb* o, MisFeatures* out, int n) {
+    if (!o) return MIS_E_INVALID;
+    MisContext* ctx = o->ctx;
+    MIS_CHECK(ctx, out && n >= 1 && n == o->pend_n, MIS_E_STATE, "no batch of %d frames is pending", n);
+    MIS_HIP(ctx, hipSetDevice(ctx->device));
+    const hipError_t e = hipEventSynchronize(o->ev_counts);
+    for (DevImage& d : o->pend_img) if (d.data) mis_dev_image_release(ctx, &d);
+    o->pend_img.clear();
+    o->pend_n = 0;
+    if (e != hipSuccess) return mis_set_error(ctx, MIS_E_HIP, "hipEventSynchronize failed: %s (%s:%d)", hipGetErrorString(e), __FILE__, __LINE__);
     const int nl = o->ws_frames;
-    std::vector<int> ws_flags(nl, 0);
-    if (!o->host_counts) MIS_HIP(ctx, hipHostMalloc((void**)&o->host_counts, sizeof(int) * ORB_GATHER_MAX, hipHostMallocMapped));
-    for (int i0 = 0; i0 < n + nl; i0 += ORB_GATHER_MAX) {
-        const int m = std::min(ORB_GATHER_MAX, n + nl - i0);
-        GatherPtrs gp;
-        for (int k = 0; k < m; k++)
-            gp.p[k] = i0 + k < n ? feat_count(&out[i0 + k], o->out_cap) : (const int*)((const char*)o->w.flags + (size_t)(i0 + k - n) * o->ws_stride);
-        int* dev_view = nullptr;
-        MIS_HIP(ctx, hipHostGetDevicePointer((void**)&dev_view, o->host_counts, 0));
-        hipLaunchKernelGGL(gather_ints_kernel, dim3(1), dim3(ORB_GATHER_MAX), 0, ctx->stream, gp, m, dev_view);
-        MIS_HIP(ctx, hipStreamSynchronize(ctx->stream));
-        for (int k = 0; k < m; k++) (i0 + k < n ? counts[i0 + k] : ws_flags[i0 + k - n]) = o->host_counts[k];
-    }
     int flags = 0;
-    for (int k = 0; k < nl; k++) flags |= ws_flags[k];
+    for (int k = 0; k < nl; k++) flags |= o->host_counts[n + k];
     if (flags) hipMemset2DAsync(o->w.flags, o->ws_stride, 0, sizeof(int), (size_t)nl, ctx->stream);
-    for (int i = 0; i < n; i++) { out[i].n = counts[i]; mis_dev_image_release(ctx, &dimg[i]); }
+    for (int i = 0; i < n; i++) out[i].n = o->host_counts[i];
     if (flags) {
         return mis_set_error(ctx, MIS_E_OVERFLOW, "ORB candidate buffers overflowed (flags %d): too many tied scores", flags);
     }
+    return MIS_OK;
+}
+
+extern "C" int mis_orb_detect_batch(MisOrb* o, const MisImage* imgs, int n, MisFeatures* out) {
+    const int rc = mis_orb_detect_batch_enqueue(o, imgs, n, out);
+    return rc != MIS_OK ? rc : mis_orb_detect_batch_wait(o, out, n);
+}
+
+int mis_orb_pending_counts(MisContext* ctx, MisOrb* o, const MisFeatures* feats, int n, const int** counts, int* cap) {
+    MIS_CHECK(ctx, o->ctx == ctx, MIS_E_INVALID, "the finder belongs to another context");
+    MIS_CHECK(ctx, n == o->pend_n, MIS_E_STATE, "the features are not those of this finder's pending batch of %d frames", o->pend_n);
+    for (int i = 0; i < n; i++) counts[i] = feat_count(&feats[i], o->out_cap);
+    *cap = o->out_cap;
     return MIS_OK;
 }
 
diff --git a/image_stitching_amd/distributed.py b/image_stitching_amd/distributed.py
--- a/image_stitching_amd/distributed.py
+++ b/image_stitching_amd/distributed.py
@@ -121,9 +121,16 @@
         self.cctx = st.Context(ctx.device.index, stream=h.value)
         self.exchange_device = ctx.device
         self.speculative_compose = True
+        self.pending_match = self.cfg.features_type == "orb"
 
     def detect(self, frames):
         return self.finder.detect_batch(frames)
+
+    def detect_enqueue(self, frames):
+        return self.finder.detect_batch_enqueue(frames)
+
+    def match_pending(self, feats):
+        return self.matcher.match_pending(self.finder, feats)
 
     def feature_counts(self, feats):
         return torch.tensor([len(f) for f in feats], dtype=torch.int32, device=self.ctx.device)
@@ -386,8 +393,8 @@
         desc_all = self.comm.all_gather(desc).flatten(0, 1)
         return self.engine.unpack_features(kps_all, desc_all, counts_all)
 
-    def stage_match(self, feats):
-        pm = self.engine.match(feats, self.rank, self.world)
+    def stage_match(self, feats, pending=False):
+        pm = self.engine.match_pending(feats) if pending else self.engine.match(feats, self.rank, self.world)
         if self.world == 1 and not self.force_collectives and isinstance(self.engine, HipEngine):
             return pm, self.engine.confidence_tensor(pm, self.n, on_device=False)
         conf = self.engine.confidence_tensor(pm, self.n)
@@ -589,24 +596,29 @@
                 except BaseException as e:
                     box0["e"] = e
             hooked = hasattr(finder, "on_enqueued") and len(self.my_frames) > 0
+            pending = (hooked and solo_rank and getattr(self.engine, "pending_match", False) and hasattr(self.engine, "on_match_enqueued")
+                       and self.my_frames == list(range(self.n)))
             if hooked:
                 finder.on_enqueued(prep)
             else:
                 prep()
             try:
-                local = self.stage_features(frames)
+                local = self.engine.detect_enqueue([frames[i] for i in self.my_frames]) if pending else self.stage_features(frames)
             finally:
                 if hooked:
                     finder.on_enqueued(None)
             if "p" not in box0 and "e" not in box0:
                 prep()
             if "e" in box0:
+                if pending:
+                    finder.wait_batch(local)
                 raise box0["e"]
             prepared = box0["p"]
-            feats = self.stage_gather(local)
+            feats = local if pending else self.stage_gather(local)
         else:
+            pending = False
             feats = self.stage_gather(self.stage_features(frames))
-        mark("features")
+        mark("features enqueued" if pending else "features")
         if spec:
             import threading
             everyone = list(range(self.n))
@@ -632,7 +644,7 @@
             if hasattr(self.engine, "on_match_enqueued"):
                 self.engine.on_match_enqueued(work)
                 try:
-                    pm, conf = self.stage_match(feats)
+                    pm, conf = self.stage_match(feats, pending)
                 finally:
                     self.engine.on_match_enqueued(None)
                 mark("match returned")
diff --git a/image_stitching_amd/stitching.py b/image_stitching_amd/stitching.py
--- a/image_stitching_amd/stitching.py
+++ b/image_stitching_amd/stitching.py
@@ -546,6 +546,29 @@
             out.append(ImageFeatures(self.ctx, r))
         return out
 
+    def detect_batch_enqueue(self, imgs):
+        n = len(imgs)
+        arr = (capi.MisImage * n)(*[as_image(i) for i in imgs])
+        raws = (capi.MisFeatures * n)()
+        self.ctx.check(self.ctx.lib.mis_orb_detect_batch_enqueue(self.h, arr, n, raws))
+        out = []
+        for k in range(n):
+            r = capi.MisFeatures()
+            C.memmove(C.byref(r), C.byref(raws[k]), C.sizeof(capi.MisFeatures))
+            r.img_idx = k
+            out.append(ImageFeatures(self.ctx, r))
+        return out
+
+    def wait_batch(self, features):
+        n = len(features)
+        arr = (capi.MisFeatures * n)()
+        for k, f in enumerate(features):
+            C.memmove(C.byref(arr[k]), C.byref(f.raw), C.sizeof(capi.MisFeatures))
+        rc = self.ctx.lib.mis_orb_detect_batch_wait(self.h, arr, n)
+        for k, f in enumerate(features):
+            f.raw.n = arr[k].n
+        self.ctx.check(rc)
+
     def debug_level(self, level, which):
         w, h = C.c_int(), C.c_int()
         self.ctx.check(self.ctx.lib.mis_orb_debug_level(self.h, level, which, None, C.byref(w), C.byref(h)))
@@ -732,6 +755,18 @@
             rc = self.ctx.lib.mis_match_all_pairs(self.ctx.h, arr, n, C.byref(self.params), mis)
         else:
             rc = self.ctx.lib.mis_match_pairs_sharded(self.ctx.h, arr, n, C.byref(self.params), rank, world_size, mis)
+        self.ctx.check(rc)
+        return PairwiseMatches(self.ctx, mis, n)
+
+    def match_pending(self, finder, features):
+        n = len(features)
+        arr = (capi.MisFeatures * n)()
+        for k, f in enumerate(features):
+            C.memmove(C.byref(arr[k]), C.byref(f.raw), C.sizeof(capi.MisFeatures))
+        mis = (capi.MisMatchesInfo * (n * n))()
+        rc = self.ctx.lib.mis_match_all_pairs_pending(self.ctx.h, finder.h, arr, n, C.byref(self.params), mis)
+        for k, f in enumerate(features):
+            f.raw.n = arr[k].n
         self.ctx.check(rc)
         return PairwiseMatches(self.ctx, mis, n)
 
diff --git a/include/mistitch.h b/include/mistitch.h
--- a/include/mistitch.h
+++ b/include/mistitch.h
@@ -75,6 +75,8 @@
 int mis_orb_destroy(MisOrb* orb);
 int mis_orb_detect(MisOrb* orb, const MisImage* bgr, MisFeatures* out);
 int mis_orb_detect_batch(MisOrb* orb, const MisImage* bgr, int n_images, MisFeatures* out);
+int mis_orb_detect_batch_enqueue(MisOrb* orb, const MisImage* bgr, int n_images, MisFeatures* out);
+int mis_orb_detect_batch_wait(MisOrb* orb, MisFeatures* out, int n_images);
 int mis_orb_on_enqueued(MisOrb* orb, void (*fn)(void*), void* user);
 int mis_features_download(MisContext* ctx, const MisFeatures* f, MisKeyPoint* kps_host, void* desc_host);
 int mis_features_upload(MisContext* ctx, int img_w, int img_h, int n, const MisKeyPoint* kps_host,
@@ -107,6 +109,7 @@
 
 void mis_match_default_params(MisMatchParams* p);
 int mis_match_all_pairs(MisContext* ctx, const MisFeatures* feats, int n, const MisMatchParams* p, MisMatchesInfo* out);
+int mis_match_all_pairs_pending(MisContext* ctx, MisOrb* orb, MisFeatures* feats, int n, const MisMatchParams* p, MisMatchesInfo* out);
 int mis_match_pairs_sharded(MisContext* ctx, const MisFeatures* feats, int n, const MisMatchParams* p, int rank,
                             int world_size, MisMatchesInfo* out);
 int mis_matches_free(MisMatchesInfo* m, int count);
```

Result: no change. 3343 (median of 6 runs) (-0.9%).
